# DerryHub/BEVFormer_tensorrt

Hardware: AMD Instinct MI355X
Metric: frames/sec BEVFormer-base bs=1 fp16 end-to-end on MI355X (re-hosted model, random weights, synthetic 6-camera frames) (higher is better)
Workload: dtype f16

## Files before the change

bevformer_tensorrt_amd/bevformer.py:

```python
import math
import os
import time

import torch
import torch.nn as nn
import torch.nn.functional as F

from . import functions as _hip_ops
from . import geometry as G
from .functions.dispatch import OWN_KERNELS, own_kernel_choice, using as _dispatch_using
from .functions.linear import tsgemm_weight_stationary
from .utils import lib as _lib

CONFIGS = {
    "tiny": dict(depth=50, dcn=(False, False, False, False), fpn_in=[2048], out_indices=(3,), levels=1,
                 image=(480, 800), bev=(50, 50), enc_layers=3, style="pytorch"),
    "small": dict(depth=101, dcn=(False, False, True, True), fpn_in=[2048], out_indices=(3,), levels=1,
                  image=(736, 1280), bev=(150, 150), enc_layers=3, style="caffe"),
    "base": dict(depth=101, dcn=(False, False, True, True), fpn_in=[512, 1024, 2048], out_indices=(1, 2, 3),
                 levels=4, image=(928, 1600), bev=(200, 200), enc_layers=6, style="caffe"),
}
PC_RANGE = [-51.2, -51.2, -5.0, 51.2, 51.2, 3.0]
POST_CENTER_RANGE = [-61.2, -61.2, -10.0, 61.2, 61.2, 10.0]
MAX_DETECTIONS = 300
EMBED, HEADS, NUM_QUERY, NUM_CAMS = 256, 8, 900, 6


inverse_sigmoid = G.inverse_sigmoid


_CAM_IDX = {}


def _take_cams(t, cams):
    cams = tuple(cams)
    if cams == tuple(range(t.shape[0])):
        return t
    key = (cams, str(t.device))
    idx = _CAM_IDX.get(key)
    if idx is None:
        idx = _CAM_IDX[key] = torch.tensor(cams, dtype=torch.long, device=t.device)
    return t.index_select(0, idx)


def _rows(x):
    return x.permute(0, 2, 3, 1).reshape(-1, x.shape[1])


def _from_rows(y, n, h, w):
    return y.view(n, h, w, y.shape[-1]).permute(0, 3, 1, 2)


_FUSED_LINEAR = {"enabled": os.environ.get("BEVOPS_FUSED_LINEAR", "1") != "0"}
_R3 = {"enabled": os.environ.get("BEVOPS_R3_FUSIONS", "1") != "0"}
_TSA_LOCAL = {"enabled": os.environ.get("BEVOPS_TSA_LOCAL", "1") == "1"}
_TSA_GLUE = {"enabled": os.environ.get("BEVOPS_TSA_GLUE", "1") == "1"}


def _or_none(fn, *args, **kwargs):
    try:
        return fn(*args, **kwargs)
    except _lib.BevopsError as exc:
        if exc.status != _lib.NOT_SUPPORTED:
            raise
        return None


def _fused_linear(ops, x, weight, bias, residual, relu):
    fn = getattr(ops, "linear_bias_act", None)
    if fn is None or not _FUSED_LINEAR["enabled"] or x.dtype != torch.float16 or not x.is_cuda:
        return None
    auto = getattr(ops, "dense_auto", None)
    if auto is not None and _R3["enabled"]:
        return _or_none(auto, x, weight, bias, residual, relu)
    return _or_none(fn, x, weight, bias, residual, relu)


def _gemm_entry(ops):
    return getattr(ops, "dense_auto", None) or getattr(ops, "linear_bias_act", None)


def _dense(ops, lin, x, residual=None, relu=False):
    if hasattr(lin, "fake_quant_reference"):
        return lin(x, residual, relu)
    y = _fused_linear(ops, x, lin.weight, lin.bias, residual, relu)
    if y is not None:
        return y
    y = lin(x)
    if residual is not None:
        y = y + residual
    return F.relu(y, inplace=True) if relu else y


def _mlp(ops, seq, x):
    mods = list(seq)
    if not _R3["enabled"] or not all(isinstance(m, (nn.Linear, nn.ReLU)) for m in mods):
        return seq(x)
    i = 0
    while i < len(mods):
        if isinstance(mods[i], nn.ReLU):
            x = F.relu(x)
            i += 1
            continue
        relu = i + 1 < len(mods) and isinstance(mods[i + 1], nn.ReLU)
        x = _dense(ops, mods[i], x, None, relu)
        i += 2 if relu else 1
    return x


def _layer_norm(ops, norm, x):
    fn = getattr(ops, "layer_norm", None)
    if fn is None or not _FUSED_LINEAR["enabled"] or x.dtype != torch.float16 or not x.is_cuda or \
            x.shape[-1] not in (64, 128, 256, 512):
        return norm(x)
    return fn(x, norm.weight, norm.bias, norm.eps)


_FUSED_REFINE = {"enabled": os.environ.get("BEVOPS_FUSED_REFINE", "1") == "1"}
_OWN_ATTN = {"enabled": os.environ.get("BEVOPS_OWN_ATTN", "1") == "1"}
_LN_FUSED = {"enabled": os.environ.get("BEVOPS_LN_FUSED", "1") == "1"}
_INT8_LN_FUSED = {"enabled": os.environ.get("BEVOPS_INT8_LN_FUSED", "0") == "1"}
_OWN_ENCODER = {"enabled": os.environ.get("BEVOPS_OWN_ENCODER", "1") == "1"}
_SHARDED_TABLE_BACKBONE = {"enabled": _OWN_ENCODER["enabled"] and os.environ.get("BEVOPS_SHARDED_RULE_DISPATCH", "0") != "1"}


def _dense_norm(ops, lin, x, residual, norm):
    fn = getattr(ops, "tsgemm_ln", None)
    if fn is not None and _LN_FUSED["enabled"] and _R3["enabled"] and _FUSED_LINEAR["enabled"] and type(lin) is nn.Linear \
            and x.dtype == torch.float16 and x.is_cuda and lin.out_features == EMBED and lin.in_features % 64 == 0 \
            and isinstance(norm, nn.LayerNorm) and norm.elementwise_affine and norm.normalized_shape == (EMBED,) \
            and x.numel() // x.shape[-1] >= 32:
        out = _or_none(fn, x, lin.weight, lin.bias, residual, norm.weight, norm.bias, norm.eps)
        if out is not None:
            return out
    if _int8_ln_on(ops) and _int8_norm_ok(lin, x, norm):
        return lin.forward_norm_from_q(_hip_ops.quantize_rows(x, lin.scale_in), residual, norm)
    return _layer_norm(ops, norm, _dense(ops, lin, x, residual, False))


def _int8_ln_on(ops):
    on = getattr(ops, "int8_ln_fused", None)
    return _INT8_LN_FUSED["enabled"] if on is None else on


def _int8_norm_ok(lin, x, norm):
    return hasattr(lin, "fake_quant_reference") and lin.mode == "int8" \
        and lin.in_features % 128 == 0 and lin.out_features == EMBED and x.dtype == torch.float16 and x.is_cuda \
        and isinstance(norm, nn.LayerNorm) and norm.elementwise_affine and norm.normalized_shape == (EMBED,)


def _int8_ffn_chain_ok(fc1, fc2, x, norm):
    return hasattr(fc1, "fake_quant_reference") and fc1.mode == "int8" and fc1.in_features % 16 == 0 \
        and _int8_norm_ok(fc2, x, norm)


def _conv1x1_nhwc(ops, x, conv, relu, residual=None):
    s = conv.stride[0]
    if s > 1:
        strided = getattr(ops, "conv_nhwc", None)
        if strided is not None and _R3["enabled"] and _FUSED_LINEAR["enabled"] and x.dtype == torch.float16 and x.is_cuda \
                and not hasattr(conv, "lin") and conv.in_channels % 32 == 0 and x.is_contiguous(memory_format=torch.channels_last):
            return strided(x, conv.weight, conv.bias, relu, residual, s)
        lin = getattr(conv, "lin", None)
        int8_conv = getattr(ops, "conv_int8_nhwc", None)
        if lin is not None and getattr(lin, "mode", None) == "int8" and int8_conv is not None and _R3["enabled"] \
                and x.dtype == torch.float16 and x.is_cuda and conv.in_channels % 64 == 0 \
                and x.is_contiguous(memory_format=torch.channels_last):
            return int8_conv(x, lin.scale_in, lin.weight_q.view(conv.out_channels, 1, 1, conv.in_channels), lin.scale_w,
                             lin.bias_f32, relu, residual, s)
        x = x[:, :, ::s, ::s].contiguous(memory_format=torch.channels_last)
    n, c, h, w = x.shape
    if hasattr(conv, "lin"):
        y = conv.lin(_rows(x), None if residual is None else _rows(residual), relu)
        return _from_rows(y, n, h, w)
    wt = conv.weight.view(conv.out_channels, c).t()
    if residual is not None:
        y = _fused_linear(ops, _rows(x), conv.weight.view(conv.out_channels, c), conv.bias, _rows(residual), relu)
        if y is None:
            y = torch.mm(_rows(x), wt)
            ops.bias_act_nhwc_(y, conv.bias, _rows(residual), relu)
    else:
        y = _fused_linear(ops, _rows(x), conv.weight.view(conv.out_channels, c), conv.bias, None, relu) \
            if _R3["enabled"] else None
        if y is None:
            y = torch._addmm_activation(conv.bias, _rows(x), wt) if relu else torch.addmm(conv.bias, _rows(x), wt)
    return _from_rows(y, n, h, w)


def _conv_nhwc(ops, x, conv, relu, residual=None):
    qmode = getattr(conv, "qmode", None)
    if qmode == "calibrate":
        conv.collect(x)
    elif qmode == "int8" and x.is_contiguous(memory_format=torch.channels_last):
        return conv.int8_nhwc(x, residual, relu)
    auto = getattr(ops, "conv3x3_auto", None)
    if auto is not None and _R3["enabled"] and _FUSED_LINEAR["enabled"] and x.dtype == torch.float16 and x.is_cuda \
            and conv.kernel_size == (3, 3) and conv.stride[0] == conv.stride[1] and conv.padding == (1, 1) \
            and conv.groups == 1 and conv.dilation == (1, 1) and conv.in_channels % 32 == 0 \
            and x.is_contiguous(memory_format=torch.channels_last):
        return auto(x, conv.weight, conv.bias, relu, residual, conv.stride[0])
    y = F.conv2d(x, conv.weight, None, conv.stride, conv.padding)
    if not y.is_contiguous(memory_format=torch.channels_last):
        y = y.contiguous(memory_format=torch.channels_last)
    return ops.bias_act_nhwc_(y, conv.bias, residual, relu)


class DCNv2Pack(nn.Module):

    def __init__(self, cin, cout, ops, stride=1):
        super().__init__()
        self.ops, self.stride = ops, stride
        self._c32_ok = True
        self.weight = nn.Parameter(torch.randn(cout, cin, 3, 3) / math.sqrt(cin * 9))
        self.bias = nn.Parameter(torch.zeros(cout))
        self.conv_offset = nn.Conv2d(cin, 27, 3, stride, 1)
        nn.init.normal_(self.conv_offset.weight, std=0.01)
        nn.init.zeros_(self.conv_offset.bias)

    def forward(self, x):
        out = self.conv_offset(x)
        o1, o2, mask = torch.chunk(out, 3, dim=1)
        offset = torch.cat((o1, o2), dim=1)
        return self.ops.modulated_deformable_conv2d(x, offset, torch.sigmoid(mask), self.weight,
                                                    self.bias, self.stride, 1, 1, 1, 1)

    def _chain_collect(self, om):
        cal = getattr(self, "chain_cal", None)
        if cal is not None:
            cal.collect(self.chain_site + ".offset", om[:, :18])
            cal.collect(self.chain_site + ".mask", torch.sigmoid(om[:, 18:27]))

    def forward_nhwc(self, x, relu):
        fn = getattr(self.ops, "conv_offset_nhwc", None)
        if fn is not None and self.stride == 1 and _FUSED_LINEAR["enabled"] and self._c32_ok:
            try:
                out = fn(x, self.conv_offset.weight, self.conv_offset.bias)
                self._chain_collect(out)
                return self.ops.modulated_deformable_conv2d_nhwc(x, None, None, self.weight, self.bias, self.stride,
                                                                 1, 1, 1, 1, relu=relu, offset_mask_nhwc=out)
            except _lib.BevopsError as exc:
                if exc.status != _lib.NOT_SUPPORTED:
                    raise
                self._c32_ok = False
        w = self.conv_offset.weight
        if getattr(self, "_w32", None) is None or self._w32[2] != (w._version, w.dtype, w.device):
            w32 = torch.zeros(32, *w.shape[1:], dtype=w.dtype, device=w.device)
            w32[:27] = w.detach()
            b32 = torch.zeros(32, dtype=w.dtype, device=w.device)
            b32[:27] = self.conv_offset.bias.detach()
            self._w32 = (w32.contiguous(memory_format=torch.channels_last), b32, (w._version, w.dtype, w.device))
        out = F.conv2d(x, self._w32[0], None, self.stride, 1)
        if not out.is_contiguous(memory_format=torch.channels_last):
            out = out.contiguous(memory_format=torch.channels_last)
        out = self.ops.bias_act_nhwc_(out, self._w32[1], None, False)
        self._chain_collect(out)
        return self.ops.modulated_deformable_conv2d_nhwc(x, None, None, self.weight, self.bias, self.stride, 1, 1,
                                                         1, 1, relu=relu, offset_mask_nhwc=out)


_FUSED_DOWNSAMPLE = {"enabled": os.environ.get("BEVOPS_FUSED_DOWNSAMPLE", "1") != "0"}
_FUSED_DOWNSAMPLE_SHAPES = {(64, 64, 1), (128, 256, 2), (256, 512, 2), (512, 1024, 2)}


def _two_source_ok(ops, blk, x):
    ds, c3 = blk.downsample, blk.conv3
    if ds is None or not (_FUSED_DOWNSAMPLE["enabled"] and _R3["enabled"] and _FUSED_LINEAR["enabled"]) \
            or getattr(ops, "gemm2", None) is None or getattr(blk, "chain_cal", None) is not None:
        return False
    if type(ds) is not nn.Conv2d or type(c3) is not nn.Conv2d or hasattr(ds, "lin") or hasattr(c3, "lin") \
            or ds.bias is None or c3.bias is None or ds.weight.dtype != torch.float16 or c3.weight.dtype != torch.float16 \
            or ds.kernel_size != (1, 1) or c3.kernel_size != (1, 1) or c3.stride != (1, 1) or ds.stride[0] != ds.stride[1]:
        return False
    if x.dtype != torch.float16 or not x.is_cuda or x.dim() != 4 or not x.is_contiguous(memory_format=torch.channels_last):
        return False
    return (c3.in_channels, ds.in_channels, ds.stride[0]) in _FUSED_DOWNSAMPLE_SHAPES


def _stacked_pair(blk):
    ds, c3 = blk.downsample, blk.conv3
    key = _versions(c3.weight, ds.weight, c3.bias, ds.bias)
    hit = getattr(blk, "_w3d", None)
    if hit is None or hit[0] != key:
        n = c3.out_channels
        w = torch.cat([c3.weight.detach().reshape(n, -1), ds.weight.detach().reshape(n, -1)], dim=1).contiguous()
        b = (c3.bias.detach().float() + ds.bias.detach().float()).to(c3.bias.dtype).contiguous()
        hit = (key, w, b)
        blk._w3d = hit
    return hit[1], hit[2]


class Bottleneck(nn.Module):

    def __init__(self, cin, planes, stride, dcn, ops, downsample, style="caffe"):
        super().__init__()
        s1, s2 = (stride, 1) if style == "caffe" else (1, stride)
        self.conv1 = nn.Conv2d(cin, planes, 1, s1)
        self.conv2 = DCNv2Pack(planes, planes, ops, s2) if dcn else nn.Conv2d(planes, planes, 3, s2, 1)
        self.conv3 = nn.Conv2d(planes, planes * 4, 1)
        self.downsample = nn.Conv2d(cin, planes * 4, 1, stride) if downsample else None

    def forward(self, x):
        idt = x if self.downsample is None else self.downsample(x)
        out = F.relu(self.conv1(x), inplace=True)
        out = F.relu(self.conv2(out), inplace=True)
        return F.relu(self.conv3(out) + idt, inplace=True)

    def _hidden_nhwc(self, x, ops):
        out = _conv1x1_nhwc(ops, x, self.conv1, True)
        if isinstance(self.conv2, DCNv2Pack):
            return self.conv2.forward_nhwc(out, True)
        return _conv_nhwc(ops, out, self.conv2, True)

    def forward_nhwc(self, x, ops):
        if _two_source_ok(ops, self, x):
            h = self._hidden_nhwc(x, ops)
            w, b = _stacked_pair(self)
            n, _, ho, wo = h.shape
            y = _or_none(ops.gemm2, _rows(h), x, w, b, self.downsample.stride[0], True)
            if y is not None:
                return _from_rows(y, n, ho, wo)
            return _conv1x1_nhwc(ops, h, self.conv3, True, residual=_conv1x1_nhwc(ops, x, self.downsample, False))
        idt = x if self.downsample is None else _conv1x1_nhwc(ops, x, self.downsample, False)
        out = _conv1x1_nhwc(ops, x, self.conv1, True)
        cal = getattr(self, "chain_cal", None)
        if cal is not None:
            cal.collect(self.chain_site + ".t1", out)
            if self.downsample is not None:
                cal.collect(self.chain_site + ".idt", idt)
        if isinstance(self.conv2, DCNv2Pack):
            out = self.conv2.forward_nhwc(out, True)
        else:
            out = _conv_nhwc(ops, out, self.conv2, True)
        return _conv1x1_nhwc(ops, out, self.conv3, True, residual=idt)


class ResNet(nn.Module):
    def __init__(self, depth, dcn, out_indices, ops, style="caffe"):
        super().__init__()
        blocks = {50: (3, 4, 6, 3), 101: (3, 4, 23, 3)}[depth]
        self.out_indices = out_indices
        self.stem = nn.Conv2d(3, 64, 7, 2, 3)
        cin, stages = 64, []
        for i, n in enumerate(blocks):
            planes, layers = 64 * 2 ** i, []
            for j in range(n):
                layers.append(Bottleneck(cin, planes, (2 if i > 0 else 1) if j == 0 else 1, dcn[i], ops, j == 0, style))
                cin = planes * 4
            stages.append(nn.Sequential(*layers))
        self.stages = nn.ModuleList(stages)

    def forward(self, x):
        x = F.max_pool2d(F.relu(self.stem(x), inplace=True), 3, 2, 1)
        outs = []
        for i, st in enumerate(self.stages):
            x = st(x)
            if i in self.out_indices:
                outs.append(x)
        return outs

    def _stem_fused(self, x, ops):
        fused = getattr(ops, "stem_conv_pool", None)
        if fused is None or not (_R3["enabled"] and _FUSED_LINEAR["enabled"]):
            return None
        from .functions.conv import STEM_FUSED
        st = self.stem
        ok = (STEM_FUSED["enabled"] and x.is_cuda and x.dtype == torch.float16 and x.is_contiguous() and x.shape[-1] % 2 == 0
              and tuple(st.weight.shape) == (64, 3, 7, 7) and st.stride == (2, 2) and st.padding == (3, 3))
        return fused(x, st.weight, st.bias) if ok else None

    def forward_nhwc(self, x, ops):
        y = self._stem_fused(x, ops)
        if y is not None:
            return self._stages_nhwc(y, ops)
        x = x.contiguous(memory_format=torch.channels_last)
        pool = getattr(ops, "bias_relu_maxpool_nhwc", None)
        if pool is not None and _R3["enabled"] and _FUSED_LINEAR["enabled"] and x.dtype == torch.float16 and x.is_cuda:
            y = F.conv2d(x, self.stem.weight, None, self.stem.stride, self.stem.padding)
            if not y.is_contiguous(memory_format=torch.channels_last):
                y = y.contiguous(memory_format=torch.channels_last)
            x = pool(y, self.stem.bias)
        else:
            x = F.max_pool2d(_conv_nhwc(ops, x, self.stem, True), 3, 2, 1)
        return self._stages_nhwc(x, ops)

    def _stages_nhwc(self, x, ops):
        outs = []
        for i, st in enumerate(self.stages):
            for blk in st:
                x = blk.forward_nhwc(x, ops)
            if i in self.out_indices:
                outs.append(x)
        return outs


class FPN(nn.Module):

    def __init__(self, cins, cout, num_outs):
        super().__init__()
        self.lateral = nn.ModuleList(nn.Conv2d(c, cout, 1) for c in cins)
        self.fpn = nn.ModuleList(nn.Conv2d(cout, cout, 3, 1, 1) for _ in cins)
        self.extra = nn.ModuleList(nn.Conv2d(cout, cout, 3, 2, 1) for _ in range(num_outs - len(cins)))

    def forward(self, feats):
        lat = [l(f) for l, f in zip(self.lateral, feats)]
        for i in range(len(lat) - 1, 0, -1):
            lat[i - 1] = lat[i - 1] + F.interpolate(lat[i], size=lat[i - 1].shape[2:], mode="nearest")
        outs = [c(x) for c, x in zip(self.fpn, lat)]
        for e in self.extra:
            outs.append(e(F.relu(outs[-1])))
        return outs

    def forward_nhwc(self, feats, ops):
        return self.topdown_nhwc([_conv1x1_nhwc(ops, f, l, False) for l, f in zip(self.lateral, feats)], ops)

    def topdown_nhwc(self, lat, ops):
        up_add = getattr(ops, "upsample_add_nhwc_", None)
        for i in range(len(lat) - 1, 0, -1):
            a, b = lat[i - 1], lat[i]
            if up_add is not None and _FUSED_LINEAR["enabled"] and _R3["enabled"] and a.dtype == torch.float16 and a.is_cuda \
                    and a.is_contiguous(memory_format=torch.channels_last) and b.is_contiguous(memory_format=torch.channels_last):
                up_add(a, b)
            else:
                lat[i - 1] = a + F.interpolate(b, size=a.shape[2:], mode="nearest")
        outs = [_conv_nhwc(ops, x.contiguous(memory_format=torch.channels_last), c, False) for c, x in zip(self.fpn, lat)]
        for e in self.extra:
            outs.append(_conv_nhwc(ops, F.relu(outs[-1]), e, False))
        return outs


class FFN(nn.Module):
    def __init__(self, dim=EMBED, hidden=2 * EMBED):
        super().__init__()
        self.fc1, self.fc2 = nn.Linear(dim, hidden), nn.Linear(hidden, dim)

    def forward(self, x, ops=None, norm=None):
        if norm is not None and _int8_ln_on(ops) and _int8_ffn_chain_ok(self.fc1, self.fc2, x, norm):
            h_q = self.fc1.forward_q(x, self.fc2.scale_in, relu=True)
            return self.fc2.forward_norm_from_q(h_q, x, norm)
        h = _dense(ops, self.fc1, x, None, True)
        return _dense(ops, self.fc2, h, x, False) if norm is None else _dense_norm(ops, self.fc2, h, x, norm)


class TemporalSelfAttention(nn.Module):

    def __init__(self, ops, points=4):
        super().__init__()
        self.ops, self.points = ops, points
        self.sampling_offsets = nn.Linear(EMBED * 2, 2 * HEADS * points * 2)
        self.attention_weights = nn.Linear(EMBED * 2, 2 * HEADS * points)
        self.value_proj, self.output_proj = nn.Linear(EMBED, EMBED), nn.Linear(EMBED, EMBED)
        self._split = self._pos_term = None

    def _split_projection(self, query, prev0, bev_pos, prev_term=None):
        def both_terms():
            terms = self._split_terms(query, bev_pos)
            if terms is None:
                return None
            fn, wa, wb, pos_term = terms
            t = prev_term if prev_term is not None else fn(prev0.reshape(-1, EMBED), wa, None, pos_term, False)
            return fn(query.reshape(-1, EMBED), wb, None, t, False)
        return _or_none(both_terms)

    def _split_terms(self, query, bev_pos):
        fn = _gemm_entry(self.ops)
        so, aw = self.sampling_offsets, self.attention_weights
        if fn is None or not (_R3["enabled"] and _FUSED_LINEAR["enabled"]) or query.dtype != torch.float16 \
                or not query.is_cuda or type(so) is not nn.Linear or type(aw) is not nn.Linear:
            return None
        key = (so.weight._version, aw.weight._version, so.bias._version, aw.bias._version, so.weight.data_ptr())
        if self._split is None or self._split[0] != key:
            w = torch.cat([so.weight, aw.weight]).detach()
            self._split = (key, w[:, :EMBED].contiguous(), w[:, EMBED:].contiguous(),
                           torch.cat([so.bias, aw.bias]).detach().contiguous())
            self._pos_term = None
        _, wa, wb, b = self._split
        pkey = (bev_pos.data_ptr(), bev_pos._version, tuple(bev_pos.shape), bev_pos.dtype)
        if self._pos_term is None or self._pos_term[0] != pkey:
            self._pos_term = (pkey, fn(bev_pos.reshape(-1, EMBED), wb, b, None, False))
        return fn, wa, wb, self._pos_term[1]

    def forward(self, query, value, bev_pos, ref_2d, spatial_shapes, rows=None, norm=None, prev_term=None):
        identity = query
        nq, nk = query.shape[1], value.shape[1]
        mine = value if rows is None else value[:, rows[0]:rows[1]]
        both = self._split_projection(query, mine[0], bev_pos, prev_term if rows is None else None)
        split = getattr(self.ops, "tsa_split", None) if _TSA_GLUE["enabled"] else None
        pre = None
        if both is not None and split is not None and self.points == 4:
            pre = split(both, HEADS, self.points)
        elif both is not None:
            n_off = 2 * HEADS * self.points * 2
            off = both[:, :n_off].view(1, nq, HEADS, 2, 1, self.points, 2)
            w = both[:, n_off:].view(1, nq, HEADS, 2, 1, self.points)
        else:
            query = torch.cat([mine[:1], query + bev_pos], -1)
            off = self.sampling_offsets(query).view(1, nq, HEADS, 2, 1, self.points, 2)
            w = self.attention_weights(query).view(1, nq, HEADS, 2, 1, self.points)
        value = _dense(self.ops, self.value_proj, value).view(2, nk, HEADS, EMBED // HEADS)
        if pre is not None:
            off, w = pre
        else:
            w = w.permute(0, 3, 1, 2, 4, 5).contiguous().view(2, nq, HEADS, -1)
            off = off.permute(0, 3, 1, 2, 4, 5, 6).contiguous().view(2, nq, HEADS, -1)
        msda = (getattr(self.ops, "multi_scale_deformable_attn_local", None) if _TSA_LOCAL["enabled"] else None) \
            or self.ops.multi_scale_deformable_attn
        out = msda(value, spatial_shapes, ref_2d, off, w).flatten(2)
        mean2 = getattr(self.ops, "queue_mean2", None) if _TSA_GLUE["enabled"] else None
        if mean2 is not None and out.is_cuda and out.dtype == torch.float16 and out.numel() % 16 == 0 and _R3["enabled"]:
            out = mean2(out)
        else:
            out = torch.mean(out, keepdim=True, dim=0)
        if norm is not None:
            return _dense_norm(self.ops, self.output_proj, out, identity, norm)
        return _dense(self.ops, self.output_proj, out, identity, False)


class SpatialCrossAttention(nn.Module):

    def __init__(self, ops, levels, points=8):
        super().__init__()
        self.ops = ops
        self._proj_ok = True
        self.sampling_offsets = nn.Linear(EMBED, HEADS * levels * points * 2)
        self.attention_weights = nn.Linear(EMBED, HEADS * levels * points)
        self.value_proj, self.output_proj = nn.Linear(EMBED, EMBED), nn.Linear(EMBED, EMBED)

    def _offsets_weights(self, query, nq, merged):
        pair = _merged_pair(self.ops, self, "_so_aw", self.sampling_offsets, self.attention_weights, query) if merged else None
        if pair is None:
            pair = (_dense(self.ops, self.sampling_offsets, query), _dense(self.ops, self.attention_weights, query))
        return pair[0].view(1, nq, HEADS, -1), pair[1].view(1, nq, HEADS, -1)

    def forward(self, query, value, reference_points_cam, bev_mask, spatial_shapes, cams=None, gather=None, plan=None,
                residual=None, norm=None, merged=False):
        inp_residual = query if residual is None else residual
        ncam, nk, nq = value.shape[0], value.shape[1], query.shape[1]
        mode = getattr(gather, "mode", None)
        if cams is None and gather is not None and hasattr(gather, "cams"):
            cams = gather.cams
        ref = reference_points_cam.reshape(reference_points_cam.shape[0], nq, 1, -1)
        ref_l, mask_l = (ref, bev_mask) if cams is None else (_take_cams(ref, cams), _take_cams(bev_mask, cams))
        local_sum = gather is None or mode in ("reduce", "scatter")
        projected = getattr(self.ops, "spatial_cross_attention_projected", None)
        fused = getattr(self.ops, "spatial_cross_attention_sample", None)
        fp16_gpu = value.dtype == torch.float16 and value.is_cuda
        slots = None
        if local_sum and ncam == 0:
            slots = torch.zeros((1, nq, EMBED), dtype=value.dtype, device=value.device)
        elif projected is not None and local_sum and _R3["enabled"] and self._proj_ok and fp16_gpu \
                and not hasattr(self.value_proj, "fake_quant_reference"):
            off, w = self._offsets_weights(query, nq, merged)
            try:
                slots = projected(value.reshape(ncam, nk, EMBED), self.value_proj.weight, self.value_proj.bias,
                                  spatial_shapes, ref_l.contiguous(), off, w, mask_l.contiguous(), HEADS,
                                  **({"plan": plan} if plan is not None else {}))
            except _lib.BevopsError as exc:
                if exc.status != _lib.NOT_SUPPORTED:
                    raise
                self._proj_ok = False
        if slots is None:
            value = _dense(self.ops, self.value_proj, value.reshape(ncam, nk, EMBED)).view(ncam, nk, HEADS, EMBED // HEADS)
            off, w = (t.expand(ncam, -1, -1, -1) for t in self._offsets_weights(query, nq, merged))
            msda = self.ops.multi_scale_deformable_attn
            if mode == "gather":
                ref_c = ref_l.contiguous()
                queries = gather.gather(
                    lambda i: msda(value[i:i + 1], spatial_shapes, ref_c[i:i + 1], off[:1], w[:1]).flatten(2),
                    (nq, EMBED), value.dtype, value.device)
                slots = (queries * bev_mask).sum(0, keepdim=True)
            elif local_sum and fused is not None and (fp16_gpu or getattr(fused, "any_device", False)):
                slots = fused(value, spatial_shapes, ref_l, off[:1], w[:1], mask_l)
            elif local_sum:
                queries = msda(value, spatial_shapes, ref_l.contiguous(), off, w).flatten(2)
                slots = (queries * mask_l).sum(0, keepdim=True)
            else:
                queries = gather(msda(value, spatial_shapes, ref_l.contiguous(), off, w).flatten(2))
                slots = (queries * bev_mask).sum(0, keepdim=True)
        if mode == "reduce":
            slots = gather.reduce(slots)
        elif mode == "scatter":
            slots = gather.reduce_scatter_queries(slots, nq)
        if norm is not None:
            return _dense_norm(self.ops, self.output_proj, slots, inp_residual, norm)
        return _dense(self.ops, self.output_proj, slots, inp_residual, False)


class BEVFormerLayer(nn.Module):
    def __init__(self, ops, levels):
        super().__init__()
        self.tsa, self.sca, self.ffn = TemporalSelfAttention(ops), SpatialCrossAttention(ops, levels), FFN()
        self.norms = nn.ModuleList(nn.LayerNorm(EMBED) for _ in range(3))

    def forward(self, query, value, bev_pos, ref_2d, ref_cam, bev_mask, spatial_shapes, bev_shapes, prev_bev,
                use_prev_bev, cams, gather, plan=None, rows=None, tsa_prev_term=None, merged=False):
        ops = self.tsa.ops
        if rows is not None:
            lo, hi = rows
            nq = bev_pos.shape[1]
            if torch.is_tensor(use_prev_bev) or not use_prev_bev:
                full = gather.all_gather_queries(query, nq)
                prev = torch.where(use_prev_bev.to(torch.bool), prev_bev, full.expand(2, -1, -1)) \
                    if torch.is_tensor(use_prev_bev) else full.repeat(2, 1, 1)
            else:
                prev = prev_bev
            query = self.tsa(query, prev, bev_pos[:, lo:hi], ref_2d[:, lo:hi].contiguous(), bev_shapes, rows=rows,
                             norm=self.norms[0])
            full = gather.all_gather_queries(query, nq)
            query = self.sca(full, value, ref_cam, bev_mask, spatial_shapes, cams, gather, plan, residual=query,
                             norm=self.norms[1])
            return self.ffn(query, ops, norm=self.norms[2])
        if torch.is_tensor(use_prev_bev):
            prev = torch.where(use_prev_bev.to(torch.bool), prev_bev, query.expand(2, -1, -1))
        else:
            prev = prev_bev if use_prev_bev else query.repeat(2, 1, 1)
        if prev is not prev_bev:
            tsa_prev_term = None
        query = self.tsa(query, prev, bev_pos, ref_2d, bev_shapes, norm=self.norms[0], prev_term=tsa_prev_term)
        query = self.sca(query, value, ref_cam, bev_mask, spatial_shapes, cams, gather, plan, norm=self.norms[1],
                         merged=merged)
        return self.ffn(query, ops, norm=self.norms[2])


def _static_term(cache, owner, key, pos, fn, weight, bias):
    hit = getattr(owner, cache, None)
    if hit is None or hit[0] != key or hit[1] is not pos:
        hit = (key, pos, fn(pos.reshape(-1, pos.shape[-1]), weight, bias, None, False))
        setattr(owner, cache, hit)
    return hit[2]


def _fast_dense_ok(ops, x, *linears):
    return getattr(ops, "linear_bias_act", None) is not None and _R3["enabled"] and _FUSED_LINEAR["enabled"] \
        and x.dtype == torch.float16 and x.is_cuda \
        and all(isinstance(l, nn.Linear) and not hasattr(l, "fake_quant_reference") for l in linears)


def _versions(*tensors):
    return tuple(t._version for t in tensors) + tuple(t.data_ptr() for t in tensors)


_MERGED_PROJ = {"enabled": os.environ.get("BEVOPS_MERGED_PROJ", "1") != "0"}


def _merge_ok(ops, x, linears, has_res):
    if not (_MERGED_PROJ["enabled"] and _R3["enabled"] and _FUSED_LINEAR["enabled"]) \
            or getattr(ops, "dense_auto", None) is None or x.dtype != torch.float16 or not x.is_cuda \
            or not all(type(l) is nn.Linear and l.bias is not None and l.weight.dtype == torch.float16 for l in linears):
        return False
    if not OWN_KERNELS["enabled"]:
        return False
    K = x.shape[-1]
    return _per_layer_kernels(x.device, x.numel() // K, [l.weight.shape[0] for l in linears], K, not has_res, has_res) == "tiled"


def _per_layer_kernels(device, M, widths, K, has_bias, has_res):
    if M <= 0:
        return None
    names = {own_kernel_choice(device, M, n, K, False, has_bias, has_res) for n in widths}
    if names == {"small"}:
        return "small"
    if names <= {"tile", "tsgemm"} and ("tsgemm" not in names or tsgemm_weight_stationary(K)):
        return "tiled"
    return None


def _merged_pair(ops, owner, cache, lin_a, lin_b, x):
    fn = getattr(ops, "tile_gemm_dst", None)
    widths = [lin_a.weight.shape[0], lin_b.weight.shape[0]]
    if fn is None or not _merge_ok(ops, x, (lin_a, lin_b), False) or any(n % 64 for n in widths):
        return None
    key = _versions(lin_a.weight, lin_b.weight, lin_a.bias, lin_b.bias)
    hit = getattr(owner, cache, None)
    if hit is None or hit[0] != key:
        hit = (key, torch.cat([lin_a.weight, lin_b.weight]).detach().contiguous(),
               torch.cat([lin_a.bias, lin_b.bias]).detach().contiguous())
        setattr(owner, cache, hit)
    return _or_none(fn, x.reshape(-1, x.shape[-1]), hit[1], hit[2], widths)


def _merged_prev_terms(ops, owner, cache, tsas, query, prev0, bev_pos):
    fn = getattr(ops, "tile_gemm_dst", None)
    if fn is None or not (_MERGED_PROJ["enabled"] and _R3["enabled"] and _FUSED_LINEAR["enabled"]) \
            or prev0.dtype != torch.float16 or not prev0.is_cuda:
        return None
    if not OWN_KERNELS["enabled"]:
        return None

    def all_layers():
        terms = [t._split_terms(query, bev_pos) for t in tsas]
        if any(t is None for t in terms):
            return None
        widths = [t[1].shape[0] for t in terms]
        M = prev0.numel() // EMBED
        if any(n % 64 for n in widths) or _per_layer_kernels(prev0.device, M, widths, EMBED, False, True) != "tiled":
            return None
        key = tuple(t._split[0] for t in tsas)
        hit = getattr(owner, cache, None)
        if hit is None or hit[0] != key:
            hit = (key, torch.cat([t[1] for t in terms]).contiguous())
            setattr(owner, cache, hit)
        return fn(prev0.reshape(-1, EMBED), hit[1], None, widths, [t[3] for t in terms])
    return _or_none(all_layers)


def _merged_value_proj(ops, owner, cache, linears, x):
    fn = getattr(ops, "tsgemm_grouped", None)
    if fn is None or not _merge_ok(ops, x, linears, False) \
            or not all(tuple(l.weight.shape) == (EMBED, EMBED) for l in linears):
        return None
    key = _versions(*[l.weight for l in linears], *[l.bias for l in linears])
    hit = getattr(owner, cache, None)
    if hit is None or hit[0] != key:
        hit = (key, torch.cat([l.weight for l in linears]).detach().contiguous(),
               torch.cat([l.bias for l in linears]).detach().contiguous())
        setattr(owner, cache, hit)
    return _or_none(fn, x.reshape(-1, EMBED), hit[1], hit[2])


class CustomMSDeformableAttention(nn.Module):

    def __init__(self, ops, points=4):
        super().__init__()
        self.ops = ops
        self.sampling_offsets = nn.Linear(EMBED, HEADS * points * 2)
        self.attention_weights = nn.Linear(EMBED, HEADS * points)
        self.value_proj, self.output_proj = nn.Linear(EMBED, EMBED), nn.Linear(EMBED, EMBED)
        self._pos_so = self._pos_aw = self._so_aw = None

    def _merged_offsets_weights(self, q2, t_so, t_aw):
        ops, so, aw = self.ops, self.sampling_offsets, self.attention_weights
        fn = getattr(ops, "small_gemm_dst", None)
        widths = [so.weight.shape[0], aw.weight.shape[0]]
        if fn is None or not _MERGED_PROJ["enabled"] or not OWN_KERNELS["enabled"] or widths[0] % 64 or widths[1] % 8 \
                or so.weight.dtype != torch.float16 or aw.weight.dtype != torch.float16 \
                or _per_layer_kernels(q2.device, q2.shape[0], widths, EMBED, False, True) != "small":
            return None
        key = _versions(so.weight, aw.weight)
        if self._so_aw is None or self._so_aw[0] != key:
            self._so_aw = (key, torch.cat([so.weight, aw.weight]).detach().contiguous())
        return _or_none(fn, q2, self._so_aw[1], None, widths, [t_so, t_aw])

    def forward(self, query, value, query_pos, reference_points, spatial_shapes, norm=None, projected=None, merged=False):
        identity = query
        ops, so, aw = self.ops, self.sampling_offsets, self.attention_weights
        n = query.shape[0]
        if projected is not None:
            value = projected.view(1, -1, HEADS, EMBED // HEADS)
        else:
            value = _dense(ops, self.value_proj, value.view(1, -1, EMBED)).view(1, -1, HEADS, EMBED // HEADS)
        off = w = None
        if _fast_dense_ok(ops, query, so, aw):
            fn = _gemm_entry(ops)
            try:
                t_so = _static_term("_pos_so", self, _versions(so.weight, so.bias), query_pos, fn, so.weight, so.bias)
                t_aw = _static_term("_pos_aw", self, _versions(aw.weight, aw.bias), query_pos, fn, aw.weight, aw.bias)
                pair = self._merged_offsets_weights(query.view(n, EMBED), t_so, t_aw) if merged else None
                if pair is not None:
                    off, w = pair[0].view(1, n, HEADS, -1), pair[1].view(1, n, HEADS, -1)
                else:
                    off = fn(query.view(n, EMBED), so.weight, None, t_so, False).view(1, n, HEADS, -1)
                    w = fn(query.view(n, EMBED), aw.weight, None, t_aw, False).view(1, n, HEADS, -1)
            except _lib.BevopsError as exc:
                if exc.status != _lib.NOT_SUPPORTED:
                    raise
                off = None
        if off is None:
            q = (query + query_pos).view(1, -1, EMBED)
            off = so(q).view(1, n, HEADS, -1)
            w = aw(q).view(1, n, HEADS, -1)
        out = ops.multi_scale_deformable_attn(value, spatial_shapes, reference_points, off, w).flatten(2)
        if norm is not None:
            return _dense_norm(ops, self.output_proj, out.view(n, 1, EMBED), identity, norm)
        return _dense(ops, self.output_proj, out.view(n, 1, EMBED), identity, False)


class DecoderLayer(nn.Module):
    def __init__(self, ops):
        super().__init__()
        self.self_attn = nn.MultiheadAttention(EMBED, HEADS)
        self.cross_attn, self.ffn = CustomMSDeformableAttention(ops), FFN()
        self.norms = nn.ModuleList(nn.LayerNorm(EMBED) for _ in range(3))
        self._pos_qkv = None

    def _self_attention(self, ops, query, query_pos, norm=None):
        mha = self.self_attn
        if not _fast_dense_ok(ops, query, mha.out_proj) or mha.in_proj_weight is None:
            return None
        fn, n = _gemm_entry(ops), query.shape[0]
        w, b = mha.in_proj_weight, mha.in_proj_bias
        key = _versions(w, b)
        hit = self._pos_qkv
        try:
            if hit is None or hit[0] != key or hit[1] is not query_pos:
                term = torch.empty(n, 3 * EMBED, dtype=query.dtype, device=query.device)
                term[:, :2 * EMBED] = fn(query_pos.reshape(n, EMBED), w[:2 * EMBED], b[:2 * EMBED], None, False)
                term[:, 2 * EMBED:] = b[2 * EMBED:]
                hit = self._pos_qkv = (key, query_pos, term)
            qkv = fn(query.view(n, EMBED), w, None, hit[2], False).view(1, n, 3, HEADS, EMBED // HEADS)
        except _lib.BevopsError as exc:
            if exc.status != _lib.NOT_SUPPORTED:
                raise
            return None
        own = getattr(ops, "self_attention_qkv", None) if _OWN_ATTN["enabled"] else None
        o = None
        if own is not None:
            o = _or_none(own, qkv.view(n, 3, HEADS, EMBED // HEADS))
            o = o.view(n, 1, EMBED) if o is not None else None
        if o is None:
            q, k, v = (qkv[:, :, i].transpose(1, 2) for i in range(3))
            o = F.scaled_dot_product_attention(q, k, v)
            o = o.transpose(1, 2).reshape(n, 1, EMBED)
        return _dense(ops, mha.out_proj, o, query, False) if norm is None else _dense_norm(ops, mha.out_proj, o, query, norm)

    def forward(self, query, value, query_pos, reference_points, spatial_shapes, projected=None, merged=False):
        ops = self.cross_attn.ops
        query_n = self._self_attention(ops, query, query_pos, norm=self.norms[0])
        if query_n is None:
            qk = query + query_pos
            query_n = _layer_norm(ops, self.norms[0], query + self.self_attn(qk, qk, query, need_weights=False)[0])
        query = self.cross_attn(query_n, value, query_pos, reference_points, spatial_shapes, norm=self.norms[1],
                                projected=projected, merged=merged)
        return self.ffn(query, ops, norm=self.norms[2])


class BEVFormer(nn.Module):

    def __init__(self, name="base", ops=None, seed=0, backbone_layout="auto"):
        super().__init__()
        torch.manual_seed(seed)
        cfg = CONFIGS[name]
        self.cfg, self.name = cfg, name
        self.ops = ops = ops if ops is not None else _hip_ops
        self.backbone_layout = backbone_layout
        self._nhwc_ready = False
        self.bev_h, self.bev_w = cfg["bev"]
        nq = self.bev_h * self.bev_w
        self.backbone = ResNet(cfg["depth"], cfg["dcn"], cfg["out_indices"], ops, cfg["style"])
        self.neck = FPN(cfg["fpn_in"], EMBED, cfg["levels"])
        self.bev_embedding = nn.Embedding(nq, EMBED)
        self.query_embedding = nn.Embedding(NUM_QUERY, EMBED * 2)
        self.row_embed, self.col_embed = nn.Embedding(self.bev_h, EMBED // 2), nn.Embedding(self.bev_w, EMBED // 2)
        self.cls_branches = nn.ModuleList(nn.Sequential(
            nn.Linear(EMBED, EMBED), nn.LayerNorm(EMBED), nn.ReLU(inplace=True),
            nn.Linear(EMBED, EMBED), nn.LayerNorm(EMBED), nn.ReLU(inplace=True), nn.Linear(EMBED, 10)) for _ in range(6))
        self.reg_branches = nn.ModuleList(nn.Sequential(
            nn.Linear(EMBED, EMBED), nn.ReLU(inplace=True), nn.Linear(EMBED, EMBED), nn.ReLU(inplace=True),
            nn.Linear(EMBED, 10)) for _ in range(6))
        self.level_embeds = nn.Parameter(torch.randn(cfg["levels"], EMBED) * 0.02)
        self.cams_embeds = nn.Parameter(torch.randn(NUM_CAMS, EMBED) * 0.02)
        self.reference_points = nn.Linear(EMBED, 3)
        self.can_bus_mlp = nn.Sequential(nn.Linear(18, EMBED // 2), nn.ReLU(inplace=True),
                                         nn.Linear(EMBED // 2, EMBED), nn.ReLU(inplace=True), nn.LayerNorm(EMBED))
        self.encoder = nn.ModuleList(BEVFormerLayer(ops, cfg["levels"]) for _ in range(cfg["enc_layers"]))
        self.decoder = nn.ModuleList(DecoderLayer(ops) for _ in range(6))
        self.register_buffer("rotate_center", torch.tensor([100.0, 100.0]))
        self._static = None
        self._pos_cache = self._query_cache = None
        self.eval()

    def extract_feat(self, image, cams=None):
        B, N, C, H, W = image.shape
        img = image.view(B * N, C, H, W)
        if cams is not None:
            img = _take_cams(img, cams)
        nhwc = self.backbone_layout == "nhwc" or (self.backbone_layout == "auto" and self.ops is _hip_ops)
        chain = getattr(self, "int8_chain", None)
        if chain is not None and chain.ready and img.dtype == torch.float16 and img.is_cuda:
            return chain(img)
        if nhwc and img.dtype == torch.float16 and img.is_cuda:
            if not self._nhwc_ready:
                for m in list(self.backbone.modules()) + list(self.neck.modules()):
                    if isinstance(m, nn.Conv2d) and m.kernel_size != (1, 1):
                        m.weight.data = m.weight.data.contiguous(memory_format=torch.channels_last)
                self._nhwc_ready = True
            return self.neck.forward_nhwc(self.backbone.forward_nhwc(img, self.ops), self.ops)
        return self.neck(self.backbone(img))

    def positional_encoding(self, dtype, device):
        x = self.col_embed(torch.arange(self.bev_w, device=device))
        y = self.row_embed(torch.arange(self.bev_h, device=device))
        pos = torch.cat((x.unsqueeze(0).repeat(self.bev_h, 1, 1), y.unsqueeze(1).repeat(1, self.bev_w, 1)), dim=-1)
        return pos.permute(2, 0, 1).unsqueeze(0).to(dtype)

    @torch.no_grad()
    def _geometry(self, dev):
        if self._static is None or self._static[0].device != dev:
            ref_3d = G.reference_points_3d(self.bev_h, self.bev_w, PC_RANGE[5] - PC_RANGE[2], 4, device="cpu", dtype=torch.float)
            self._static = tuple(t.to(dev) for t in (ref_3d, G.reference_points_2d(ref_3d),
                                                     G.pillar_points(ref_3d, PC_RANGE)))
        return self._static

    @torch.no_grad()
    def project(self, lidar2img, image_shape, dtype, cams=None):
        _, _, pillars = self._geometry(lidar2img.device)
        fused = getattr(self.ops, "point_sampling", None)
        if fused is not None and _R3["enabled"] and lidar2img.is_cuda and dtype in (torch.float16, torch.float32) \
                and pillars.shape[0] == 4:
            ref_cam, bev_mask = fused(pillars, lidar2img, image_shape, dtype)
        else:
            ref_cam, bev_mask = G.project_points(pillars, lidar2img.float(), image_shape, projection="fma")
            ref_cam, bev_mask = ref_cam.to(dtype), bev_mask.to(dtype)
        plan = self._sca_plan(bev_mask, cams)
        return (ref_cam, bev_mask) if plan is None else (ref_cam, bev_mask, plan)

    def _sca_plan(self, bev_mask, cams):
        fn = getattr(self.ops, "spatial_cross_attention_plan", None)
        if fn is None or not _R3["enabled"] or not bev_mask.is_cuda or bev_mask.dtype != torch.float16 \
                or self.cfg["levels"] != 4:
            return None
        mask_l = bev_mask if cams is None else _take_cams(bev_mask, cams)
        return fn(mask_l) if mask_l.shape[0] > 0 else None

    def forward(self, image, prev_bev, use_prev_bev, can_bus, lidar2img, cams=None, gather=None, shift=None, proj=None):
        mlvl = self.extract_feat(image, cams)
        own = _OWN_ENCODER["enabled"] and image.is_cuda and image.dtype == torch.float16
        with _dispatch_using(own=True if own else None):
            return self._transformer(mlvl, image, prev_bev, use_prev_bev, can_bus, lidar2img, cams, gather, shift, proj)

    def _transformer(self, mlvl, image, prev_bev, use_prev_bev, can_bus, lidar2img, cams, gather, shift, proj):
        dev, dtype = image.device, image.dtype
        image_shape = image.shape[-2:]
        bev_h, bev_w, nq = self.bev_h, self.bev_w, self.bev_h * self.bev_w
        bev_queries = self.bev_embedding.weight.to(dtype).unsqueeze(1)
        pkey = (self.col_embed.weight._version, self.row_embed.weight._version, dtype, dev)
        if _R3["enabled"] and self._pos_cache is not None and self._pos_cache[0] == pkey:
            bev_pos = self._pos_cache[1]
        else:
            bev_pos = self.positional_encoding(dtype, dev).flatten(2).permute(2, 0, 1).contiguous()
            self._pos_cache = (pkey, bev_pos)

        grid_length = ((PC_RANGE[4] - PC_RANGE[1]) / bev_h, (PC_RANGE[3] - PC_RANGE[0]) / bev_w)
        if shift is None:
            shift = G.bev_shift(can_bus.float(), bev_h, bev_w, grid_length)
        shift = shift.to(dtype)
        rot_hwc = getattr(self.ops, "rotate_hwc", None)
        stack = None
        if rot_hwc is not None and prev_bev.is_cuda and prev_bev.shape[-1] % 8 == 0 and _R3["enabled"] \
                and prev_bev.dtype == dtype and prev_bev.shape[-1] == EMBED:
            stack = torch.empty((2, nq, EMBED), dtype=dtype, device=dev)
            rot_hwc(prev_bev.view(bev_h, bev_w, -1), can_bus[-1].float().reshape(1), self.rotate_center.float(),
                    out=stack[0].view(bev_h, bev_w, EMBED))
            prev_bev = stack[0].view(nq, 1, EMBED)
            bev_queries = torch.add(bev_queries.detach(),
                                    self.can_bus_mlp(can_bus.view(1, -1).to(dtype)).view(1, 1, -1).detach(),
                                    out=stack[1].view(nq, 1, EMBED))
        elif rot_hwc is not None and prev_bev.is_cuda and prev_bev.shape[-1] % 8 == 0:
            prev_bev = rot_hwc(prev_bev.view(bev_h, bev_w, -1), can_bus[-1].float().reshape(1),
                               self.rotate_center.float()).view(nq, 1, -1)
        else:
            prev_bev = self.ops.rotate(prev_bev.view(bev_h, bev_w, -1).permute(2, 0, 1),
                                       can_bus[-1].float().reshape(1), self.rotate_center.float())
            prev_bev = prev_bev.permute(1, 2, 0).reshape(nq, 1, -1)
        if stack is None:
            bev_queries = bev_queries + self.can_bus_mlp(can_bus.view(1, -1).to(dtype)).view(1, 1, -1)
        feats, level_hw = [], []
        cam_embed = self.cams_embeds if cams is None else _take_cams(self.cams_embeds, cams)
        embed_fn = getattr(self.ops, "feat_embed_nhwc", None)
        fused_embed = embed_fn is not None and _FUSED_LINEAR["enabled"] and _R3["enabled"] and dtype == torch.float16 and image.is_cuda \
            and all(f.is_contiguous(memory_format=torch.channels_last) for f in mlvl) and mlvl[0].shape[0] > 0
        if fused_embed:
            level_hw = [f.shape[-2:] for f in mlvl]
            feat_flatten = torch.empty((mlvl[0].shape[0], sum(h * w for h, w in level_hw), EMBED), dtype=dtype, device=dev)
            row = 0
            for lvl, feat in enumerate(mlvl):
                hw = feat.shape[2] * feat.shape[3]
                embed_fn(feat.permute(0, 2, 3, 1).reshape(feat.shape[0], hw, feat.shape[1]), cam_embed,
                         self.level_embeds[lvl], feat_flatten[:, row:row + hw, :])
                row += hw
        else:
            for lvl, feat in enumerate(mlvl):
                level_hw.append(feat.shape[-2:])
                if feat.is_contiguous(memory_format=torch.channels_last):
                    f = feat.permute(0, 2, 3, 1).reshape(feat.shape[0], feat.shape[2] * feat.shape[3], feat.shape[1])
                else:
                    f = feat.flatten(2).permute(0, 2, 1)
                feats.append(f + cam_embed.to(dtype)[:, None, :] + self.level_embeds[lvl].to(dtype)[None, None, :])
            feat_flatten = torch.cat(feats, dim=1)
        spatial_shapes, _ = G.level_layout(level_hw, "cpu")
        bev_shapes = torch.tensor([[bev_h, bev_w]])

        ref_3d, ref_2d, pillars = self._geometry(dev)
        if cams is None and gather is not None and hasattr(gather, "cams"):
            cams = gather.cams
        ref_cam, bev_mask, *rest = proj if proj is not None else self.project(lidar2img, image_shape, dtype, cams)
        plan = rest[0] if rest else None
        hybrid = G.hybrid_ref_2d(ref_2d, shift.float(), use_prev_bev).to(dtype)
        q = bev_queries.view(1, nq, EMBED)
        pos = bev_pos.view(1, nq, EMBED)
        prev = stack if stack is not None else torch.cat([prev_bev.view(1, nq, EMBED), q], dim=0)
        rows = None
        if getattr(gather, "mode", None) == "scatter":
            lo, hi, _ = gather.query_range(nq)
            rows = (lo, hi)
            q = q[:, lo:hi].contiguous()
        merged = gather is None and not torch.is_tensor(use_prev_bev) and bool(use_prev_bev)
        tsa_terms = None
        if merged:
            tsa_terms = _merged_prev_terms(self.ops, self, "_tsa_wacat", [l.tsa for l in self.encoder], q, prev[0], pos)
        for li, layer in enumerate(self.encoder):
            q = layer(q, feat_flatten, pos, hybrid, ref_cam, bev_mask, spatial_shapes, bev_shapes, prev,
                      use_prev_bev, cams, gather, plan, rows, None if tsa_terms is None else tsa_terms[li], merged)
            if tsa_terms is not None:
                tsa_terms[li] = None
        if rows is not None:
            q = gather.all_gather_queries(q, nq)
        bev_embed = q.view(nq, 1, EMBED)

        qkey = _versions(self.query_embedding.weight, self.reference_points.weight, self.reference_points.bias) + (dtype, dev)
        if _R3["enabled"] and self._query_cache is not None and self._query_cache[0] == qkey:
            _, query_pos, query, reference_points = self._query_cache
        else:
            query_pos, query = (t.contiguous() for t in
                                torch.split(self.query_embedding.weight.to(dtype).unsqueeze(1), EMBED, dim=2))
            reference_points = self.reference_points(query_pos).sigmoid().view(1, NUM_QUERY, 3)
            self._query_cache = (qkey, query_pos, query, reference_points)
        init_reference = reference_points
        inter, inter_refs, regs = [], [], []
        out = query
        fused_refine = getattr(self.ops, "refine_reference_points", None) if _FUSED_REFINE["enabled"] and _R3["enabled"] \
            and dtype == torch.float16 and dev.type == "cuda" else None
        ref_xy = reference_points[..., :2].unsqueeze(2).contiguous()
        dec_values = _merged_value_proj(self.ops, self, "_dec_vcat", [l.cross_attn.value_proj for l in self.decoder],
                                        bev_embed) if merged else None
        for lid, layer in enumerate(self.decoder):
            out = layer(out, bev_embed, query_pos, ref_xy, bev_shapes, None if dec_values is None else dec_values[lid], merged)
            tmp = _mlp(self.ops, self.reg_branches[lid], out).view(1, -1, 10)
            if fused_refine is not None:
                reference_points, ref_xy = fused_refine(tmp, reference_points)
            else:
                reference_points = G.refine_reference_points(tmp, reference_points)
                ref_xy = reference_points[..., :2].unsqueeze(2).contiguous()
            inter.append(out)
            inter_refs.append(reference_points)
            regs.append(tmp)

        if not _R3["enabled"]:
            classes, coords = [], []
            for lvl in range(6):
                reference = inverse_sigmoid(init_reference if lvl == 0 else inter_refs[lvl - 1])
                hs = inter[lvl].view(1, NUM_QUERY, EMBED)
                crd = self.reg_branches[lvl](hs).clone()
                crd[..., 0:2] = (crd[..., 0:2] + reference[..., 0:2]).sigmoid()
                crd[..., 4:5] = (crd[..., 4:5] + reference[..., 2:3]).sigmoid()
                crd[..., 0:1] = crd[..., 0:1] * (PC_RANGE[3] - PC_RANGE[0]) + PC_RANGE[0]
                crd[..., 1:2] = crd[..., 1:2] * (PC_RANGE[4] - PC_RANGE[1]) + PC_RANGE[1]
                crd[..., 4:5] = crd[..., 4:5] * (PC_RANGE[5] - PC_RANGE[2]) + PC_RANGE[2]
                classes.append(self.cls_branches[lvl](hs))
                coords.append(crd)
            return bev_embed, torch.stack(classes), torch.stack(coords)
        crd = torch.stack(regs)
        decode = getattr(self.ops, "decode_boxes", None) if fused_refine is not None else None
        hs = torch.stack(inter).view(6, NUM_QUERY, EMBED)
        if decode is not None:
            crd = decode(crd, torch.stack([init_reference] + inter_refs[:-1]), PC_RANGE)
            return bev_embed, self._cls_batched(hs).view(6, 1, NUM_QUERY, -1), crd
        reference = inverse_sigmoid(torch.stack([init_reference] + inter_refs[:-1]))
        crd[..., 0:2] = (crd[..., 0:2] + reference[..., 0:2]).sigmoid()
        crd[..., 4:5] = (crd[..., 4:5] + reference[..., 2:3]).sigmoid()
        crd[..., 0:1] = crd[..., 0:1] * (PC_RANGE[3] - PC_RANGE[0]) + PC_RANGE[0]
        crd[..., 1:2] = crd[..., 1:2] * (PC_RANGE[4] - PC_RANGE[1]) + PC_RANGE[1]
        crd[..., 4:5] = crd[..., 4:5] * (PC_RANGE[5] - PC_RANGE[2]) + PC_RANGE[2]
        return bev_embed, self._cls_batched(hs).view(6, 1, NUM_QUERY, -1), crd

    @property
    def bbox_coder(self):
        from .postprocess import NMSFreeCoder
        if getattr(self, "_bbox_coder", None) is None:
            self._bbox_coder = NMSFreeCoder(PC_RANGE, voxel_size=[0.512, 0.512, 8], post_center_range=POST_CENTER_RANGE,
                                            max_num=MAX_DETECTIONS, num_classes=10)
        return self._bbox_coder

    def get_bboxes(self, classes, coords, padded=False):
        padded_out = self.bbox_coder.decode_padded(classes[-1], coords[-1], bottom_center=True)
        if padded:
            return padded_out
        from .postprocess import _dicts
        return _dicts(padded_out, 9, torch.int64, classes.device)

    def _cls_batched(self, hs):
        key = tuple(p._version for p in self.cls_branches.parameters()) + (hs.dtype, hs.device)
        if getattr(self, "_cls_stack", None) is None or self._cls_stack[0] != key:
            st = lambda k, attr: torch.stack([getattr(b[k], attr).detach() for b in self.cls_branches]).to(hs.dtype)
            self._cls_stack = (key, [(st(k, "weight").transpose(1, 2).contiguous(), st(k, "bias").unsqueeze(1)) for k in (0, 3, 6)],
                               [(st(k, "weight").unsqueeze(1), st(k, "bias").unsqueeze(1), self.cls_branches[0][k].eps) for k in (1, 4)])
        _, lin, norm = self._cls_stack
        x = hs
        for i in range(3):
            x = torch.baddbmm(lin[i][1], x, lin[i][0])
            if i < 2:
                g, b, eps = norm[i]
                x = F.relu(F.layer_norm(x, (x.shape[-1],), None, None, eps) * g + b, inplace=True)
        return x


def use_tuned_gemms(path=None):
    import os
    path = path or os.path.join(os.path.dirname(os.path.abspath(__file__)), "tunableop_gfx950.csv")
    try:
        if not os.path.exists(path) or os.environ.get("PYTORCH_TUNABLEOP_ENABLED") is not None:
            return False
        import torch.cuda.tunable as tunable
        tunable.enable(True)
        tunable.tuning_enable(False)
        tunable.set_filename(path)
        tunable.read_file(path)
        return True
    except Exception:
        return False


class FrameRunner:

    def __init__(self, model, device, dtype, graph=False, cams=None, gather=None, clone_outputs=True, decode=False,
                 raw_size=None):
        self.model, self.device, self.dtype, self.clone_outputs = model, device, dtype, clone_outputs
        self.cams, self.gather, self.decode = cams, gather, decode
        self.tuned_gemms = use_tuned_gemms() if device.type == "cuda" else False
        nq = model.bev_h * model.bev_w
        self.prev_bev = torch.zeros(nq, 1, EMBED, device=device, dtype=dtype)
        self.prev = {"scene": None, "pos": None, "angle": None}
        self.use_graph, self._graphs, self._graphs_raw, self._use = graph, {}, {}, 0.0
        H, W = model.cfg["image"]
        self.raw_size, self.pipeline = None, None
        if raw_size is not None:
            from .functions.image import BEVFORMER_IMAGE_PIPELINES, padded_size, scaled_size
            self.raw_size = (int(raw_size[0]), int(raw_size[1]))
            self.pipeline = BEVFORMER_IMAGE_PIPELINES[model.name]
            net = padded_size(*scaled_size(*self.raw_size, self.pipeline["scale"]), self.pipeline["size_divisor"])
            if tuple(net) != (H, W):
                raise ValueError(f"raw_size {self.raw_size}: the {model.name} pipeline (scale {self.pipeline['scale']}, "
                                 f"pad to {self.pipeline['size_divisor']}) gives {net}, the model takes {(H, W)}")
        n_small = 20 + NUM_CAMS * 16
        small = torch.zeros(n_small, device=device)
        self._host_small = torch.zeros(n_small)
        self._in = dict(image=torch.zeros(1, NUM_CAMS, 3, H, W, device=device, dtype=dtype),
                        small=small, can_bus=small[:18], shift=small[18:20].view(1, 2),
                        lidar2img=small[20:].view(1, NUM_CAMS, 4, 4),
                        use=torch.zeros((), device=device, dtype=dtype))
        if self.raw_size is not None:
            self._in["raw"] = torch.zeros((NUM_CAMS,) + self.raw_size + (3,), device=device, dtype=torch.uint8)

    @property
    def image_buffer(self):
        return self._in["image"]

    @property
    def raw_buffer(self):
        return self._in.get("raw")

    @property
    def _graph(self):
        return self._graphs.get(self._use, (None, None))[0]

    def _prepare(self):
        fn = getattr(self.model.ops, "image_normalize_resize_pad", None)
        if fn is None:
            raise RuntimeError("the operator set has no image_normalize_resize_pad")
        p, buf = self.pipeline, self._in["image"][0]
        fn(self._in["raw"], scale=p["scale"], mean=p["mean"], std=p["std"], to_rgb=p["to_rgb"],
           size_divisor=p["size_divisor"], dtype=buf.dtype, out=buf)

    def _forward(self, raw=False):
        if raw:
            self._prepare()
        if self.gather is not None and self.device.type == "cuda" and not _SHARDED_TABLE_BACKBONE["enabled"]:
            with _dispatch_using(rule=True):
                return self._forward_impl()
        return self._forward_impl()

    def _forward_impl(self):
        i = self._in
        if not _R3["enabled"]:
            return self.model(i["image"], self.prev_bev, i["use"], i["can_bus"], i["lidar2img"], self.cams, self.gather,
                              shift=i["shift"])
        return self.model(i["image"], self.prev_bev, self._use, i["can_bus"], i["lidar2img"], self.cams, self.gather,
                          shift=i["shift"])

    def _capture(self, raw=False):
        s = torch.cuda.Stream()
        s.wait_stream(torch.cuda.current_stream())
        with torch.cuda.stream(s):
            for _ in range(2):
                out = self._forward(raw)
                if self.decode:
                    self.model.get_bboxes(out[1], out[2], padded=True)
        torch.cuda.current_stream().wait_stream(s)
        graph = torch.cuda.CUDAGraph()
        kw = {"capture_error_mode": "thread_local"} if self.gather is not None else {}
        if self.gather is not None or (torch.distributed.is_available() and torch.distributed.is_initialized()):
            torch.cuda.synchronize()
            time.sleep(0.35)
        with torch.cuda.graph(graph, **kw):
            bev, cls, crd = self._forward(raw)
            self.prev_bev.copy_(bev)
            det = self.model.get_bboxes(cls, crd, padded=True) if self.decode else ()
        (self._graphs_raw if raw else self._graphs)[self._use] = (graph, (cls, crd) + tuple(det))

    def step_raw(self, raw_images, can_bus, lidar2img, scene_token):
        if self.raw_size is not None:
            from .functions.image import scale_lidar2img
            buf = self._in["raw"]
            if raw_images.dtype != torch.uint8 or tuple(raw_images.shape) != tuple(buf.shape):
                raise ValueError(f"raw_images must be uint8 {list(buf.shape)}")
            if raw_images.data_ptr() != buf.data_ptr():
                buf.copy_(raw_images, non_blocking=True)
            return self._step(None, can_bus, scale_lidar2img(lidar2img, self.pipeline["scale"]), scene_token, raw=True)
        fn = getattr(self.model.ops, "image_normalize_pad", None)
        if fn is None:
            raise RuntimeError("the operator set has no image_normalize_pad")
        buf = self._in["image"][0]
        fn(raw_images, dtype=buf.dtype, out=buf)
        return self.step(buf[None], can_bus, lidar2img, scene_token)

    def step(self, image, can_bus, lidar2img, scene_token):
        return self._step(image, can_bus, lidar2img, scene_token)

    def _step(self, image, can_bus, lidar2img, scene_token, raw=False):
        can_bus = can_bus.clone().float()
        use_prev = 0.0 if scene_token != self.prev["scene"] else 1.0
        pos, angle = can_bus[:3].clone(), can_bus[-1].clone()
        if use_prev:
            can_bus[:3] -= self.prev["pos"]
            can_bus[-1] -= self.prev["angle"]
        else:
            can_bus[:3] = 0
            can_bus[-1] = 0
        self.prev.update(scene=scene_token, pos=pos, angle=angle)
        i = self._in
        if not raw and image.data_ptr() != i["image"].data_ptr():
            i["image"].copy_(image, non_blocking=True)
        m = self.model
        grid_length = ((PC_RANGE[4] - PC_RANGE[1]) / m.bev_h, (PC_RANGE[3] - PC_RANGE[0]) / m.bev_w)
        can_host = can_bus.cpu()
        self._host_small[:18] = can_host
        self._host_small[18:20] = G.bev_shift(can_host, m.bev_h, m.bev_w, grid_length)[0]
        on_host = lidar2img.device.type == "cpu"
        if on_host:
            self._host_small[20:] = lidar2img.detach().reshape(-1).to(torch.float32)
        i["small"].copy_(self._host_small)
        if not on_host:
            i["lidar2img"].copy_(lidar2img.detach().reshape(i["lidar2img"].shape), non_blocking=True)
        if not _R3["enabled"]:
            i["use"].fill_(use_prev)
        self._use = use_prev
        if self.use_graph:
            graphs = self._graphs_raw if raw else self._graphs
            if self._use not in graphs:
                saved = self.prev_bev.clone()
                self._capture(raw)
                self.prev_bev.copy_(saved)
            graph, outs = graphs[self._use]
            graph.replay()
            return tuple(t.clone() for t in outs) if self.clone_outputs else outs
        bev_embed, cls, crd = self._forward(raw)
        self.prev_bev = bev_embed
        if self.decode:
            return (cls, crd) + tuple(self.model.get_bboxes(cls, crd, padded=True))
        return cls, crd
```

bevformer_tensorrt_amd/csrc/capi.hip:

```cpp
#include <string.h>

#include "common.h"

extern "C" const char *bevops_version(void) { return "bevops-hip 0.1 (gfx950)"; }

extern "C" const char *bevops_status_string(int status) {
  switch (status) {
    case BEVOPS_SUCCESS: return "success";
    case BEVOPS_FAILURE: return "failure (kernel launch error)";
    case BEVOPS_BAD_PARAM: return "bad parameter";
    case BEVOPS_NOT_SUPPORTED: return "dtype/shape combination not supported";
    case BEVOPS_NOT_INITIALIZED: return "not initialized";
    default: return "unknown status";
  }
}

namespace {
struct Entry {
  const char *name;
  void *fn;
};
const Entry kTable[] = {
    {"bevops_msda_forward", (void *)&bevops_msda_forward},
    {"bevops_msda_forward_ws", (void *)&bevops_msda_forward_ws},
    {"bevops_msda_workspace_size", (void *)&bevops_msda_workspace_size},
    {"MultiScaleDeformableAttnTRT", (void *)&bevops_msda_forward},
    {"MultiScaleDeformableAttnTRT2", (void *)&bevops_msda_forward},
    {"bevops_rotate_forward", (void *)&bevops_rotate_forward},
    {"RotateTRT", (void *)&bevops_rotate_forward},
    {"RotateTRT2", (void *)&bevops_rotate_forward},
    {"bevops_grid_sampler_2d_forward", (void *)&bevops_grid_sampler_2d_forward},
    {"GridSampler2DTRT", (void *)&bevops_grid_sampler_2d_forward},
    {"GridSampler2DTRT2", (void *)&bevops_grid_sampler_2d_forward},
    {"bevops_grid_sampler_3d_forward", (void *)&bevops_grid_sampler_3d_forward},
    {"GridSampler3DTRT", (void *)&bevops_grid_sampler_3d_forward},
    {"GridSampler3DTRT2", (void *)&bevops_grid_sampler_3d_forward},
    {"bevops_bev_pool_v2_forward", (void *)&bevops_bev_pool_v2_forward},
    {"BEVPoolV2TRT", (void *)&bevops_bev_pool_v2_forward},
    {"BEVPoolV2TRT2", (void *)&bevops_bev_pool_v2_forward},
    {"bevops_mdconv_forward", (void *)&bevops_mdconv_forward},
    {"bevops_mdconv_workspace_size", (void *)&bevops_mdconv_workspace_size},
    {"bevops_mdconv_forward_int8", (void *)&bevops_mdconv_forward_int8},
    {"bevops_mdconv_forward_int8_packed", (void *)&bevops_mdconv_forward_int8_packed},
    {"ModulatedDeformableConv2dTRT", (void *)&bevops_mdconv_forward},
    {"ModulatedDeformableConv2dTRT2", (void *)&bevops_mdconv_forward},
    {"bevops_qkv_forward", (void *)&bevops_qkv_forward},
    {"bevops_qkv_workspace_size", (void *)&bevops_qkv_workspace_size},
    {"QKVTRT", (void *)&bevops_qkv_forward},
    {"QKVTRT2", (void *)&bevops_qkv_forward},
    {"bevops_inverse_forward", (void *)&bevops_inverse_forward},
    {"InverseTRT", (void *)&bevops_inverse_forward},
    {"bevops_nms_free_decode", (void *)&bevops_nms_free_decode},
    {"bevops_centerpoint_decode", (void *)&bevops_centerpoint_decode},
    {"bevops_centerpoint_decode_ex", (void *)&bevops_centerpoint_decode_ex},
    {"bevops_centerpoint_decode_workspace_size", (void *)&bevops_centerpoint_decode_workspace_size},
    {"bevops_bev_nms", (void *)&bevops_bev_nms},
    {"bevops_bev_nms_workspace_size", (void *)&bevops_bev_nms_workspace_size},
    {"bevops_bev_iou", (void *)&bevops_bev_iou},
    {"bevops_centernet_decode", (void *)&bevops_centernet_decode},
    {"bevops_centernet_decode_workspace_size", (void *)&bevops_centernet_decode_workspace_size},
    {"bevops_yolox_decode", (void *)&bevops_yolox_decode},
    {"bevops_box_nms", (void *)&bevops_box_nms},
    {"bevops_box_nms_workspace_size", (void *)&bevops_box_nms_workspace_size},
    {"bevops_lss_voxel_prepare", (void *)&bevops_lss_voxel_prepare},
    {"bevops_lss_voxel_prepare_workspace_size", (void *)&bevops_lss_voxel_prepare_workspace_size},
    {"bevops_lss_voxel_prepare_batched", (void *)&bevops_lss_voxel_prepare_batched},
    {"bevops_lss_voxel_prepare_batched_workspace_size", (void *)&bevops_lss_voxel_prepare_batched_workspace_size},
    {"bevops_bev_pool_v2_forward_indirect", (void *)&bevops_bev_pool_v2_forward_indirect},
    {"bevops_grid_sampler_2d_forward_ws", (void *)&bevops_grid_sampler_2d_forward_ws},
    {"bevops_grid_sampler_2d_workspace_size", (void *)&bevops_grid_sampler_2d_workspace_size},
    {"bevops_rotate_forward_hwc", (void *)&bevops_rotate_forward_hwc},
    {"bevops_sca_forward", (void *)&bevops_sca_forward},
    {"bevops_mdconv_forward_nhwc", (void *)&bevops_mdconv_forward_nhwc},
    {"bevops_conv3x3_c32_forward_nhwc", (void *)&bevops_conv3x3_c32_forward_nhwc},
    {"bevops_bias_act_nhwc", (void *)&bevops_bias_act_nhwc},
    {"bevops_bias_relu_maxpool_nhwc", (void *)&bevops_bias_relu_maxpool_nhwc},
    {"bevops_stem_packed_size", (void *)&bevops_stem_packed_size},
    {"bevops_stem_pack", (void *)&bevops_stem_pack},
    {"bevops_stem_conv_pool", (void *)&bevops_stem_conv_pool},
    {"bevops_stem_set_variant", (void *)&bevops_stem_set_variant},
    {"bevops_upsample_add_nhwc", (void *)&bevops_upsample_add_nhwc},
    {"bevops_lss_depth_split", (void *)&bevops_lss_depth_split},
    {"bevops_upsample_bilinear_concat_nhwc", (void *)&bevops_upsample_bilinear_concat_nhwc},
    {"bevops_lss_depth_split_s8", (void *)&bevops_lss_depth_split_s8},
    {"bevops_upsample_bilinear_s8", (void *)&bevops_upsample_bilinear_s8},
    {"bevops_tsa_split", (void *)&bevops_tsa_split},
    {"bevops_queue_mean2", (void *)&bevops_queue_mean2},
    {"bevops_tsgemm_f16", (void *)&bevops_tsgemm_f16},
    {"bevops_tsgemm_s8", (void *)&bevops_tsgemm_s8},
    {"bevops_tsgemm_s8_ln", (void *)&bevops_tsgemm_s8_ln},
    {"bevops_tsgemm_tile_rows", (void *)&bevops_tsgemm_tile_rows},
    {"bevops_tsgemm_f16_ln", (void *)&bevops_tsgemm_f16_ln},
    {"bevops_tsgemm_f16_grouped", (void *)&bevops_tsgemm_f16_grouped},
    {"bevops_mha_selfattn_f16", (void *)&bevops_mha_selfattn_f16},
    {"bevops_mha_selfattn_max_queries", (void *)&bevops_mha_selfattn_max_queries},
    {"bevops_value_proj_packed_size", (void *)&bevops_value_proj_packed_size},
    {"bevops_value_proj_packed", (void *)&bevops_value_proj_packed},
    {"bevops_value_pack_planes", (void *)&bevops_value_pack_planes},
    {"bevops_sca_prepacked_workspace_size", (void *)&bevops_sca_prepacked_workspace_size},
    {"bevops_sca_forward_prepacked", (void *)&bevops_sca_forward_prepacked},
    {"bevops_sca_plan_size", (void *)&bevops_sca_plan_size},
    {"bevops_sca_plan_build", (void *)&bevops_sca_plan_build},
    {"bevops_sca_forward_planned", (void *)&bevops_sca_forward_planned},
    {"bevops_point_sampling", (void *)&bevops_point_sampling},
    {"bevops_feat_embed_nhwc", (void *)&bevops_feat_embed_nhwc},
    {"bevops_linear_bias_act", (void *)&bevops_linear_bias_act},
    {"bevops_linear_tune", (void *)&bevops_linear_tune},
    {"bevops_quantize_rows", (void *)&bevops_quantize_rows},
    {"bevops_dequantize_rows", (void *)&bevops_dequantize_rows},
    {"bevops_linear_int8", (void *)&bevops_linear_int8},
    {"bevops_linear_int8_fused", (void *)&bevops_linear_int8_fused},
    {"bevops_tile_gemm_f16", (void *)&bevops_tile_gemm_f16},
    {"bevops_tile_gemm_f16_dst", (void *)&bevops_tile_gemm_f16_dst},
    {"bevops_gemm2_f16", (void *)&bevops_gemm2_f16},
    {"bevops_small_gemm_f16_dst", (void *)&bevops_small_gemm_f16_dst},
    {"bevops_small_gemm_f16", (void *)&bevops_small_gemm_f16},
    {"bevops_conv_tile_f16", (void *)&bevops_conv_tile_f16},
    {"bevops_conv3x3_c64_f16", (void *)&bevops_conv3x3_c64_f16},
    {"bevops_deconv4x4s2_packed_weight_size", (void *)&bevops_deconv4x4s2_packed_weight_size},
    {"bevops_deconv4x4s2_pack_weight", (void *)&bevops_deconv4x4s2_pack_weight},
    {"bevops_deconv4x4s2_f16", (void *)&bevops_deconv4x4s2_f16},
    {"bevops_conv_slice_f16", (void *)&bevops_conv_slice_f16},
    {"bevops_conv_slice_f16_ex", (void *)&bevops_conv_slice_f16_ex},
    {"bevops_lss_camera_gate_packed_size", (void *)&bevops_lss_camera_gate_packed_size},
    {"bevops_lss_camera_gate", (void *)&bevops_lss_camera_gate},
    {"bevops_se_gate2_nhwc", (void *)&bevops_se_gate2_nhwc},
    {"bevops_global_avgpool_nhwc", (void *)&bevops_global_avgpool_nhwc},
    {"bevops_focus_nhwc", (void *)&bevops_focus_nhwc},
    {"bevops_spp_maxpool_nhwc", (void *)&bevops_spp_maxpool_nhwc},
    {"bevops_upsample_nearest2x_nhwc", (void *)&bevops_upsample_nearest2x_nhwc},
    {"bevops_conv_slice_s8", (void *)&bevops_conv_slice_s8},
    {"bevops_conv_slice_s8_ex", (void *)&bevops_conv_slice_s8_ex},
    {"bevops_conv_slice_s8_ex2", (void *)&bevops_conv_slice_s8_ex2},
    {"bevops_se_gate2_nhwc_s8", (void *)&bevops_se_gate2_nhwc_s8},
    {"bevops_global_avgpool_nhwc_s8", (void *)&bevops_global_avgpool_nhwc_s8},
    {"bevops_deconv4x4s2_s8", (void *)&bevops_deconv4x4s2_s8},
    {"bevops_focus_nhwc_q", (void *)&bevops_focus_nhwc_q},
    {"bevops_spp_maxpool_nhwc_s8", (void *)&bevops_spp_maxpool_nhwc_s8},
    {"bevops_upsample_nearest2x_nhwc_s8", (void *)&bevops_upsample_nearest2x_nhwc_s8},
    {"bevops_refine_reference_points", (void *)&bevops_refine_reference_points},
    {"bevops_decode_boxes", (void *)&bevops_decode_boxes},
    {"bevops_conv_tile_int8_fused", (void *)&bevops_conv_tile_int8_fused},
    {"bevops_linear_int8_chain", (void *)&bevops_linear_int8_chain},
    {"bevops_conv_tile_int8", (void *)&bevops_conv_tile_int8},
    {"bevops_bias_relu_maxpool_nhwc_int8", (void *)&bevops_bias_relu_maxpool_nhwc_int8},
    {"bevops_mdconv_int8_nhwc_workspace_size", (void *)&bevops_mdconv_int8_nhwc_workspace_size},
    {"bevops_mdconv_forward_int8_nhwc", (void *)&bevops_mdconv_forward_int8_nhwc},
    {"bevops_image_normalize_pad", (void *)&bevops_image_normalize_pad},
    {"bevops_image_normalize_resize_pad", (void *)&bevops_image_normalize_resize_pad},
    {"bevops_image_letterbox", (void *)&bevops_image_letterbox},
    {"bevops_image_resize_plan_size", (void *)&bevops_image_resize_plan_size},
    {"bevops_image_resize_plan_build", (void *)&bevops_image_resize_plan_build},
    {"bevops_image_resize_crop_normalize", (void *)&bevops_image_resize_crop_normalize},
    {"bevops_msda_packed_size", (void *)&bevops_msda_packed_size},
    {"bevops_msda_pack_value", (void *)&bevops_msda_pack_value},
    {"bevops_msda_forward_prepacked", (void *)&bevops_msda_forward_prepacked},
    {"bevops_linear_workspace_size", (void *)&bevops_linear_workspace_size},
    {"bevops_msda_workspace_size_shapes", (void *)&bevops_msda_workspace_size_shapes},
    {"bevops_sca_workspace_size", (void *)&bevops_sca_workspace_size},
    {"bevops_mdconv_forward_packed", (void *)&bevops_mdconv_forward_packed},
    {"bevops_mdconv_pack_weight", (void *)&bevops_mdconv_pack_weight},
    {"bevops_mdconv_packed_weight_size", (void *)&bevops_mdconv_packed_weight_size},
    {"bevops_conv3x3_c32_pack_weight", (void *)&bevops_conv3x3_c32_pack_weight},
    {"bevops_conv3x3_c32_packed_weight_size", (void *)&bevops_conv3x3_c32_packed_weight_size},
    {"bevops_layer_norm", (void *)&bevops_layer_norm},
    {"bevops_calib_state_size", (void *)&bevops_calib_state_size},
    {"bevops_calib_collect", (void *)&bevops_calib_collect},
    {"bevops_calib_threshold_workspace_size", (void *)&bevops_calib_threshold_workspace_size},
    {"bevops_calib_threshold", (void *)&bevops_calib_threshold},
    {"bevops_deform_conv3x3_nhwc_f16", (void *)&bevops_deform_conv3x3_nhwc_f16},
};
}

extern "C" void *bevops_query(const char *name) {
  if (!name) return nullptr;
  for (const Entry &e : kTable)
    if (strcmp(e.name, name) == 0) return e.fn;
  return nullptr;
}
```

bevformer_tensorrt_amd/functions/__init__.py:

```python
from .multi_scale_deformable_attn import (
    multi_scale_deformable_attn,
    multi_scale_deformable_attn2,
    multi_scale_deformable_attn_int8,
    multi_scale_deformable_attn_local,
    msda_pack_value,
    multi_scale_deformable_attn_prepacked,
)
from .rotate import rotate, rotate2, rotate_int8, rotate_hwc
from .grid_sampler import grid_sampler, grid_sampler2, grid_sampler_int8
from .bev_pool_v2 import bev_pool_v2, bev_pool_v2_2, bev_pool_v2_int8
from .modulated_deformable_conv2d import (modulated_deformable_conv2d, modulated_deformable_conv2d2,
                                          modulated_deformable_conv2d_int8, modulated_deformable_conv2d_nhwc,
                                          bias_act_nhwc_, bias_relu_maxpool_nhwc, conv_offset_nhwc, upsample_add_nhwc_,
                                          feat_embed_nhwc)
from .spatial_cross_attention import (spatial_cross_attention_sample, spatial_cross_attention_projected,
                                      spatial_cross_attention_plan)
from .linear import (linear_bias_act, layer_norm, quantize_rows, dequantize_rows, linear_int8, tsgemm, tsgemm_ln, tsgemm_grouped, tile_gemm, tile_gemm_dst, gemm2, small_gemm, small_gemm_dst,
                     dense_auto, tsa_split, queue_mean2)
from .int8_chain import linear_int8_chain, linear_int8_ln, conv_int8_chain_nhwc, modulated_deformable_conv2d_int8_nhwc
from .conv import conv_nhwc, conv3x3_nhwc, conv3x3_auto, conv3x3_c64, conv_int8_nhwc, stem_conv_pool
from .image import (image_normalize_pad, padded_size, bevdet_test_augmentation, bevdet_post_transform, image_resize_plan,
                    image_resize_crop_normalize, BEVFORMER_IMAGE_PIPELINES, scaled_size, scale_lidar2img,
                    image_normalize_resize_pad, DETECT2D_IMAGE_PIPELINES, keep_ratio_size, yolox_test_geometry,
                    centernet_test_geometry, image_letterbox)
from .point_sampling import point_sampling
from .attention import self_attention_qkv
from .refine import refine_reference_points, decode_boxes
from .multi_head_attn import qkv, qkv2
from .inverse import inverse
from .decode import nms_free_decode, centerpoint_decode
from .nms import bev_nms, nms_bev, circle_nms, bev_iou
from .decode2d import centernet_decode, yolox_decode, box_nms
from .lss_prepare import (lss_voxel_prepare, lss_lidar_coor, bev_pool_v2_indirect, lss_voxel_prepare_batched,
                          lss_lidar_coor_batched)
from .calibrate import calib_state_size, calib_collect, calib_threshold
from .bev_half import lss_depth_split, upsample_bilinear_concat_nhwc, lss_depth_split_q, upsample_bilinear_nhwc_q
from .deconv import conv_transpose2d_nhwc, pack_deconv4x4s2, deconv_packed_weight, conv_transpose2d_q_nhwc, quantize_deconv_weight
from .yolox_ops import (conv_slice_nhwc, conv_slice_taps, conv_slice_packed_weight, focus_nhwc, spp_maxpool_nhwc,
                        upsample_nearest2x_nhwc, pad_channels, unpad_channels, conv_slice_q_taps, focus_nhwc_q,
                        quantize_weight_taps)
from .lss_depthnet import (lss_camera_gate, se_gate2_nhwc, global_avgpool_nhwc, pack_camera_gate, camera_gate_packed,
                           se_gate2_nhwc_q, global_avgpool_nhwc_q)
from .deform_conv import deform_conv2d, deform_conv2d_nhwc, deform_conv_packed_weight
from ..utils.register import TRT_FUNCTIONS

TRT_FUNCTIONS.register_module(module=multi_scale_deformable_attn)
TRT_FUNCTIONS.register_module(module=multi_scale_deformable_attn2)
TRT_FUNCTIONS.register_module(module=multi_scale_deformable_attn_int8)
for _f in (rotate, rotate2, rotate_int8, grid_sampler, grid_sampler2, grid_sampler_int8,
           bev_pool_v2, bev_pool_v2_2, bev_pool_v2_int8, modulated_deformable_conv2d,
           modulated_deformable_conv2d2, modulated_deformable_conv2d_int8,
           spatial_cross_attention_sample, inverse, qkv, qkv2):
    TRT_FUNCTIONS.register_module(module=_f)

__all__ = [
    "multi_scale_deformable_attn",
    "multi_scale_deformable_attn2",
    "multi_scale_deformable_attn_int8",
    "rotate", "rotate2", "rotate_int8",
    "grid_sampler", "grid_sampler2", "grid_sampler_int8",
    "bev_pool_v2", "bev_pool_v2_2", "bev_pool_v2_int8",
    "modulated_deformable_conv2d", "modulated_deformable_conv2d2", "modulated_deformable_conv2d_int8",
    "inverse", "qkv", "qkv2",
    "nms_free_decode", "centerpoint_decode",
    "bev_nms", "nms_bev", "circle_nms", "bev_iou",
    "centernet_decode", "yolox_decode", "box_nms",
    "lss_voxel_prepare", "lss_lidar_coor", "bev_pool_v2_indirect", "lss_voxel_prepare_batched", "lss_lidar_coor_batched",
    "calib_state_size", "calib_collect", "calib_threshold",
    "bevdet_test_augmentation", "bevdet_post_transform", "image_resize_plan", "image_resize_crop_normalize",
    "BEVFORMER_IMAGE_PIPELINES", "scaled_size", "scale_lidar2img", "image_normalize_resize_pad",
    "DETECT2D_IMAGE_PIPELINES", "keep_ratio_size", "yolox_test_geometry", "centernet_test_geometry", "image_letterbox",
    "spatial_cross_attention_sample", "spatial_cross_attention_projected", "spatial_cross_attention_plan", "modulated_deformable_conv2d_nhwc", "bias_act_nhwc_", "linear_bias_act", "layer_norm", "rotate_hwc", "conv_offset_nhwc", "upsample_add_nhwc_", "feat_embed_nhwc",
    "msda_pack_value", "multi_scale_deformable_attn_prepacked", "multi_scale_deformable_attn_local", "image_normalize_pad", "padded_size", "quantize_rows", "dequantize_rows", "linear_int8", "tsgemm", "tsgemm_ln", "tsgemm_grouped", "tile_gemm", "tile_gemm_dst", "gemm2", "small_gemm_dst", "small_gemm", "dense_auto", "tsa_split", "queue_mean2", "conv_nhwc", "conv3x3_nhwc", "conv3x3_auto", "conv3x3_c64", "conv_int8_nhwc", "bias_relu_maxpool_nhwc", "stem_conv_pool", "point_sampling", "self_attention_qkv", "refine_reference_points", "decode_boxes",
    "linear_int8_chain", "linear_int8_ln", "conv_int8_chain_nhwc", "modulated_deformable_conv2d_int8_nhwc",
    "lss_depth_split", "upsample_bilinear_concat_nhwc", "lss_depth_split_q", "upsample_bilinear_nhwc_q",
    "conv_transpose2d_nhwc", "pack_deconv4x4s2", "deconv_packed_weight", "conv_transpose2d_q_nhwc", "quantize_deconv_weight",
    "conv_slice_nhwc", "conv_slice_taps", "conv_slice_packed_weight", "focus_nhwc", "spp_maxpool_nhwc",
    "upsample_nearest2x_nhwc", "pad_channels", "unpad_channels",
    "conv_slice_q_taps", "focus_nhwc_q", "quantize_weight_taps",
    "lss_camera_gate", "se_gate2_nhwc", "global_avgpool_nhwc", "pack_camera_gate", "camera_gate_packed",
    "se_gate2_nhwc_q", "global_avgpool_nhwc_q",
    "deform_conv2d", "deform_conv2d_nhwc", "deform_conv_packed_weight",
]
```

bevformer_tensorrt_amd/functions/linear.py:

```python
import ctypes
import os

import torch

from ..utils import lib as _lib
from ..utils import workspace as _ws
from . import dispatch as _dispatch
from .dispatch import (DENSE_LOG, DENSE_MISSES, DETERMINISTIC, OWN_KERNELS, _DENSE_CHOICE, _TABLE,
                       _dense_default, _dense_deterministic, _dense_own, _problem, _small_pays, _table, graph_time_us,
                       own_kernel_choice)


_TUNED = set()


def _tune_once(handle, key, args, x2, out_shape):
    _TUNED.add(key)
    if os.environ.get("BEVOPS_LINEAR_TUNE", "1") == "0":
        return
    scratch = torch.empty(out_shape, dtype=x2.dtype, device=x2.device)
    a = list(args)
    a[5] = scratch.data_ptr()
    handle.bevops_linear_tune(*a)


def _operands(x, weight, bias, residual, out, bias_dtype=torch.float16, res_dtypes=None, out_dtype=None):
    K, N = x.shape[-1], weight.shape[0]
    if weight.shape[1] != K:
        raise ValueError(f"weight {tuple(weight.shape)} does not match x [..., {K}]")
    x2 = x.reshape(-1, K)
    if not x2.is_contiguous():
        x2 = x2.contiguous()
    if not weight.is_contiguous():
        weight = weight.contiguous()
    M = x2.shape[0]
    r2 = None
    if residual is not None:
        if residual.dtype not in (res_dtypes or (x.dtype,)) or residual.numel() != M * N:
            raise ValueError(f"residual must be {res_dtypes or x.dtype} with M*N elements")
        r2 = residual.reshape(M, N)
        if not r2.is_contiguous():
            r2 = r2.contiguous()
    if bias is not None and (bias.dtype != bias_dtype or not bias.is_contiguous()):
        bias = bias.to(bias_dtype).contiguous()
    if out is None:
        out = torch.empty((M, N), dtype=out_dtype or x.dtype, device=x.device)
    elif out is not False:
        assert out.is_contiguous() and out.numel() == M * N and out.dtype == (out_dtype or x.dtype)
    return x2, weight, bias, r2, out, M, N, K


def _like_rows(out, x, N):
    return out.view(*x.shape[:-1], N)


def _ptr(t):
    return t.data_ptr() if t is not None else None


def _call(entry, device, *args):
    handle = _lib.load_library()
    with torch.cuda.device(device):
        st = getattr(handle, entry)(*args, _lib.current_stream_ptr(device))
    _lib.check(st, entry)


def _gemm_f16(entry, x, weight, bias, residual, relu, out, max_rows=None, launch=None):
    assert x.is_cuda and x.dtype == torch.float16 and weight.dtype == torch.float16
    x2, weight, bias, r2, out, M, N, K = _operands(x, weight, bias, residual, out)
    if max_rows is not None and M > max_rows:
        raise _lib.BevopsError(f"{entry}: more than {max_rows} rows (the tiled GEMMs' domain)", _lib.NOT_SUPPORTED)
    if M == 0:
        return _like_rows(out, x, N)
    handle = _lib.load_library()
    stream = _lib.current_stream_ptr(x.device)
    args = (x2.data_ptr(), weight.data_ptr(), _ptr(bias), _ptr(r2), out.data_ptr(), M, N, K, int(bool(relu)))
    with torch.cuda.device(x.device):
        st = getattr(handle, entry)(*args, stream) if launch is None else launch(handle, args, stream)
    _lib.check(st, entry)
    return _like_rows(out, x, N)


def linear_bias_act(x, weight, bias=None, residual=None, relu=False, out=None):
    def launch(handle, args, stream):
        nbytes = handle.bevops_linear_workspace_size() if os.environ.get("BEVOPS_LINEAR_WS", "1") != "0" else 0
        ws = _ws.lend("linear", nbytes, x.device, stream) if nbytes else None
        full = (_lib.F16,) + args + (_ptr(ws), nbytes, stream)
        key = (str(x.device),) + args[5:8] + (bool(relu), args[2] is not None, args[3] is not None)
        if key not in _TUNED and not torch.cuda.is_current_stream_capturing():
            _tune_once(handle, key, full, x, args[5:7])
        return handle.bevops_linear_bias_act(*full)
    return _gemm_f16("bevops_linear_bias_act", x, weight, bias, residual, relu, out, launch=launch)


def layer_norm(x, weight=None, bias=None, eps=1e-5, out=None):
    assert x.is_cuda and x.dtype == torch.float16
    C = x.shape[-1]
    x2 = x.reshape(-1, C)
    if not x2.is_contiguous():
        x2 = x2.contiguous()
    if out is None:
        out = torch.empty_like(x2)
    else:
        assert out.is_contiguous() and out.numel() == x2.numel() and out.dtype == x.dtype
    w = weight.to(torch.float16).contiguous() if weight is not None else None
    b = bias.to(torch.float16).contiguous() if bias is not None else None
    if x2.shape[0] == 0:
        return out.view(x.shape)
    _call("bevops_layer_norm", x.device, _lib.F16, x2.data_ptr(), _ptr(w), _ptr(b), out.data_ptr(), x2.shape[0], C, float(eps))
    return out.view(x.shape)


def _scaled_rows(entry, x, scale, out_dtype, out=None):
    x = x.contiguous()
    if x.numel() % 8:
        raise ValueError("element count must be a multiple of 8")
    if out is None:
        out = torch.empty(x.shape, dtype=out_dtype, device=x.device)
    if x.numel() == 0:
        return out
    _call(entry, x.device, _lib.F16, x.data_ptr(), out.data_ptr(), x.numel(), float(scale))
    return out


def quantize_rows(x, scale, out=None):
    assert x.is_cuda and x.dtype == torch.float16
    return _scaled_rows("bevops_quantize_rows", x, scale, torch.int8, out)


def dequantize_rows(q, scale):
    assert q.is_cuda and q.dtype == torch.int8
    return _scaled_rows("bevops_dequantize_rows", q, scale, torch.float16)


def linear_int8(a_q, scale_a, w_q, scale_w, bias=None, residual=None, relu=False, out_dtype=torch.float16,
                scale_out=1.0):
    assert a_q.is_cuda and a_q.dtype in (torch.int8, torch.float16) and w_q.dtype == torch.int8
    fused = a_q.dtype == torch.float16
    a2, w_q, b, r, out, M, N, K = _operands(a_q, w_q, bias, residual, None, bias_dtype=torch.float32,
                                            res_dtypes=(torch.float16,), out_dtype=out_dtype)
    per_channel = torch.is_tensor(scale_w)
    ws = scale_w.float().contiguous() if per_channel else None
    if M == 0:
        return _like_rows(out, a_q, N)
    _call("bevops_linear_int8_fused" if fused else "bevops_linear_int8", a_q.device,
          a2.data_ptr(), float(scale_a), w_q.data_ptr(), _ptr(ws), 1.0 if per_channel else float(scale_w), _ptr(b),
          _ptr(r), _lib.torch_dtype_code(out), out.data_ptr(), float(scale_out), M, N, K, int(bool(relu)))
    return _like_rows(out, a_q, N)


def tsgemm(x, weight, bias=None, residual=None, relu=False, out=None):
    return _gemm_f16("bevops_tsgemm_f16", x, weight, bias, residual, relu, out)


def tsgemm_grouped(x, weight, bias=None, out=None):
    assert x.is_cuda and x.dtype == torch.float16 and weight.dtype == torch.float16
    x2, weight, bias, _, _, M, N, K = _operands(x, weight, bias, None, False)
    if N % 256 != 0 or N == 0:
        raise ValueError(f"weight {tuple(weight.shape)} must be [G * 256, {K}]")
    G = N // 256
    if out is None:
        out = torch.empty((G, M, 256), dtype=x.dtype, device=x.device)
    else:
        assert out.is_contiguous() and tuple(out.shape) == (G, M, 256) and out.dtype == x.dtype
    if M == 0:
        return out
    _call("bevops_tsgemm_f16_grouped", x.device, x2.data_ptr(), weight.data_ptr(), _ptr(bias), out.data_ptr(), M * 256, M, G, K)
    return out


def tsgemm_ln(x, weight, bias, residual, ln_weight, ln_bias, eps=1e-5):
    g, b = ln_weight.to(torch.float16).contiguous(), ln_bias.to(torch.float16).contiguous()
    return _gemm_f16("bevops_tsgemm_f16_ln", x, weight, bias, residual, False, None, launch=lambda handle, a, stream:
                     handle.bevops_tsgemm_f16_ln(*a[:4], g.data_ptr(), b.data_ptr(), float(eps), *a[4:8], stream))


def tile_gemm(x, weight, bias=None, residual=None, relu=False, out=None):
    return _gemm_f16("bevops_tile_gemm_f16", x, weight, bias, residual, relu, out)


class _GemmDst(ctypes.Structure):
    _fields_ = [("col_begin", ctypes.c_int), ("col_end", ctypes.c_int), ("out", ctypes.c_void_p),
                ("out_pitch", ctypes.c_longlong), ("res", ctypes.c_void_p), ("res_pitch", ctypes.c_longlong)]


def tile_gemm_dst(x, weight, bias, widths, residuals=None, relu=False, outs=None, _entry="bevops_tile_gemm_f16_dst"):
    assert x.is_cuda and x.dtype == torch.float16 and weight.dtype == torch.float16
    x2, weight, bias, _, _, M, N, K = _operands(x, weight, bias, None, False)
    if sum(widths) != N:
        raise ValueError(f"weight {tuple(weight.shape)} does not match widths {list(widths)}")
    if outs is None:
        outs = [torch.empty((M, n), dtype=x.dtype, device=x.device) for n in widths]
    residuals = residuals if residuals is not None else [None] * len(widths)
    if M == 0:
        return outs
    tab = (_GemmDst * len(widths))()
    col = 0
    for i, n in enumerate(widths):
        o, r = outs[i], residuals[i]
        assert o.dtype == x.dtype and tuple(o.shape) == (M, n) and (n == 1 or o.stride(1) == 1)
        tab[i].col_begin, tab[i].col_end, tab[i].out, tab[i].out_pitch = col, col + n, o.data_ptr(), o.stride(0) if M > 1 else n
        if r is not None:
            if r.dtype != x.dtype or tuple(r.shape) != (M, n) or r.stride(1) != 1:
                raise ValueError("residual must be fp16 [M, width] with unit column stride")
            tab[i].res, tab[i].res_pitch = r.data_ptr(), r.stride(0) if M > 1 else n
        col += n
    _call(_entry, x.device, x2.data_ptr(), weight.data_ptr(), _ptr(bias), ctypes.addressof(tab), len(widths), M, N, K,
          int(bool(relu)))
    return outs


def gemm2(a1, a2, weight, bias=None, stride=1, relu=False, out=None):
    assert a1.is_cuda and a1.dtype == torch.float16 and a2.dtype == torch.float16 and weight.dtype == torch.float16
    if a2.dim() != 4 or not a2.is_contiguous(memory_format=torch.channels_last):
        raise ValueError("a2 must be a 4-d tensor in channels-last memory")
    B, K2, H, W = a2.shape
    K1, N = a1.shape[-1], weight.shape[0]
    if weight.shape[1] != K1 + K2:
        raise ValueError(f"weight {tuple(weight.shape)} does not match [N, {K1} + {K2}]")
    x1 = a1.reshape(-1, K1)
    if not x1.is_contiguous():
        x1 = x1.contiguous()
    if not weight.is_contiguous():
        weight = weight.contiguous()
    if bias is not None and (bias.dtype != torch.float16 or not bias.is_contiguous()):
        bias = bias.to(torch.float16).contiguous()
    M = x1.shape[0]
    if out is None:
        out = torch.empty((M, N), dtype=a1.dtype, device=a1.device)
    else:
        assert out.is_contiguous() and out.numel() == M * N and out.dtype == a1.dtype
    if M == 0:
        return out
    _call("bevops_gemm2_f16", a1.device, x1.data_ptr(), a2.data_ptr(), weight.data_ptr(), _ptr(bias), out.data_ptr(), M, N,
          K1, K2, B, H, W, int(stride), int(bool(relu)))
    return out


def small_gemm_dst(x, weight, bias, widths, residuals=None, relu=False, outs=None):
    if x.numel() // x.shape[-1] > 8192:
        raise _lib.BevopsError("small_gemm_dst: more than 8192 rows (the tiled GEMMs' domain)", _lib.NOT_SUPPORTED)
    return tile_gemm_dst(x, weight, bias, widths, residuals, relu, outs, _entry="bevops_small_gemm_f16_dst")


def tsgemm_weight_stationary(K):
    return _lib.load_library().bevops_tsgemm_tile_rows(int(K)) == 64


def small_gemm(x, weight, bias=None, residual=None, relu=False, out=None):
    return _gemm_f16("bevops_small_gemm_f16", x, weight, bias, residual, relu, out, max_rows=8192)


def _torch_dense(x, weight, bias, residual, relu):
    if residual is not None or bias is None:
        raise _lib.BevopsError("torch addmm path: bias required, no identity term", _lib.NOT_SUPPORTED)
    x2 = x.reshape(-1, x.shape[-1])
    y = torch._addmm_activation(bias, x2, weight.t()) if relu else torch.addmm(bias, x2, weight.t())
    return y.view(*x.shape[:-1], weight.shape[0])


_DENSE = {"tsgemm": tsgemm, "tile": tile_gemm, "small": small_gemm, "blaslt": linear_bias_act, "torch": _torch_dense}


def dense_auto(x, weight, bias=None, residual=None, relu=False):
    K, N = x.shape[-1], weight.shape[0]
    M = x.numel() // K
    if M == 0:
        return x.new_empty((*x.shape[:-1], N))
    key = (str(x.device), M, N, K, bool(relu), bias is not None, residual is not None)
    name, keep, miss = _dispatch.dense_choice(key, DETERMINISTIC["enabled"], OWN_KERNELS["enabled"],
                                              torch.cuda.is_current_stream_capturing, _dispatch._tune, _table(_TABLE),
                                              _DENSE_CHOICE.get(key))
    if miss and _problem(key) not in DENSE_MISSES:
        DENSE_MISSES.append(_problem(key))
    if name == "measure":
        name = _dense_measure(key, x, weight, bias, residual, relu)
    if keep:
        _DENSE_CHOICE[key] = name
    try:
        return _DENSE[name](x, weight, bias, residual, relu)
    except _lib.BevopsError as exc:
        if exc.status != _lib.NOT_SUPPORTED or name == "blaslt":
            raise
        return linear_bias_act(x, weight, bias, residual, relu)


def _dense_measure(key, x, weight, bias, residual, relu, rounds=3, iters=8):
    with torch.cuda.device(x.device):
        times = _dispatch.measure(_DENSE, lambda name: _DENSE[name](x, weight, bias, residual, relu), iters, rounds)
    DENSE_LOG.append((key, {k: round(v, 1) for k, v in times.items()}))
    return min(times, key=times.get) if times else "blaslt"


def tsa_split(both, heads, points):
    assert both.is_cuda and both.dtype == torch.float16 and both.dim() == 2 and both.is_contiguous()
    nq = both.shape[0]
    assert both.shape[1] == heads * 2 * points * 3
    off = torch.empty((2, nq, heads, points * 2), dtype=both.dtype, device=both.device)
    w = torch.empty((2, nq, heads, points), dtype=both.dtype, device=both.device)
    _call("bevops_tsa_split", both.device, _lib.F16, both.data_ptr(), off.data_ptr(), w.data_ptr(), nq, heads, points)
    return off, w


def queue_mean2(x):
    assert x.is_cuda and x.dtype == torch.float16 and x.shape[0] == 2 and x.is_contiguous()
    out = torch.empty((1,) + tuple(x.shape[1:]), dtype=x.dtype, device=x.device)
    if out.numel() == 0:
        return out
    _call("bevops_queue_mean2", x.device, _lib.F16, x.data_ptr(), out.data_ptr(), out.numel())
    return out
```

bevformer_tensorrt_amd/utils/lib.py:

```python
import ctypes
import os

_PKG = os.path.dirname(os.path.dirname(os.path.abspath(__file__)))
_LIB = None

c_int, c_float, c_void_p, c_size_t = ctypes.c_int, ctypes.c_float, ctypes.c_void_p, ctypes.c_size_t

SIGNATURES = {
    "bevops_version": (ctypes.c_char_p, []),
    "bevops_status_string": (ctypes.c_char_p, [c_int]),
    "bevops_query": (c_void_p, [ctypes.c_char_p]),
    "bevops_msda_set_variant": (c_int, [c_int]),
    "bevops_msda_forward": (c_int, [c_int, c_void_p, c_void_p, c_void_p, c_void_p, c_int,
                                    c_void_p, c_void_p, c_void_p] + [c_int] * 8 +
                            [c_float] * 4 + [c_void_p]),
    "bevops_msda_workspace_size": (c_size_t, [c_int] * 8),
    "bevops_msda_workspace_size_shapes": (c_size_t, [c_int, c_void_p] + [c_int] * 7),
    "bevops_msda_forward_ws": (c_int, [c_int, c_void_p, c_void_p, c_void_p, c_void_p, c_int,
                                       c_void_p, c_void_p, c_void_p] + [c_int] * 8 +
                               [c_float] * 4 + [c_int, c_void_p, c_size_t, c_void_p]),
    "bevops_msda_packed_size": (c_size_t, [c_int, c_void_p] + [c_int] * 7),
    "bevops_msda_pack_value": (c_int, [c_int, c_int, c_void_p, c_void_p, c_void_p, c_size_t] + [c_int] * 7 + [c_void_p]),
    "bevops_msda_forward_prepacked": (c_int, [c_int, c_void_p, c_size_t, c_void_p, c_void_p, c_int, c_void_p, c_void_p,
                                              c_void_p] + [c_int] * 8 + [c_float] * 4 + [c_int, c_void_p]),
    "bevops_sca_workspace_size": (c_size_t, [c_int, c_void_p] + [c_int] * 7),
    "bevops_sca_forward": (c_int, [c_int] + [c_void_p] * 7 + [c_int] * 8 + [c_void_p, c_size_t, c_void_p]),
    "bevops_rotate_forward": (c_int, [c_int, c_void_p, c_void_p, c_void_p, c_int, c_void_p,
                                      c_int, c_int, c_int, c_int, c_float, c_float, c_void_p]),
    "bevops_grid_sampler_2d_forward": (c_int, [c_int, c_void_p, c_void_p, c_void_p] + [c_int] * 9 +
                                       [c_float] * 3 + [c_void_p]),
    "bevops_grid_sampler_2d_workspace_size": (c_size_t, [c_int] * 5),
    "bevops_grid_sampler_2d_forward_ws": (c_int, [c_int, c_void_p, c_void_p, c_void_p] + [c_int] * 9 +
                                          [c_float] * 3 + [c_void_p, c_size_t, c_void_p]),
    "bevops_bev_pool_v2_forward": (c_int, [c_int] + [c_void_p] * 8 + [c_int] * 4 + [c_float] * 3 +
                                   [c_void_p]),
    "bevops_mdconv_set_variant": (c_int, [c_int]),
    "bevops_mdconv_workspace_size": (c_size_t, [c_int] * 16),
    "bevops_mdconv_forward_int8": (c_int, [c_void_p, c_float, c_void_p, c_float, c_void_p, c_float,
                                           c_void_p, c_float, c_void_p, c_void_p, c_float, c_void_p,
                                           c_size_t] + [c_int] * 15 + [c_void_p]),
    "bevops_mdconv_forward_int8_packed": (c_int, [c_void_p, c_float, c_void_p, c_float, c_void_p, c_float,
                                           c_void_p, c_float, c_void_p, c_void_p, c_float, c_void_p,
                                           c_size_t] + [c_int] * 15 + [c_void_p]),
    "bevops_mdconv_forward": (c_int, [c_int] + [c_void_p] * 7 + [c_size_t] + [c_int] * 15 +
                              [c_void_p]),
    "bevops_mdconv_forward_packed": (c_int, [c_int] + [c_void_p] * 7 + [c_size_t] + [c_int] * 15 +
                                     [c_void_p]),
    "bevops_mdconv_forward_nhwc": (c_int, [c_int] + [c_void_p] * 6 + [c_int, c_int, c_void_p, c_size_t] + [c_int] * 15 +
                                   [c_void_p]),
    "bevops_bias_act_nhwc": (c_int, [c_int, c_void_p, c_void_p, c_void_p, c_size_t, c_int, c_int, c_void_p]),
    "bevops_value_proj_packed_size": (c_size_t, [c_void_p] + [c_int] * 7),
    "bevops_value_proj_packed": (c_int, [c_void_p] * 5 + [c_size_t] + [c_int] * 7 + [c_void_p]),
    "bevops_value_pack_planes": (c_int, [c_void_p, c_void_p, c_void_p, c_size_t] + [c_int] * 7 + [c_void_p]),
    "bevops_sca_prepacked_workspace_size": (c_size_t, [c_int] * 4),
    "bevops_sca_forward_prepacked": (c_int, [c_int, c_void_p, c_size_t] + [c_void_p] * 6 + [c_int] * 8 +
                                     [c_void_p, c_size_t, c_void_p]),
    "bevops_sca_plan_size": (c_size_t, [c_int, c_int]),
    "bevops_sca_plan_build": (c_int, [c_int, c_void_p, c_int, c_int, c_void_p, c_size_t, c_void_p]),
    "bevops_sca_forward_planned": (c_int, [c_int, c_void_p, c_size_t] + [c_void_p] * 6 + [c_size_t, c_void_p] + [c_int] * 8 +
                                   [c_void_p, c_size_t, c_void_p]),
    "bevops_point_sampling": (c_int, [c_int, c_void_p, c_void_p, c_void_p, c_void_p, c_int, c_int, c_int, c_float, c_float,
                                      c_void_p]),
    "bevops_tsgemm_f16": (c_int, [c_void_p] * 5 + [ctypes.c_longlong, c_int, c_int, c_int, c_void_p]),
    "bevops_tsgemm_f16_grouped": (c_int, [c_void_p] * 4 + [ctypes.c_longlong, ctypes.c_longlong, c_int, c_int, c_void_p]),
    "bevops_tsgemm_set_variant": (c_int, [c_int]),
    "bevops_tsgemm_tile_rows": (c_int, [c_int]),
    "bevops_tsgemm_f16_ln": (c_int, [c_void_p] * 6 + [c_float, c_void_p, ctypes.c_longlong, c_int, c_int, c_void_p]),
    "bevops_mha_selfattn_max_queries": (c_size_t, []),
    "bevops_mha_selfattn_f16": (c_int, [c_void_p, c_void_p, c_int, c_int, c_int, c_float, c_void_p]),
    "bevops_tsgemm_s8": (c_int, [c_void_p, c_float, c_void_p, c_void_p, c_float, c_void_p, c_void_p, c_int, c_float, c_int,
                                 c_void_p, c_float, ctypes.c_longlong, c_int, c_int, c_int, c_void_p]),
    "bevops_tsgemm_s8_ln": (c_int, [c_void_p, c_float, c_void_p, c_void_p, c_float, c_void_p, c_void_p, c_int, c_float,
                                    c_void_p, c_void_p, c_float, c_void_p, ctypes.c_longlong, c_int, c_int, c_void_p]),
    "bevops_tsa_split": (c_int, [c_int, c_void_p, c_void_p, c_void_p, c_int, c_int, c_int, c_void_p]),
    "bevops_queue_mean2": (c_int, [c_int, c_void_p, c_void_p, c_size_t, c_void_p]),
    "bevops_upsample_add_nhwc": (c_int, [c_int, c_void_p, c_void_p] + [c_int] * 6 + [c_void_p]),
    "bevops_lss_depth_split": (c_int, [c_int, c_void_p, c_void_p, c_void_p] + [c_int] * 7 + [c_void_p]),
    "bevops_upsample_bilinear_concat_nhwc": (c_int, [c_int, c_void_p, c_void_p, c_void_p] + [c_int] * 7 + [c_void_p]),
    "bevops_lss_depth_split_s8": (c_int, [c_void_p, c_void_p, c_void_p] + [c_int] * 7 + [c_float, c_float, c_void_p]),
    "bevops_upsample_bilinear_s8": (c_int, [c_void_p, c_int, c_float, c_void_p, c_int, c_float] + [c_int] * 6 +
                                    [c_void_p]),
    "bevops_feat_embed_nhwc": (c_int, [c_int, c_void_p, c_void_p, c_void_p, c_void_p, c_int, c_size_t, c_int, c_size_t,
                                       c_void_p]),
    "bevops_conv3x3_c32_set_variant": (c_int, [c_int]),
    "bevops_conv3x3_c32_packed_weight_size": (c_size_t, [c_int, c_int]),
    "bevops_conv3x3_c32_pack_weight": (c_int, [c_int, c_void_p, c_void_p, c_int, c_int, c_void_p]),
    "bevops_conv3x3_c32_forward_nhwc": (c_int, [c_int, c_void_p, c_void_p, c_void_p, c_void_p, c_int, c_int, c_int,
                                                c_int, c_void_p]),
    "bevops_rotate_set_variant": (c_int, [c_int]),
    "bevops_rotate_forward_hwc": (c_int, [c_int, c_void_p, c_void_p, c_void_p, c_int, c_void_p,
                                          c_int, c_int, c_int, c_int, c_void_p]),
    "bevops_layer_norm": (c_int, [c_int, c_void_p, c_void_p, c_void_p, c_void_p, c_size_t, c_int, c_float, c_void_p]),
    "bevops_linear_workspace_size": (c_size_t, []),
    "bevops_linear_bias_act": (c_int, [c_int] + [c_void_p] * 5 + [ctypes.c_longlong, c_int, c_int, c_int,
                                                                  c_void_p, c_size_t, c_void_p]),
    "bevops_image_normalize_pad": (c_int, [c_int, c_void_p, c_int, c_void_p] + [c_int] * 5 +
                                   [ctypes.POINTER(ctypes.c_double), ctypes.POINTER(ctypes.c_double), c_int, c_int, c_void_p]),
    "bevops_image_normalize_resize_pad": (c_int, [c_int, c_void_p, c_int, c_void_p] + [c_int] * 7 +
                                          [ctypes.POINTER(ctypes.c_double), ctypes.POINTER(ctypes.c_double), c_int, c_int,
                                           c_void_p]),
    "bevops_image_letterbox": (c_int, [c_int, c_void_p, c_int, c_void_p] + [c_int] * 9 +
                               [ctypes.POINTER(ctypes.c_double)] * 3 + [c_int, c_int, c_void_p]),
    "bevops_image_resize_plan_size": (c_size_t, [c_int] * 8),
    "bevops_image_resize_plan_build": (c_int, [c_int] * 8 + [c_void_p, c_size_t]),
    "bevops_image_resize_crop_normalize": (c_int, [c_void_p, c_void_p, c_size_t, c_int, c_void_p, c_void_p] + [c_int] * 10 +
                                           [ctypes.POINTER(ctypes.c_double), ctypes.POINTER(ctypes.c_double), c_int, c_int,
                                            c_int, c_void_p]),
    "bevops_quantize_rows": (c_int, [c_int, c_void_p, c_void_p, c_size_t, c_float, c_void_p]),
    "bevops_dequantize_rows": (c_int, [c_int, c_void_p, c_void_p, c_size_t, c_float, c_void_p]),
    "bevops_linear_int8": (c_int, [c_void_p, c_float, c_void_p, c_void_p, c_float, c_void_p, c_void_p, c_int, c_void_p,
                                   c_float, ctypes.c_longlong, c_int, c_int, c_int, c_void_p]),
    "bevops_linear_int8_fused": (c_int, [c_void_p, c_float, c_void_p, c_void_p, c_float, c_void_p, c_void_p, c_int, c_void_p,
                                         c_float, ctypes.c_longlong, c_int, c_int, c_int, c_void_p]),
    "bevops_small_gemm_f16": (c_int, [c_void_p] * 5 + [ctypes.c_longlong, c_int, c_int, c_int, c_void_p]),
    "bevops_tile_gemm_f16": (c_int, [c_void_p] * 5 + [ctypes.c_longlong, c_int, c_int, c_int, c_void_p]),
    "bevops_tile_gemm_f16_dst": (c_int, [c_void_p] * 4 + [c_int, ctypes.c_longlong, c_int, c_int, c_int, c_void_p]),
    "bevops_gemm2_f16": (c_int, [c_void_p] * 5 + [ctypes.c_longlong] + [c_int] * 8 + [c_void_p]),
    "bevops_small_gemm_f16_dst": (c_int, [c_void_p] * 4 + [c_int, ctypes.c_longlong, c_int, c_int, c_int, c_void_p]),
    "bevops_conv_tile_f16": (c_int, [c_void_p] * 5 + [c_int] * 8 + [c_void_p]),
    "bevops_conv3x3_c64_f16": (c_int, [c_void_p] * 4 + [c_int] * 6 + [c_void_p]),
    "bevops_deconv4x4s2_packed_weight_size": (c_size_t, [c_int] * 3),
    "bevops_deconv4x4s2_pack_weight": (c_int, [c_int, c_void_p, c_void_p, c_int, c_int, c_void_p]),
    "bevops_deconv4x4s2_f16": (c_int, [c_int] + [c_void_p] * 4 + [c_int] * 9 + [c_void_p]),
    "bevops_conv_slice_f16": (c_int, [c_void_p, c_int, c_void_p, c_void_p, c_void_p, c_int, c_void_p] + [c_int] * 9 +
                              [c_void_p]),
    "bevops_conv_slice_f16_ex": (c_int, [c_void_p, c_int, c_void_p, c_void_p, c_void_p, c_int, c_void_p] + [c_int] * 11 +
                                 [c_void_p]),
    "bevops_lss_camera_gate_packed_size": (c_size_t, [c_int]),
    "bevops_lss_camera_gate": (c_int, [c_void_p, c_int, c_void_p, c_void_p, c_int, c_int, c_void_p]),
    "bevops_se_gate2_nhwc": (c_int, [c_void_p, c_int, c_void_p, c_void_p, c_int, c_void_p] + [c_int] * 4 + [c_void_p]),
    "bevops_global_avgpool_nhwc": (c_int, [c_void_p, c_int, c_void_p] + [c_int] * 4 + [c_void_p]),
    "bevops_focus_nhwc": (c_int, [c_void_p, c_void_p] + [c_int] * 4 + [c_void_p]),
    "bevops_spp_maxpool_nhwc": (c_int, [c_void_p, c_int, c_void_p] + [c_int] * 8 + [c_void_p]),
    "bevops_upsample_nearest2x_nhwc": (c_int, [c_void_p, c_int, c_void_p] + [c_int] * 5 + [c_void_p]),
    "bevops_conv_slice_s8": (c_int, [c_void_p, c_int, c_float, c_void_p, c_void_p, c_float, c_void_p, c_void_p, c_int,
                                     c_float, c_int, c_void_p, c_int, c_float] + [c_int] * 8 + [c_void_p]),
    "bevops_conv_slice_s8_ex": (c_int, [c_void_p, c_int, c_float, c_void_p, c_void_p, c_float, c_void_p, c_void_p, c_int,
                                        c_float, c_int, c_void_p, c_int, c_float] + [c_int] * 9 + [c_void_p]),
    "bevops_conv_slice_s8_ex2": (c_int, [c_void_p, c_int, c_float, c_void_p, c_void_p, c_float, c_void_p, c_void_p, c_int,
                                         c_float, c_int, c_void_p, c_int, c_float] + [c_int] * 10 + [c_void_p, c_int, c_void_p]),
    "bevops_se_gate2_nhwc_s8": (c_int, [c_void_p, c_int, c_float, c_void_p, c_void_p, c_int, c_float, c_void_p, c_int,
                                        c_float] + [c_int] * 3 + [c_void_p]),
    "bevops_global_avgpool_nhwc_s8": (c_int, [c_void_p, c_int, c_float, c_void_p] + [c_int] * 4 + [c_void_p]),
    "bevops_deconv4x4s2_s8": (c_int, [c_void_p, c_float, c_void_p, c_void_p, c_float, c_void_p, c_int, c_void_p, c_float] +
                              [c_int] * 6 + [c_void_p]),
    "bevops_focus_nhwc_q": (c_int, [c_void_p, c_float, c_void_p] + [c_int] * 4 + [c_void_p]),
    "bevops_spp_maxpool_nhwc_s8": (c_int, [c_void_p, c_int, c_void_p] + [c_int] * 8 + [c_void_p]),
    "bevops_upsample_nearest2x_nhwc_s8": (c_int, [c_void_p, c_int, c_void_p] + [c_int] * 5 + [c_void_p]),
    "bevops_refine_reference_points": (c_int, [c_int] + [c_void_p] * 4 + [c_int] * 2 + [c_void_p] * 3),
    "bevops_decode_boxes": (c_int, [c_int] + [c_void_p] * 3 + [c_int] + [c_float] * 6 + [c_void_p] * 3),
    "bevops_bias_relu_maxpool_nhwc": (c_int, [c_int, c_void_p, c_void_p, c_void_p, c_int, c_int, c_int, c_int, c_void_p]),
    "bevops_stem_packed_size": (c_size_t, []),
    "bevops_stem_pack": (c_int, [c_int, c_void_p, c_void_p, c_void_p, c_void_p]),
    "bevops_stem_conv_pool": (c_int, [c_int, c_int, c_void_p, c_void_p, c_void_p, c_int, c_int, c_int, c_float, c_void_p]),
    "bevops_stem_set_variant": (c_int, [c_int]),
    "bevops_conv_tile_int8_fused": (c_int, [c_void_p, c_float, c_void_p, c_void_p, c_float, c_void_p, c_void_p, c_void_p]
                                    + [c_int] * 8 + [c_void_p]),
    "bevops_linear_int8_chain": (c_int, [c_void_p, c_int, c_float, c_void_p, c_void_p, c_float, c_void_p, c_void_p, c_int,
                                         c_float, c_int, c_void_p, c_float, ctypes.c_longlong, c_int, c_int, c_int, c_void_p]),
    "bevops_conv_tile_int8": (c_int, [c_void_p, c_float, c_void_p, c_void_p, c_float, c_void_p, c_void_p, c_int, c_void_p,
                                      c_float] + [c_int] * 8 + [c_void_p]),
    "bevops_bias_relu_maxpool_nhwc_int8": (c_int, [c_int, c_void_p, c_void_p, c_void_p, c_float, c_int, c_int, c_int, c_int,
                                                   c_void_p]),
    "bevops_mdconv_int8_nhwc_workspace_size": (c_size_t, []),
    "bevops_mdconv_forward_int8_nhwc": (c_int, [c_void_p, c_float, c_void_p, c_int, c_float, c_float, c_void_p, c_float,
                                                c_void_p, c_void_p, c_float, c_int, c_int, c_void_p, c_size_t] + [c_int] * 15 +
                                        [c_void_p]),
    "bevops_linear_tune": (c_int, [c_int] + [c_void_p] * 5 + [ctypes.c_longlong, c_int, c_int, c_int,
                                                              c_void_p, c_size_t, c_void_p]),
    "bevops_mdconv_packed_weight_size": (c_size_t, [c_int] * 5),
    "bevops_mdconv_pack_weight": (c_int, [c_int, c_void_p, c_void_p] + [c_int] * 4 + [c_void_p]),
    "bevops_grid_sampler_3d_forward": (c_int, [c_int, c_void_p, c_void_p, c_void_p] + [c_int] * 11 +
                                       [c_void_p]),
    "bevops_qkv_workspace_size": (c_size_t, [c_int] * 5),
    "bevops_qkv_forward": (c_int, [c_int, c_void_p, c_void_p, c_void_p, c_void_p] + [c_int] * 4 + [c_float] * 4 +
                           [c_void_p, c_size_t, c_void_p]),
    "bevops_inverse_forward": (c_int, [c_int, c_void_p, c_void_p, c_int, c_int, c_void_p]),
    "bevops_nms_free_decode": (c_int, [c_int] + [c_void_p] * 6 + [c_int] * 4 + [c_void_p, c_float, c_int, c_void_p]),
    "bevops_centerpoint_decode_workspace_size": (c_size_t, [c_int] * 5),
    "bevops_centerpoint_decode": (c_int, [c_int] + [c_void_p] * 11 + [c_int] * 5 + [c_float] * 5 +
                                  [c_void_p, c_float, c_int, c_int, c_void_p, c_size_t, c_void_p]),
    "bevops_centerpoint_decode_ex": (c_int, [c_int] + [c_void_p] * 11 + [c_int] * 5 + [c_float] * 5 +
                                     [c_void_p, c_float, c_int, c_int, c_void_p, c_size_t, c_void_p]),
    "bevops_bev_nms_workspace_size": (c_size_t, [c_int, c_int]),
    "bevops_bev_nms": (c_int, [c_int] + [c_void_p] * 9 + [c_int] * 4 + [c_float, c_void_p, c_int, c_int, c_void_p,
                                                                        c_size_t, c_void_p]),
    "bevops_bev_iou": (c_int, [c_void_p, c_int, c_void_p, c_int, c_void_p, c_void_p]),
    "bevops_centernet_decode_workspace_size": (c_size_t, [c_int] * 5),
    "bevops_centernet_decode": (c_int, [c_int] + [c_void_p] * 8 + [c_int] * 8 + [c_void_p, c_void_p, c_float, c_void_p,
                                                                               c_size_t, c_void_p]),
    "bevops_yolox_decode": (c_int, [c_int] + [c_void_p] * 8 + [c_int] * 3 + [c_void_p, c_void_p]),
    "bevops_box_nms_workspace_size": (c_size_t, [c_int, c_int]),
    "bevops_box_nms": (c_int, [c_void_p] * 9 + [c_int, c_int, c_float, c_float, c_int, c_int, c_void_p, c_size_t,
                                                c_void_p]),
    "bevops_lss_voxel_prepare_workspace_size": (c_size_t, [c_int] * 4),
    "bevops_lss_voxel_prepare": (c_int, [c_void_p] * 10 + [c_int] * 5 + [c_void_p, c_size_t, c_void_p]),
    "bevops_lss_voxel_prepare_batched_workspace_size": (c_size_t, [c_int] * 5),
    "bevops_lss_voxel_prepare_batched": (c_int, [c_void_p] * 10 + [c_int] * 5 + [c_void_p, c_size_t, c_void_p]),
    "bevops_bev_pool_v2_forward_indirect": (c_int, [c_int] + [c_void_p] * 9 + [c_int] * 4 + [c_float] * 3 + [c_void_p]),
    "bevops_calib_state_size": (c_size_t, []),
    "bevops_calib_collect": (c_int, [c_int, c_void_p, c_size_t, c_void_p, c_void_p]),
    "bevops_calib_threshold_workspace_size": (c_size_t, [c_int]),
    "bevops_calib_threshold": (c_int, [c_int, ctypes.c_double, c_void_p, c_int, c_size_t, c_void_p, c_void_p, c_void_p,
                                       c_size_t, c_void_p]),
    "bevops_deform_conv3x3_nhwc_f16": (c_int, [c_void_p, c_void_p, c_int, c_void_p, c_void_p, c_void_p] + [c_int] * 7 +
                                       [c_void_p]),
}

F32, F16, I8, U8 = 0, 1, 2, 3


def lib_path():
    return os.environ.get("BEVOPS_LIB", os.path.join(_PKG, "libbevops_hip.so"))


def load_library():
    global _LIB
    if _LIB is not None:
        return _LIB
    path = lib_path()
    if not os.path.exists(path):
        raise RuntimeError(
            f"{path} not found: build the HIP kernels first "
            "(`python -c 'import __graft_entry__ as g; g.build()'` or "
            "`make -C bevformer_tensorrt_amd/csrc`). There is no fallback path.")
    import torch
    handle = ctypes.CDLL(os.path.realpath(path))
    for name, (res, args) in SIGNATURES.items():
        fn = getattr(handle, name)
        fn.restype, fn.argtypes = res, args
    _LIB = handle
    return handle


SUCCESS, FAILURE, BAD_PARAM, NOT_SUPPORTED, NOT_INITIALIZED = range(5)


class BevopsError(RuntimeError):

    def __init__(self, message, status):
        super().__init__(message)
        self.status = status


def check(status, what):
    if status != 0:
        msg = load_library().bevops_status_string(status).decode()
        raise BevopsError(f"{what}: {msg} (status {status})", status)


def torch_dtype_code(t):
    import torch
    code = {torch.float32: F32, torch.float16: F16, torch.int8: I8}.get(t.dtype)
    if code is None:
        raise TypeError(f"unsupported dtype {t.dtype}; expected float32, float16 or int8")
    return code


def current_stream_ptr(device):
    import torch
    return torch.cuda.current_stream(device).cuda_stream
```

include/bevops.h:

```cpp
#ifndef BEVOPS_H_
#define BEVOPS_H_

#include <stddef.h>
#include <stdint.h>

#ifdef __cplusplus
extern "C" {
#endif

typedef enum {
  BEVOPS_SUCCESS = 0,
  BEVOPS_FAILURE = 1,
  BEVOPS_BAD_PARAM = 2,
  BEVOPS_NOT_SUPPORTED = 3,
  BEVOPS_NOT_INITIALIZED = 4
} bevops_status_t;

typedef enum { BEVOPS_F32 = 0, BEVOPS_F16 = 1, BEVOPS_I8 = 2, BEVOPS_U8 = 3  } bevops_dtype_t;

typedef enum { BEVOPS_BILINEAR = 0, BEVOPS_NEAREST = 1, BEVOPS_BICUBIC = 2 } bevops_interp_t;
typedef enum { BEVOPS_PAD_ZEROS = 0, BEVOPS_PAD_BORDER = 1, BEVOPS_PAD_REFLECTION = 2 } bevops_pad_t;

const char *bevops_version(void);
const char *bevops_status_string(int status);
void *bevops_query(const char *name);

int bevops_msda_forward(int dtype, const void *value, const int32_t *spatial_shapes,
                        const int32_t *spatial_shapes_host, const void *reference_points,
                        int ref_dtype, const void *sampling_offsets,
                        const void *attention_weights, void *output, int bs, int nk,
                        int heads, int channels, int num_levels, int num_query,
                        int num_point, int points_per_group, float scale_value,
                        float scale_offset, float scale_weight, float scale_out,
                        void *stream);

size_t bevops_msda_workspace_size(int dtype, int bs, int nk, int heads, int channels,
                                  int num_levels, int num_query, int num_point);
size_t bevops_msda_workspace_size_shapes(int dtype, const int32_t *spatial_shapes_host, int bs,
                                         int nk, int heads, int channels, int num_levels,
                                         int num_query, int num_point);
int bevops_msda_forward_ws(int dtype, const void *value, const int32_t *spatial_shapes,
                           const int32_t *spatial_shapes_host, const void *reference_points,
                           int ref_dtype, const void *sampling_offsets,
                           const void *attention_weights, void *output, int bs, int nk,
                           int heads, int channels, int num_levels, int num_query,
                           int num_point, int points_per_group, float scale_value,
                           float scale_offset, float scale_weight, float scale_out,
                           int shared_offsets, void *workspace, size_t workspace_bytes,
                           void *stream);

int bevops_msda_set_variant(int variant);


int bevops_rotate_forward(int dtype, const void *img, const void *angle, const void *center,
                          int angle_dtype, void *output, int channels, int height, int width,
                          int interpolation, float scale_in, float scale_out, void *stream);

int bevops_grid_sampler_2d_forward(int dtype, const void *input, const void *grid, void *output,
                                   int N, int C, int H_in, int W_in, int H_out, int W_out,
                                   int interpolation, int padding, int align_corners,
                                   float scale_in, float scale_grid, float scale_out,
                                   void *stream);
size_t bevops_grid_sampler_2d_workspace_size(int dtype, int N, int C, int H_in, int W_in);
int bevops_grid_sampler_2d_forward_ws(int dtype, const void *input, const void *grid, void *output,
                                      int N, int C, int H_in, int W_in, int H_out, int W_out,
                                      int interpolation, int padding, int align_corners,
                                      float scale_in, float scale_grid, float scale_out,
                                      void *workspace, size_t workspace_bytes, void *stream);
int bevops_grid_sampler_3d_forward(int dtype, const void *input, const void *grid, void *output,
                                   int N, int C, int D_in, int H_in, int W_in, int D_out,
                                   int H_out, int W_out, int interpolation, int padding,
                                   int align_corners, void *stream);

int bevops_bev_pool_v2_forward(int dtype, const void *depth, const void *feat,
                               const int32_t *ranks_depth, const int32_t *ranks_feat,
                               const int32_t *ranks_bev, const int32_t *interval_starts,
                               const int32_t *interval_lengths, void *output, int channels,
                               int n_intervals, int out_height, int out_width,
                               float scale_depth, float scale_feat, float scale_out,
                               void *stream);

size_t bevops_sca_workspace_size(int dtype, const int32_t *spatial_shapes_host, int num_cams, int nk,
                                 int heads, int channels, int num_levels, int num_query,
                                 int num_point);
int bevops_sca_forward(int dtype, const void *value, const int32_t *spatial_shapes_host,
                       const void *reference_points_cam, const void *sampling_offsets,
                       const void *attention_weights, const void *bev_mask, void *output,
                       int num_cams, int nk, int heads, int channels, int num_levels, int num_query,
                       int num_point, int points_per_group, void *workspace, size_t workspace_bytes,
                       void *stream);

int bevops_mdconv_set_variant(int variant);
size_t bevops_mdconv_workspace_size(int dtype, int B, int Cin, int H, int W, int Cout, int Kh,
                                    int Kw, int stride_h, int stride_w, int pad_h, int pad_w,
                                    int dil_h, int dil_w, int groups, int deform_groups);
int bevops_mdconv_forward_int8(const void *input, float scale_in, const void *offset,
                               float scale_offset, const void *mask, float scale_mask,
                               const void *weight, float scale_weight, const float *bias,
                               void *output, float scale_out, void *workspace,
                               size_t workspace_bytes, int B, int Cin, int H, int W, int Cout, int Kh,
                               int Kw, int stride_h, int stride_w, int pad_h, int pad_w, int dil_h,
                               int dil_w, int groups, int deform_groups, void *stream);
int bevops_mdconv_forward_int8_packed(const void *input, float scale_in, const void *offset,
                                      float scale_offset, const void *mask, float scale_mask,
                                      const void *packed_weight, float scale_weight, const float *bias,
                                      void *output, float scale_out, void *workspace,
                                      size_t workspace_bytes, int B, int Cin, int H, int W, int Cout, int Kh,
                                      int Kw, int stride_h, int stride_w, int pad_h, int pad_w, int dil_h,
                                      int dil_w, int groups, int deform_groups, void *stream);
int bevops_mdconv_forward(int dtype, const void *input, const void *offset, const void *mask,
                          const void *weight, const void *bias, void *output, void *workspace,
                          size_t workspace_bytes, int B, int Cin, int H, int W, int Cout, int Kh,
                          int Kw, int stride_h, int stride_w, int pad_h, int pad_w, int dil_h,
                          int dil_w, int groups, int deform_groups, void *stream);
size_t bevops_mdconv_packed_weight_size(int dtype, int Cout, int Cin_per_group, int Kh, int Kw);
int bevops_mdconv_pack_weight(int dtype, const void *weight, void *packed, int Cout,
                              int Cin_per_group, int Kh, int Kw, void *stream);
int bevops_mdconv_forward_nhwc(int dtype, const void *input_nhwc, const void *offset,
                               const void *mask, const void *packed_weight, const void *bias,
                               void *output_nhwc, int relu, int offset_mask_channels,
                               void *workspace, size_t workspace_bytes,
                               int B, int Cin, int H, int W, int Cout, int Kh, int Kw, int stride_h,
                               int stride_w, int pad_h, int pad_w, int dil_h, int dil_w, int groups,
                               int deform_groups, void *stream);
int bevops_bias_act_nhwc(int dtype, void *x, const void *bias, const void *residual, size_t rows,
                         int channels, int relu, void *stream);
int bevops_bias_relu_maxpool_nhwc(int dtype, const void *x, const void *bias, void *out, int n, int h, int w,
                                  int channels, void *stream);
size_t bevops_stem_packed_size(void);
int bevops_stem_pack(int dtype, const void *weight, const void *bias, void *packed, void *stream);
int bevops_stem_conv_pool(int dtype, int out_dtype, const void *x, const void *packed, void *out, int n, int h, int w,
                          float scale_out, void *stream);
int bevops_stem_set_variant(int variant);

int bevops_upsample_add_nhwc(int dtype, void *a, const void *b, int n, int h, int w, int hb, int wb,
                             int channels, void *stream);

int bevops_lss_depth_split(int dtype, const void *x, void *depth, void *feat, int n, int hw, int row_stride,
                           int depth_offset, int D, int feat_offset, int C, void *stream);

int bevops_upsample_bilinear_concat_nhwc(int dtype, const void *a, const void *b, void *out, int n, int h, int w,
                                         int ca, int hb, int wb, int cb, void *stream);

int bevops_lss_depth_split_s8(const void *x_f16, void *depth_q, void *feat_q, int n, int hw, int row_stride,
                              int depth_offset, int D, int feat_offset, int C, float scale_depth, float scale_feat,
                              void *stream);

int bevops_upsample_bilinear_s8(const void *b_q, int b_pitch, float scale_b, void *out_q, int out_pitch, float scale_out,
                                int n, int h, int w, int hb, int wb, int C, void *stream);

int bevops_feat_embed_nhwc(int dtype, const void *src, const void *cam_embed, const void *level_embed, void *dst,
                           int n, size_t rows, int channels, size_t dst_batch_stride, void *stream);
size_t bevops_conv3x3_c32_packed_weight_size(int dtype, int Cin);
int bevops_conv3x3_c32_pack_weight(int dtype, const void *weight, void *packed, int Cout, int Cin, void *stream);
int bevops_conv3x3_c32_set_variant(int variant);
int bevops_conv3x3_c32_forward_nhwc(int dtype, const void *input_nhwc, const void *packed_weight,
                                    const void *bias32, void *output_nhwc, int B, int H, int W, int Cin,
                                    void *stream);
int bevops_rotate_set_variant(int variant);
int bevops_tsa_split(int dtype, const void *both, void *offsets, void *weights, int num_query, int heads, int points,
                     void *stream);
int bevops_queue_mean2(int dtype, const void *x, void *out, size_t count, void *stream);
int bevops_rotate_forward_hwc(int dtype, const void *img, const void *angle, const void *center,
                              int angle_dtype, void *output, int channels, int height, int width,
                              int interpolation, void *stream);
int bevops_layer_norm(int dtype, const void *x, const void *gamma, const void *beta, void *out,
                      size_t rows, int channels, float eps, void *stream);
int bevops_quantize_rows(int dtype, const void *x, void *q, size_t count, float scale, void *stream);
int bevops_dequantize_rows(int dtype, const void *q, void *out, size_t count, float scale, void *stream);
int bevops_linear_int8(const void *a_q, float scale_a, const void *w_q, const float *w_scales,
                       float scale_w, const float *bias, const void *residual, int out_dtype,
                       void *out, float scale_out, long long M, int N, int K, int relu, void *stream);
int bevops_linear_int8_fused(const void *x_f16, float scale_a, const void *w_q, const float *w_scales,
                             float scale_w, const float *bias, const void *residual, int out_dtype,
                             void *out, float scale_out, long long M, int N, int K, int relu, void *stream);
int bevops_tile_gemm_f16(const void *x, const void *weight, const void *bias, const void *residual,
                         void *out, long long M, int N, int K, int relu, void *stream);
int bevops_gemm2_f16(const void *a1, const void *a2, const void *weight, const void *bias, void *out, long long M, int N,
                     int K1, int K2, int a2_B, int a2_H, int a2_W, int a2_stride, int relu, void *stream);
typedef struct bevops_gemm_dst {
  int col_begin, col_end;
  void *out;
  long long out_pitch;
  const void *res;
  long long res_pitch;
} bevops_gemm_dst;
int bevops_tile_gemm_f16_dst(const void *x, const void *weight, const void *bias, const bevops_gemm_dst *dst, int num_dst,
                             long long M, int N, int K, int relu, void *stream);
int bevops_small_gemm_f16_dst(const void *x, const void *weight, const void *bias, const bevops_gemm_dst *dst, int num_dst,
                              long long M, int N, int K, int relu, void *stream);
int bevops_conv_tile_f16(const void *x, const void *weight_taps, const void *bias, const void *residual,
                         void *out, int B, int H, int W, int Cin, int Cout, int ksize, int stride, int relu,
                         void *stream);
int bevops_conv3x3_c64_f16(const void *x, const void *weight_taps, const void *bias, void *out, int B, int H, int W,
                           int Cin, int Cout, int relu, void *stream);
size_t bevops_deconv4x4s2_packed_weight_size(int dtype, int Cin, int Cout);
int bevops_deconv4x4s2_pack_weight(int dtype, const void *weight, void *packed, int Cin, int Cout, void *stream);
int bevops_deconv4x4s2_f16(int dtype, const void *x, const void *packed_weight, const void *bias, void *out, int B, int H,
                           int W, int Cin, int Cout, int ksize, int stride, int pad, int relu, void *stream);
int bevops_conv_slice_f16(const void *x, int x_pitch, const void *weight_taps, const void *bias, const void *residual,
                          int res_pitch, void *out, int out_pitch, int B, int H, int W, int Cin, int Cout, int ksize,
                          int stride, int act, void *stream);
int bevops_conv_slice_f16_ex(const void *x, int x_pitch, const void *weight_taps, const void *bias, const void *residual,
                             int res_pitch, void *out, int out_pitch, int B, int H, int W, int Cin, int Cout, int ksize,
                             int stride, int act, int dilation, int bias_pitch, void *stream);
size_t bevops_lss_camera_gate_packed_size(int mid);
int bevops_lss_camera_gate(const float *mlp_input, int in_pitch, const void *packed, float *gates, int n, int mid,
                           void *stream);
int bevops_se_gate2_nhwc(const void *x, int x_pitch, const float *gates, void *out_a, int a_pitch, void *out_b,
                         int b_pitch, int n, int hw, int c, void *stream);
int bevops_global_avgpool_nhwc(const void *x, int x_pitch, void *out, int out_pitch, int n, int hw, int c, void *stream);
int bevops_focus_nhwc(const void *image, void *out, int out_pitch, int B, int H, int W, void *stream);
int bevops_spp_maxpool_nhwc(const void *x, int x_pitch, void *out, int out_pitch, int B, int H, int W, int C, int k0,
                            int k1, int k2, void *stream);
int bevops_upsample_nearest2x_nhwc(const void *x, int x_pitch, void *out, int out_pitch, int B, int H, int W, int C,
                                   void *stream);
int bevops_conv_slice_s8(const void *x_q, int x_pitch, float scale_a, const void *w_q_taps, const float *w_scales,
                         float scale_w, const float *bias, const void *residual_q, int res_pitch, float scale_res,
                         int out_dtype, void *out, int out_pitch, float scale_out, int B, int H, int W, int Cin, int Cout,
                         int ksize, int stride, int act, void *stream);
int bevops_conv_slice_s8_ex(const void *x_q, int x_pitch, float scale_a, const void *w_q_taps, const float *w_scales,
                            float scale_w, const float *bias, const void *residual_q, int res_pitch, float scale_res,
                            int out_dtype, void *out, int out_pitch, float scale_out, int B, int H, int W, int Cin, int Cout,
                            int ksize, int stride, int act, int res_first, void *stream);
int bevops_conv_slice_s8_ex2(const void *x_q, int x_pitch, float scale_a, const void *w_q_taps, const float *w_scales,
                             float scale_w, const float *bias, const void *residual_q, int res_pitch, float scale_res,
                             int out_dtype, void *out, int out_pitch, float scale_out, int B, int H, int W, int Cin, int Cout,
                             int ksize, int stride, int act, int res_first, int dilation, const void *image_bias_f16,
                             int image_bias_pitch, void *stream);
int bevops_se_gate2_nhwc_s8(const void *x_q, int x_pitch, float scale_x, const float *gates, void *out_a, int a_pitch,
                            float scale_a, void *out_b, int b_pitch, float scale_b, int n, int hw, int c, void *stream);
int bevops_global_avgpool_nhwc_s8(const void *x_q, int x_pitch, float scale_x, void *out, int out_pitch, int n, int hw,
                                  int c, void *stream);
int bevops_deconv4x4s2_s8(const void *x_q, float scale_a, const void *packed_w_q, const float *w_scales, float scale_w,
                          const float *bias, int out_dtype, void *out, float scale_out, int B, int H, int W, int Cin,
                          int Cout, int relu, void *stream);
int bevops_focus_nhwc_q(const void *image, float scale, void *out, int out_pitch, int B, int H, int W, void *stream);
int bevops_spp_maxpool_nhwc_s8(const void *x, int x_pitch, void *out, int out_pitch, int B, int H, int W, int C, int k0,
                               int k1, int k2, void *stream);
int bevops_upsample_nearest2x_nhwc_s8(const void *x, int x_pitch, void *out, int out_pitch, int B, int H, int W, int C,
                                      void *stream);
int bevops_refine_reference_points(int dtype, const void *tmp, const void *reference_points, void *new_reference_points,
                                   void *reference_xy, int num_query, int tmp_stride, const void *log_table,
                                   const void *sigmoid_table, void *stream);
int bevops_decode_boxes(int dtype, const void *regs, const void *refs, void *out, int count, float scale_x, float offset_x,
                        float scale_y, float offset_y, float scale_z, float offset_z, const void *log_table,
                        const void *sigmoid_table, void *stream);
int bevops_conv_tile_int8_fused(const void *x_f16, float scale_a, const void *w_q_taps, const float *w_scales,
                                float scale_w, const float *bias, const void *residual, void *out, int B, int H,
                                int W, int Cin, int Cout, int ksize, int stride, int relu, void *stream);
int bevops_linear_int8_chain(const void *a, int a_dtype, float scale_a, const void *w_q, const float *w_scales,
                             float scale_w, const float *bias, const void *residual, int res_dtype, float scale_res,
                             int out_dtype, void *out, float scale_out, long long M, int N, int K, int relu,
                             void *stream);
int bevops_conv_tile_int8(const void *x_q, float scale_a, const void *w_q_taps, const float *w_scales, float scale_w,
                          const float *bias, const void *residual, int out_dtype, void *out, float scale_out, int B,
                          int H, int W, int Cin, int Cout, int ksize, int stride, int relu, void *stream);
int bevops_bias_relu_maxpool_nhwc_int8(int dtype, const void *x, const void *bias, void *out_q, float scale_out,
                                       int n, int h, int w, int channels, void *stream);
size_t bevops_mdconv_int8_nhwc_workspace_size(void);
int bevops_mdconv_forward_int8_nhwc(const void *input_nhwc, float scale_in, const void *offset_mask_nhwc,
                                    int offset_mask_channels, float scale_offset, float scale_mask,
                                    const void *packed_weight, float scale_weight, const float *bias,
                                    void *output_nhwc, float scale_out, int relu, int exact, void *workspace,
                                    size_t workspace_bytes, int B, int Cin, int H, int W, int Cout, int Kh, int Kw,
                                    int stride_h, int stride_w, int pad_h, int pad_w, int dil_h, int dil_w,
                                    int groups, int deform_groups, void *stream);
int bevops_image_normalize_pad(int in_dtype, const void *images, int out_dtype, void *output, int N,
                               int H0, int W0, int Hp, int Wp, const double *mean_host,
                               const double *std_host, int to_rgb, int channels_last, void *stream);
size_t bevops_image_resize_plan_size(int H0, int W0, int resize_w, int resize_h, int crop_x0, int crop_y0,
                                     int crop_x1, int crop_y1);
int bevops_image_resize_plan_build(int H0, int W0, int resize_w, int resize_h, int crop_x0, int crop_y0, int crop_x1,
                                   int crop_y1, void *plan_host, size_t plan_bytes);
int bevops_image_resize_crop_normalize(const void *images, const void *plan_dev, size_t plan_bytes, int out_dtype,
                                       void *output, void *canvas_or_null, int N, int H0, int W0, int resize_w,
                                       int resize_h, int crop_x0, int crop_y0, int crop_x1, int crop_y1, int rotate,
                                       const double *mean_host, const double *std_host, int to_rgb, int flip,
                                       int channels_last, void *stream);
int bevops_image_normalize_resize_pad(int in_dtype, const void *images, int out_dtype, void *output, int N,
                                      int H0, int W0, int Hs, int Ws, int Hp, int Wp, const double *mean_host,
                                      const double *std_host, int to_rgb, int channels_last, void *stream);
int bevops_image_letterbox(int arith, const void *images, int out_dtype, void *output, int N, int H0, int W0, int Hs,
                           int Ws, int Hp, int Wp, int oy, int ox, const double *pad_host, const double *mean_host,
                           const double *std_host, int to_rgb, int channels_last, void *stream);
size_t bevops_msda_packed_size(int dtype, const int32_t *spatial_shapes_host, int bs, int nk, int heads,
                               int channels, int num_levels, int num_query, int num_point);
int bevops_msda_pack_value(int dtype, int ref_dtype, const void *value, const int32_t *spatial_shapes_host,
                           void *packed, size_t packed_bytes, int bs, int nk, int heads, int channels,
                           int num_levels, int num_query, int num_point, void *stream);
int bevops_msda_forward_prepacked(int dtype, const void *packed, size_t packed_bytes,
                                  const int32_t *spatial_shapes_host, const void *reference_points,
                                  int ref_dtype, const void *sampling_offsets, const void *attention_weights,
                                  void *output, int bs, int nk, int heads, int channels, int num_levels,
                                  int num_query, int num_point, int points_per_group, float scale_value,
                                  float scale_offset, float scale_weight, float scale_out, int shared_offsets,
                                  void *stream);
size_t bevops_linear_workspace_size(void);
int bevops_linear_bias_act(int dtype, const void *a, const void *weight, const void *bias,
                           const void *residual, void *out, long long M, int N, int K, int relu,
                           void *workspace, size_t workspace_bytes, void *stream);
size_t bevops_value_proj_packed_size(const int32_t *spatial_shapes_host, int num_cams, int nk, int heads, int channels,
                                     int num_levels, int num_query, int num_point);
int bevops_value_proj_packed(const void *x, const void *weight, const void *bias, const int32_t *spatial_shapes_host,
                             void *packed, size_t packed_bytes, int num_cams, int nk, int heads, int channels,
                             int num_levels, int num_query, int num_point, void *stream);
int bevops_value_pack_planes(const void *value, const int32_t *spatial_shapes_host, void *packed, size_t packed_bytes,
                             int num_cams, int nk, int heads, int channels, int num_levels, int num_query,
                             int num_point, void *stream);
size_t bevops_sca_prepacked_workspace_size(int num_cams, int heads, int channels, int num_query);
int bevops_sca_forward_prepacked(int dtype, const void *packed, size_t packed_bytes, const int32_t *spatial_shapes_host,
                                 const void *reference_points_cam, const void *sampling_offsets,
                                 const void *attention_weights, const void *bev_mask, void *output, int num_cams,
                                 int nk, int heads, int channels, int num_levels, int num_query, int num_point,
                                 int points_per_group, void *workspace, size_t workspace_bytes, void *stream);
size_t bevops_sca_plan_size(int num_cams, int num_query);
int bevops_sca_plan_build(int dtype, const void *bev_mask, int num_cams, int num_query, void *plan, size_t plan_bytes,
                          void *stream);
int bevops_sca_forward_planned(int dtype, const void *packed, size_t packed_bytes, const int32_t *spatial_shapes_host,
                               const void *reference_points_cam, const void *sampling_offsets,
                               const void *attention_weights, const void *bev_mask, const void *plan, size_t plan_bytes,
                               void *output, int num_cams, int nk, int heads, int channels, int num_levels,
                               int num_query, int num_point, int points_per_group, void *workspace,
                               size_t workspace_bytes, void *stream);

int bevops_point_sampling(int out_dtype, const float *pillars, const float *lidar2img, void *reference_points_cam,
                          void *bev_mask, int num_cams, int num_query, int num_points_in_pillar, float image_h,
                          float image_w, void *stream);

int bevops_tsgemm_f16(const void *x, const void *weight, const void *bias, const void *residual, void *out,
                      long long m, int n, int k, int relu, void *stream);
int bevops_tsgemm_set_variant(int variant);
int bevops_tsgemm_tile_rows(int k);
int bevops_tsgemm_f16_grouped(const void *x, const void *weight, const void *bias, void *out, long long group_stride,
                              long long m, int groups, int k, void *stream);
int bevops_tsgemm_f16_ln(const void *x, const void *weight, const void *bias, const void *residual, const void *ln_weight,
                         const void *ln_bias, float eps, void *out, long long m, int n, int k, void *stream);
size_t bevops_mha_selfattn_max_queries(void);
int bevops_mha_selfattn_f16(const void *qkv, void *out, int num_query, int heads, int head_dim, float scale, void *stream);
int bevops_tsgemm_s8(const void *a_q, float scale_a, const void *w_q, const float *w_scales, float scale_w,
                     const float *bias, const void *residual, int res_dtype, float scale_res, int out_dtype,
                     void *out, float scale_out, long long m, int n, int k, int relu, void *stream);
int bevops_tsgemm_s8_ln(const void *a_q, float scale_a, const void *w_q, const float *w_scales, float scale_w,
                        const float *bias, const void *residual, int res_dtype, float scale_res,
                        const void *ln_weight, const void *ln_bias, float eps, void *out, long long m, int n, int k,
                        void *stream);

int bevops_small_gemm_f16(const void *x, const void *weight, const void *bias, const void *residual, void *out,
                          long long m, int n, int k, int relu, void *stream);

int bevops_linear_tune(int dtype, const void *a, const void *weight, const void *bias,
                       const void *residual, void *out, long long M, int N, int K, int relu,
                       void *workspace, size_t workspace_bytes, void *stream);
int bevops_mdconv_forward_packed(int dtype, const void *input, const void *offset,
                                 const void *mask, const void *packed_weight, const void *bias,
                                 void *output, void *workspace, size_t workspace_bytes, int B,
                                 int Cin, int H, int W, int Cout, int Kh, int Kw, int stride_h,
                                 int stride_w, int pad_h, int pad_w, int dil_h, int dil_w,
                                 int groups, int deform_groups, void *stream);

size_t bevops_qkv_workspace_size(int dtype, int batch, int q_len, int kv_len, int embed_dim);
int bevops_qkv_forward(int dtype, const void *query, const void *key, const void *value, void *output, int batch,
                       int q_len, int kv_len, int embed_dim, float scale_q, float scale_k, float scale_v,
                       float scale_o, void *workspace, size_t workspace_bytes, void *stream);

int bevops_inverse_forward(int dtype, const void *input, void *output, int batch, int n, void *stream);

int bevops_nms_free_decode(int dtype, const void *cls_logits, const void *bbox_preds, float *boxes, float *scores,
                           int32_t *labels, int32_t *count, int batch, int num_query, int num_classes, int max_num,
                           const float *post_center_range_host, float score_threshold, int bottom_center,
                           void *stream);
size_t bevops_centerpoint_decode_workspace_size(int batch, int num_classes, int height, int width, int max_num);
int bevops_centerpoint_decode(int dtype, const void *reg, const void *height, const void *dim, const void *rot,
                              const void *vel, const void *heatmap, const int32_t *strides_host, float *boxes,
                              float *scores, int32_t *labels, int32_t *count, int batch, int num_classes, int map_h,
                              int map_w, int max_num, float out_size_factor, float voxel_x, float voxel_y, float pc_x,
                              float pc_y, const float *post_center_range_host, float score_threshold, int norm_bbox,
                              int heatmap_is_score, void *workspace, size_t workspace_bytes, void *stream);
int bevops_centerpoint_decode_ex(int dtype, const void *reg, const void *height, const void *dim, const void *rot,
                                 const void *vel, const void *heatmap, const int64_t *strides_host, float *boxes,
                                 float *scores, int32_t *labels, int32_t *count, int batch, int num_classes, int map_h,
                                 int map_w, int max_num, float out_size_factor, float voxel_x, float voxel_y,
                                 float pc_x, float pc_y, const float *post_center_range_host, float score_threshold,
                                 int norm_bbox, int heatmap_is_score, void *workspace, size_t workspace_bytes,
                                 void *stream);

size_t bevops_bev_nms_workspace_size(int batch, int num);
int bevops_bev_nms(int mode, const float *boxes_in, const float *scores_in, const int32_t *labels_in,
                   const int32_t *count_in, float *boxes, float *scores, int32_t *labels, int32_t *count,
                   int32_t *index, int batch, int num, int pre_max_size, int post_max_size, float threshold,
                   const float *rescale_factor_host, int num_factors, int bottom_center, void *workspace,
                   size_t workspace_bytes, void *stream);
int bevops_bev_iou(const float *boxes_a, int num_a, const float *boxes_b, int num_b, float *iou, void *stream);

size_t bevops_centernet_decode_workspace_size(int batch, int num_classes, int height, int width, int k);
int bevops_centernet_decode(int dtype, const void *heatmap, const void *wh, const void *offset,
                            const int32_t *strides_host, float *boxes, float *scores, int32_t *labels, int32_t *count,
                            int batch, int num_classes, int map_h, int map_w, int k, int kernel, int inp_h, int inp_w,
                            const float *border_host, const float *scale_factor_host, float score_threshold,
                            void *workspace, size_t workspace_bytes, void *stream);
int bevops_yolox_decode(int dtype, const void *const *cls_host, const void *const *bbox_host,
                        const void *const *obj_host, const int32_t *level_shapes_host, const int32_t *strides_host,
                        float *boxes, float *scores, int32_t *labels, int batch, int num_levels, int num_classes,
                        const float *scale_factor_host, void *stream);
size_t bevops_box_nms_workspace_size(int batch, int num);
int bevops_box_nms(const float *boxes_in, const float *scores_in, const int32_t *labels_in, const int32_t *count_in,
                   float *boxes, float *scores, int32_t *labels, int32_t *count, int32_t *index, int batch, int num,
                   float score_threshold, float iou_threshold, int class_aware, int max_out, void *workspace,
                   size_t workspace_bytes, void *stream);

size_t bevops_lss_voxel_prepare_workspace_size(int n_cams, int d, int h, int w);
int bevops_lss_voxel_prepare(const float *frustum, const float *calib, const float *grid_host, int32_t *ranks_bev,
                             int32_t *ranks_depth, int32_t *ranks_feat, int32_t *interval_starts,
                             int32_t *interval_lengths, int32_t *counts, float *coor, int batch, int n_cams, int d,
                             int h, int w, void *workspace, size_t workspace_bytes, void *stream);
size_t bevops_lss_voxel_prepare_batched_workspace_size(int batch, int n_cams, int d, int h, int w);
int bevops_lss_voxel_prepare_batched(const float *frustum, const float *calib, const float *grid_host,
                                     int32_t *ranks_bev, int32_t *ranks_depth, int32_t *ranks_feat,
                                     int32_t *interval_starts, int32_t *interval_lengths, int32_t *counts, float *coor,
                                     int batch, int n_cams, int d, int h, int w, void *workspace,
                                     size_t workspace_bytes, void *stream);
int bevops_bev_pool_v2_forward_indirect(int dtype, const void *depth, const void *feat, const int32_t *ranks_depth,
                                        const int32_t *ranks_feat, const int32_t *ranks_bev,
                                        const int32_t *interval_starts, const int32_t *interval_lengths,
                                        const int32_t *n_intervals_dev, void *output, int channels, int max_intervals,
                                        int out_height, int out_width, float scale_depth, float scale_feat,
                                        float scale_out, void *stream);

size_t bevops_calib_state_size(void);
int bevops_calib_collect(int dtype, const void *x, size_t count, void *state, void *stream);
size_t bevops_calib_threshold_workspace_size(int num_states);
int bevops_calib_threshold(int method, double percentile, const void *states, int num_states, size_t state_stride,
                           int32_t *bins, double *kl, void *workspace, size_t workspace_bytes, void *stream);

int bevops_deform_conv3x3_nhwc_f16(const void *input_nhwc, const void *offset_nhwc, int offset_channels,
                                   const void *packed_weight, const void *bias, void *output_nhwc, int relu,
                                   int B, int H, int W, int Cin, int Cout, int groups, void *stream);

#ifdef __cplusplus
}
#endif
#endif
```

Measured before the change: 106.6.

## Fuse decoder layer tail and classifier MLPs into a row-chained GEMM kernel

Adds a row_chain kernel that runs a sequence of linear+bias+ReLU/LayerNorm/residual stages for a 16-row block while keeping intermediates in LDS. The decoder uses it to fuse output_proj+norm, FFN, the regression MLP and the next layer's QKV projection into one launch per layer. The batched classification heads go through the same path. This is meant to remove many small kernel launches and global-memory round trips at 900 queries. The cost is low occupancy: few blocks of 1024 threads with large LDS use.

```diff
diff --git a/bevformer_tensorrt_amd/bevformer.py b/bevformer_tensorrt_amd/bevformer.py
--- a/bevformer_tensorrt_amd/bevformer.py
+++ b/bevformer_tensorrt_amd/bevformer.py
@@ -642,6 +642,35 @@
 _MERGED_PROJ = {"enabled": os.environ.get("BEVOPS_MERGED_PROJ", "1") != "0"}
 
 
+_ROW_CHAIN = {"enabled": os.environ.get("BEVOPS_ROW_CHAIN", "1") != "0"}
+
+
+def _chain_ok(ops, x, linears, norms=()):
+    return _ROW_CHAIN["enabled"] and getattr(ops, "row_chain", None) is not None and OWN_KERNELS["enabled"] \
+        and _fast_dense_ok(ops, x, *linears) \
+        and all(type(l) is nn.Linear and l.bias is not None and l.weight.dtype == torch.float16 for l in linears) \
+        and all(isinstance(n, nn.LayerNorm) and n.elementwise_affine and n.weight.dtype == torch.float16 for n in norms)
+
+
+def _packed_weights(ops, owner, cache, weights):
+    key = _versions(*weights)
+    hit = getattr(owner, cache, None)
+    if hit is None or hit[0] != key:
+        hit = (key, [ops.pack_chain_weight(w) for w in weights])
+        setattr(owner, cache, hit)
+    return hit[1]
+
+
+def _chain_stage(lin, norm=None, packed=None, **kw):
+    st = {"weight": lin.weight, "bias": lin.bias}
+    if packed is not None:
+        st["weight"], st["packed"] = packed, tuple(lin.weight.shape)
+    if norm is not None:
+        st["norm"] = (norm.weight, norm.bias, norm.eps)
+    st.update(kw)
+    return st
+
+
 def _merge_ok(ops, x, linears, has_res):
     if not (_MERGED_PROJ["enabled"] and _R3["enabled"] and _FUSED_LINEAR["enabled"]) \
             or getattr(ops, "dense_auto", None) is None or x.dtype != torch.float16 or not x.is_cuda \
@@ -740,7 +769,8 @@
             self._so_aw = (key, torch.cat([so.weight, aw.weight]).detach().contiguous())
         return _or_none(fn, q2, self._so_aw[1], None, widths, [t_so, t_aw])
 
-    def forward(self, query, value, query_pos, reference_points, spatial_shapes, norm=None, projected=None, merged=False):
+    def forward(self, query, value, query_pos, reference_points, spatial_shapes, norm=None, projected=None, merged=False,
+                sample_only=False):
         identity = query
         ops, so, aw = self.ops, self.sampling_offsets, self.attention_weights
         n = query.shape[0]
@@ -769,6 +799,8 @@
             off = so(q).view(1, n, HEADS, -1)
             w = aw(q).view(1, n, HEADS, -1)
         out = ops.multi_scale_deformable_attn(value, spatial_shapes, reference_points, off, w).flatten(2)
+        if sample_only:
+            return out.view(n, EMBED)
         if norm is not None:
             return _dense_norm(ops, self.output_proj, out.view(n, 1, EMBED), identity, norm)
         return _dense(ops, self.output_proj, out.view(n, 1, EMBED), identity, False)
@@ -782,21 +814,27 @@
         self.norms = nn.ModuleList(nn.LayerNorm(EMBED) for _ in range(3))
         self._pos_qkv = None
 
-    def _self_attention(self, ops, query, query_pos, norm=None):
+    def _qkv_term(self, ops, query, query_pos):
+        fn, n = _gemm_entry(ops), query.shape[0]
+        w, b = self.self_attn.in_proj_weight, self.self_attn.in_proj_bias
+        key = _versions(w, b)
+        hit = self._pos_qkv
+        if hit is None or hit[0] != key or hit[1] is not query_pos:
+            term = torch.empty(n, 3 * EMBED, dtype=query.dtype, device=query.device)
+            term[:, :2 * EMBED] = fn(query_pos.reshape(n, EMBED), w[:2 * EMBED], b[:2 * EMBED], None, False)
+            term[:, 2 * EMBED:] = b[2 * EMBED:]
+            hit = self._pos_qkv = (key, query_pos, term)
+        return hit[2]
+
+    def _self_attention(self, ops, query, query_pos, norm=None, qkv=None):
         mha = self.self_attn
         if not _fast_dense_ok(ops, query, mha.out_proj) or mha.in_proj_weight is None:
             return None
         fn, n = _gemm_entry(ops), query.shape[0]
-        w, b = mha.in_proj_weight, mha.in_proj_bias
-        key = _versions(w, b)
-        hit = self._pos_qkv
         try:
-            if hit is None or hit[0] != key or hit[1] is not query_pos:
-                term = torch.empty(n, 3 * EMBED, dtype=query.dtype, device=query.device)
-                term[:, :2 * EMBED] = fn(query_pos.reshape(n, EMBED), w[:2 * EMBED], b[:2 * EMBED], None, False)
-                term[:, 2 * EMBED:] = b[2 * EMBED:]
-                hit = self._pos_qkv = (key, query_pos, term)
-            qkv = fn(query.view(n, EMBED), w, None, hit[2], False).view(1, n, 3, HEADS, EMBED // HEADS)
+            if qkv is None:
+                qkv = fn(query.view(n, EMBED), mha.in_proj_weight, None, self._qkv_term(ops, query, query_pos), False)
+            qkv = qkv.view(1, n, 3, HEADS, EMBED // HEADS)
         except _lib.BevopsError as exc:
             if exc.status != _lib.NOT_SUPPORTED:
                 raise
@@ -812,12 +850,47 @@
             o = o.transpose(1, 2).reshape(n, 1, EMBED)
         return _dense(ops, mha.out_proj, o, query, False) if norm is None else _dense_norm(ops, mha.out_proj, o, query, norm)
 
-    def forward(self, query, value, query_pos, reference_points, spatial_shapes, projected=None, merged=False):
+    def _tail(self, ops, sampled, query_n, query_pos, reg, nxt, out, reg_out):
+        n = sampled.shape[0]
+        cross, ffn = self.cross_attn, self.ffn
+        lins = [cross.output_proj, ffn.fc1, ffn.fc2, reg[0], reg[2], reg[4]]
+        if not _chain_ok(ops, sampled, lins, (self.norms[1], self.norms[2])):
+            return None
+
+        def launch():
+            mha = nxt.self_attn if nxt is not None else None
+            if mha is not None and (mha.in_proj_weight is None or mha.in_proj_weight.dtype != torch.float16
+                                    or not _fast_dense_ok(ops, sampled, mha.out_proj)):
+                mha = None
+            pk = _packed_weights(ops, self, "_tail_packed", [l.weight for l in lins] + ([mha.in_proj_weight] if mha else []))
+            stages = [_chain_stage(cross.output_proj, self.norms[1], pk[0], res=query_n.view(n, EMBED)),
+                      _chain_stage(ffn.fc1, None, pk[1], relu=True),
+                      _chain_stage(ffn.fc2, self.norms[2], pk[2], res_stage=1, store=out),
+                      _chain_stage(reg[0], None, pk[3], relu=True), _chain_stage(reg[2], None, pk[4], relu=True),
+                      _chain_stage(reg[4], None, pk[5], store=reg_out)]
+            if mha is not None:
+                stages.append({"weight": pk[6], "packed": tuple(mha.in_proj_weight.shape), "bias": None, "input": 2,
+                               "res": nxt._qkv_term(ops, sampled, query_pos), "store": True})
+            got = ops.row_chain(sampled, stages)
+            return got[0], got[1], got[2] if len(got) > 2 else None
+        return _or_none(launch)
+
+    def forward(self, query, value, query_pos, reference_points, spatial_shapes, projected=None, merged=False, qkv=None,
+                tail=None):
         ops = self.cross_attn.ops
-        query_n = self._self_attention(ops, query, query_pos, norm=self.norms[0])
+        query_n = self._self_attention(ops, query, query_pos, norm=self.norms[0], qkv=qkv)
         if query_n is None:
             qk = query + query_pos
             query_n = _layer_norm(ops, self.norms[0], query + self.self_attn(qk, qk, query, need_weights=False)[0])
+        if tail is not None:
+            reg, nxt, out, reg_out = tail
+            sampled = self.cross_attn(query_n, value, query_pos, reference_points, spatial_shapes, projected=projected,
+                                      merged=merged, sample_only=True)
+            done = self._tail(ops, sampled, query_n, query_pos, reg, nxt, out, reg_out)
+            if done is not None:
+                return done[0].view(-1, 1, EMBED), done[1].view(1, -1, 10), done[2]
+            query = _dense_norm(ops, self.cross_attn.output_proj, sampled.view(-1, 1, EMBED), query_n, self.norms[1])
+            return self.ffn(query, ops, norm=self.norms[2]), None, None
         query = self.cross_attn(query_n, value, query_pos, reference_points, spatial_shapes, norm=self.norms[1],
                                 projected=projected, merged=merged)
         return self.ffn(query, ops, norm=self.norms[2])
@@ -1022,9 +1095,24 @@
         ref_xy = reference_points[..., :2].unsqueeze(2).contiguous()
         dec_values = _merged_value_proj(self.ops, self, "_dec_vcat", [l.cross_attn.value_proj for l in self.decoder],
                                         bev_embed) if merged else None
+        chained = _ROW_CHAIN["enabled"] and _fast_dense_ok(self.ops, out) and OWN_KERNELS["enabled"] \
+            and getattr(self.ops, "row_chain", None) is not None and all(len(b) == 5 for b in self.reg_branches)
+        hs_all = reg_all = qkv = None
+        if chained:
+            hs_all = torch.empty(6, NUM_QUERY, EMBED, dtype=dtype, device=dev)
+            reg_all = torch.empty(6, NUM_QUERY, 10, dtype=dtype, device=dev)
         for lid, layer in enumerate(self.decoder):
-            out = layer(out, bev_embed, query_pos, ref_xy, bev_shapes, None if dec_values is None else dec_values[lid], merged)
-            tmp = _mlp(self.ops, self.reg_branches[lid], out).view(1, -1, 10)
+            tmp = None
+            if chained:
+                out, tmp, qkv = layer(out, bev_embed, query_pos, ref_xy, bev_shapes, None if dec_values is None else dec_values[lid],
+                                      merged, qkv, (self.reg_branches[lid], self.decoder[lid + 1] if lid < 5 else None,
+                                                    hs_all[lid], reg_all[lid]))
+                if tmp is None:
+                    chained, hs_all = False, None
+            else:
+                out = layer(out, bev_embed, query_pos, ref_xy, bev_shapes, None if dec_values is None else dec_values[lid], merged)
+            if tmp is None:
+                tmp = _mlp(self.ops, self.reg_branches[lid], out).view(1, -1, 10)
             if fused_refine is not None:
                 reference_points, ref_xy = fused_refine(tmp, reference_points)
             else:
@@ -1048,9 +1136,9 @@
                 classes.append(self.cls_branches[lvl](hs))
                 coords.append(crd)
             return bev_embed, torch.stack(classes), torch.stack(coords)
-        crd = torch.stack(regs)
+        crd = reg_all.view(6, 1, NUM_QUERY, 10) if hs_all is not None else torch.stack(regs)
         decode = getattr(self.ops, "decode_boxes", None) if fused_refine is not None else None
-        hs = torch.stack(inter).view(6, NUM_QUERY, EMBED)
+        hs = hs_all if hs_all is not None else torch.stack(inter).view(6, NUM_QUERY, EMBED)
         if decode is not None:
             crd = decode(crd, torch.stack([init_reference] + inter_refs[:-1]), PC_RANGE)
             return bev_embed, self._cls_batched(hs).view(6, 1, NUM_QUERY, -1), crd
@@ -1079,6 +1167,22 @@
 
     def _cls_batched(self, hs):
         key = tuple(p._version for p in self.cls_branches.parameters()) + (hs.dtype, hs.device)
+        b0 = self.cls_branches[0]
+        if hs.is_contiguous() and all(len(b) == 7 and (b[1].eps, b[4].eps) == (b0[1].eps, b0[4].eps) for b in self.cls_branches) \
+                and _chain_ok(self.ops, hs, [b[k] for b in self.cls_branches for k in (0, 3, 6)],
+                              [b[k] for b in self.cls_branches for k in (1, 4)]):
+            ckey = key + tuple(p.data_ptr() for p in self.cls_branches.parameters())
+            if getattr(self, "_cls_chain", None) is None or self._cls_chain[0] != ckey:
+                st = lambda k, attr: torch.stack([getattr(b[k], attr).detach() for b in self.cls_branches]).contiguous()
+                pk = lambda k: {"weight": self.ops.pack_chain_weight(st(k, "weight")), "packed": tuple(b0[k].weight.shape),
+                                "bias": st(k, "bias")}
+                self._cls_chain = (ckey, [
+                    dict(pk(0), norm=(st(1, "weight"), st(1, "bias"), b0[1].eps), relu=True),
+                    dict(pk(3), norm=(st(4, "weight"), st(4, "bias"), b0[4].eps), relu=True),
+                    dict(pk(6), store=True)])
+            got = _or_none(self.ops.row_chain, hs.view(-1, hs.shape[-1]), self._cls_chain[1], len(self.cls_branches))
+            if got is not None:
+                return got[0].view(len(self.cls_branches), hs.shape[1], -1)
         if getattr(self, "_cls_stack", None) is None or self._cls_stack[0] != key:
             st = lambda k, attr: torch.stack([getattr(b[k], attr).detach() for b in self.cls_branches]).to(hs.dtype)
             self._cls_stack = (key, [(st(k, "weight").transpose(1, 2).contiguous(), st(k, "bias").unsqueeze(1)) for k in (0, 3, 6)],
diff --git a/bevformer_tensorrt_amd/csrc/capi.hip b/bevformer_tensorrt_amd/csrc/capi.hip
--- a/bevformer_tensorrt_amd/csrc/capi.hip
+++ b/bevformer_tensorrt_amd/csrc/capi.hip
@@ -115,6 +115,7 @@
     {"bevops_gemm2_f16", (void *)&bevops_gemm2_f16},
     {"bevops_small_gemm_f16_dst", (void *)&bevops_small_gemm_f16_dst},
     {"bevops_small_gemm_f16", (void *)&bevops_small_gemm_f16},
+    {"bevops_row_chain_f16", (void *)&bevops_row_chain_f16},
     {"bevops_conv_tile_f16", (void *)&bevops_conv_tile_f16},
     {"bevops_conv3x3_c64_f16", (void *)&bevops_conv3x3_c64_f16},
     {"bevops_deconv4x4s2_packed_weight_size", (void *)&bevops_deconv4x4s2_packed_weight_size},
diff --git a/bevformer_tensorrt_amd/csrc/row_chain.hip b/bevformer_tensorrt_amd/csrc/row_chain.hip
--- /dev/null
+++ b/bevformer_tensorrt_amd/csrc/row_chain.hip
@@ -0,0 +1,356 @@
+#include "gemm_host.h"
+
+namespace bevops {
+namespace {
+
+typedef _Float16 f16x8_t __attribute__((ext_vector_type(8)));
+
+#ifndef RC_WAVES
+#define RC_WAVES 16
+#endif
+#ifndef RC_DEPTH
+#define RC_DEPTH 1
+#endif
+constexpr int kRcRows = 16, kRcWaves = RC_WAVES, kRcThreads = 64 * kRcWaves, kRcDepth = RC_DEPTH, kRcUnit = 8;
+constexpr int kRcLnLanes = kRcThreads / kRcRows;
+constexpr int kRcUnitK = kRcUnit * 32;
+constexpr int kRcMaxStages = 8, kRcMaxK = 768, kRcMaxN = 768, kRcPad = 8;
+constexpr int kRcXLoads = (kRcRows * kRcMaxK / 8 + kRcThreads - 1) / kRcThreads;
+constexpr int kRcParLoads = (kRcMaxN + kRcThreads - 1) / kRcThreads;
+constexpr int kRcMaxTiles = (kRcMaxN / 16 + kRcWaves - 1) / kRcWaves;
+constexpr size_t kRcMaxLds = 160 * 1024;
+
+struct RcStage {
+  const __half *w, *bias, *gamma, *beta, *res;
+  __half *out[2];
+  int pitch[2], c0[2], c1[2];
+  int K, N, act, norm, ndst, packed;
+  int in_off, in_stride, out_off, out_stride, res_off, res_stride, par_off;
+  unsigned res_bytes;
+  int res_pitch;
+  float eps;
+};
+
+struct RcArgs {
+  const __half *x;
+  unsigned x_bytes;
+  int x_pitch, M, tiles_m, nstages, ln_off, ln_stride, zero_bytes;
+  RcStage s[kRcMaxStages];
+};
+
+__device__ __forceinline__ void rc_emit(const RcStage &st, char *lds, long long grow, int row, bool m_ok, int n, f32x4 v) {
+  if (st.act) {
+#pragma unroll
+    for (int i = 0; i < 4; ++i) v[i] = fmaxf(v[i], 0.f);
+  }
+  const u32x2 q = {pack_h2(v[0], v[1]), pack_h2(v[2], v[3])};
+  if (st.out_off >= 0)
+    *reinterpret_cast<u32x2 *>(lds + st.out_off + ((size_t)row * st.out_stride + n) * 2) = q;
+  if (!m_ok) return;
+#pragma unroll
+  for (int d = 0; d < 2; ++d) {
+    if (d >= st.ndst || n < st.c0[d] || n >= st.c1[d]) continue;
+    __half *o = st.out[d] + grow * st.pitch[d] + (n - st.c0[d]);
+    if (n + 3 < st.c1[d] && (st.pitch[d] & 3) == 0) {
+      *reinterpret_cast<u32x2 *>(o) = q;
+    } else {
+#pragma unroll
+      for (int i = 0; i < 4; ++i)
+        if (n + i < st.c1[d]) o[i] = __ushort_as_half((unsigned short)((i & 1 ? q[i >> 1] >> 16 : q[i >> 1]) & 0xffffu));
+    }
+  }
+}
+
+__device__ __forceinline__ float rc_row_sum(float v) {
+#pragma unroll
+  for (int k = 1; k < kRcLnLanes; k <<= 1) v += __shfl_xor(v, k, kRcLnLanes);
+  return v;
+}
+
+__device__ __forceinline__ f32x4 rc_h4(u32x2 q) { return f32x4{h2f_lo(q[0]), h2f_hi(q[0]), h2f_lo(q[1]), h2f_hi(q[1])}; }
+
+__global__ __launch_bounds__(kRcThreads) void row_chain_f16_kernel(const RcArgs p) {
+  extern __shared__ __attribute__((aligned(16))) char lds[];
+  const int tid = threadIdx.x, lane = tid & 63, wave = tid >> 6;
+  const int g = (int)blockIdx.x / p.tiles_m, m0 = ((int)blockIdx.x % p.tiles_m) * kRcRows;
+  const long long grow0 = (long long)g * p.M + m0;
+  const int l15 = lane & 15, kofs = 8 * (lane >> 4);
+
+  {
+    const int K0 = p.s[0].K, per_row = K0 / 8;
+    const __amdgpu_buffer_rsrc_t rs_x = __builtin_amdgcn_make_buffer_rsrc(const_cast<__half *>(p.x), 0, p.x_bytes, 0x00020000);
+    u32x4 xr[kRcXLoads];
+#pragma unroll
+    for (int i = 0; i < kRcXLoads; ++i) {
+      const int id = tid + i * kRcThreads, r = id / per_row, c = (id % per_row) * 8;
+      const bool ok = r < kRcRows && m0 + r < p.M;
+      xr[i] = __builtin_amdgcn_raw_buffer_load_b128(rs_x, (int)(ok ? (unsigned)(((grow0 + r) * p.x_pitch + c) * 2) : kGemmOob), 0, 0);
+    }
+    unsigned short pr[kRcMaxStages][3][kRcParLoads];
+#pragma unroll
+    for (int s = 0; s < kRcMaxStages; ++s)
+#pragma unroll
+      for (int a = 0; a < 3; ++a) {
+        const __half *src = a == 0 ? p.s[s].bias : a == 1 ? p.s[s].gamma : p.s[s].beta;
+        const int n = s < p.nstages ? p.s[s].N : 0;
+        const __amdgpu_buffer_rsrc_t rs = __builtin_amdgcn_make_buffer_rsrc(
+            const_cast<__half *>(src), 0, src ? (unsigned)((g + 1) * n * 2) : 0u, 0x00020000);
+#pragma unroll
+        for (int i = 0; i < kRcParLoads; ++i) {
+          const int id = tid + i * kRcThreads;
+          pr[s][a][i] = __builtin_amdgcn_raw_buffer_load_b16(rs, (int)(id < n ? (unsigned)((g * n + id) * 2) : kGemmOob), 0, 0);
+        }
+      }
+    if (p.zero_bytes) {
+      for (int i = tid * 16; i < p.zero_bytes; i += kRcThreads * 16) *reinterpret_cast<uint4 *>(lds + i) = make_uint4(0u, 0u, 0u, 0u);
+      __syncthreads();
+    }
+#pragma unroll
+    for (int i = 0; i < kRcXLoads; ++i) {
+      const int id = tid + i * kRcThreads, r = id / per_row, c = (id % per_row) * 8;
+      if (r < kRcRows) *reinterpret_cast<u32x4 *>(lds + ((size_t)r * p.s[0].in_stride + c) * 2) = xr[i];
+    }
+#pragma unroll
+    for (int s = 0; s < kRcMaxStages; ++s)
+#pragma unroll
+      for (int a = 0; a < 3; ++a)
+#pragma unroll
+        for (int i = 0; i < kRcParLoads; ++i) {
+          const int id = tid + i * kRcThreads;
+          if (s < p.nstages && id < p.s[s].N)
+            *reinterpret_cast<unsigned short *>(lds + p.s[s].par_off + ((size_t)a * ((p.s[s].N + 3) & ~3) + id) * 2) = pr[s][a][i];
+        }
+  }
+
+  for (int s = 0; s < p.nstages; ++s) {
+    const RcStage &st = p.s[s];
+    const int K = st.K, N = st.N, N4 = (N + 3) & ~3, ksteps = K / 32;
+    const int chunks = (ksteps + kRcUnit - 1) / kRcUnit;
+    const int ntiles = (N + 15) / 16;
+    const int my_tiles = wave < ntiles ? (ntiles - wave + kRcWaves - 1) / kRcWaves : 0;
+    const int units = my_tiles * chunks;
+    const size_t w_elems = (size_t)(st.packed ? ntiles * 16 : N) * K;
+    const __half *wg = st.w + (size_t)g * w_elems;
+    const __amdgpu_buffer_rsrc_t rs_w = __builtin_amdgcn_make_buffer_rsrc(
+        const_cast<__half *>(wg), 0, (unsigned)(w_elems * 2), 0x00020000);
+    const __amdgpu_buffer_rsrc_t rs_r = __builtin_amdgcn_make_buffer_rsrc(
+        const_cast<__half *>(st.res), 0, st.res_bytes, 0x00020000);
+    const bool m_ok = m0 + l15 < p.M;
+    const char *in_rows = lds + st.in_off + ((size_t)l15 * st.in_stride + kofs) * 2;
+    const unsigned res_row = (unsigned)((grow0 + l15) * st.res_pitch * 2);
+    u32x2 res_t[kRcMaxTiles];
+#pragma unroll
+    for (int t = 0; t < kRcMaxTiles; ++t) {
+      const int n = (wave + kRcWaves * t) * 16 + 4 * (lane >> 4);
+      res_t[t] = __builtin_bit_cast(u32x2, __builtin_amdgcn_raw_buffer_load_b64(
+          rs_r, (int)(m_ok && n < N ? res_row + (unsigned)n * 2 : kGemmOob), 0, 0));
+    }
+    __builtin_amdgcn_sched_barrier(0);
+
+    auto load_unit = [&](u32x4(&f)[kRcUnit], int j, int c) {
+      const int tile = wave + kRcWaves * j, n = tile * 16 + l15;
+      const unsigned base = st.packed ? (unsigned)((((size_t)tile * ksteps + c * kRcUnit) * 64 + lane) * 16)
+                                      : (unsigned)(((size_t)n * K + c * kRcUnitK + kofs) * 2);
+      const unsigned step = st.packed ? 1024u : 64u;
+      const bool n_ok = st.packed ? tile < ntiles : n < N;
+#pragma unroll
+      for (int i = 0; i < kRcUnit; ++i) {
+        const bool ok = n_ok && c * kRcUnit + i < ksteps;
+        f[i] = __builtin_amdgcn_raw_buffer_load_b128(rs_w, (int)(ok ? base + i * step : kGemmOob), 0, 0);
+      }
+    };
+
+    u32x4 wf[kRcDepth][kRcUnit];
+    int pj = 0, pc = 0;
+#pragma unroll
+    for (int d = 0; d < kRcDepth; ++d) {
+      load_unit(wf[d], pj, pc);
+      if (++pc == chunks) { pc = 0; ++pj; }
+      __builtin_amdgcn_sched_barrier(0);
+    }
+    __syncthreads();
+    int cj = 0, cc = 0;
+    f32x4 acc = {0.f, 0.f, 0.f, 0.f};
+    for (int u0 = 0; u0 < units; u0 += kRcDepth) {
+#pragma unroll
+      for (int d = 0; d < kRcDepth; ++d) {
+        const int n = (wave + kRcWaves * cj) * 16 + 4 * (lane >> 4);
+        if (cc == 0) acc = f32x4{0.f, 0.f, 0.f, 0.f};
+#pragma unroll
+        for (int i = 0; i < kRcUnit; ++i) {
+          const u32x4 b = *reinterpret_cast<const u32x4 *>(in_rows + (size_t)(cc * kRcUnit + i) * 64);
+          acc = __builtin_amdgcn_mfma_f32_16x16x32_f16(__builtin_bit_cast(f16x8_t, wf[d][i]),
+                                                       __builtin_bit_cast(f16x8_t, b), acc, 0, 0, 0);
+        }
+        __builtin_amdgcn_sched_barrier(0);
+        load_unit(wf[d], pj, pc);
+        if (++pc == chunks) { pc = 0; ++pj; }
+        __builtin_amdgcn_sched_barrier(0);
+        if (cc == chunks - 1 && cj < my_tiles && n < N) {
+          f32x4 v = acc + rc_h4(*reinterpret_cast<const u32x2 *>(lds + st.par_off + (size_t)n * 2));
+          if (st.res_off >= 0)
+            v += rc_h4(*reinterpret_cast<const u32x2 *>(lds + st.res_off + ((size_t)l15 * st.res_stride + n) * 2));
+          else {
+            u32x2 rres = res_t[0];
+#pragma unroll
+            for (int t = 1; t < kRcMaxTiles; ++t) rres = cj == t ? res_t[t] : rres;
+            v += rc_h4(rres);
+          }
+          if (st.norm)
+            *reinterpret_cast<f32x4 *>(lds + p.ln_off + ((size_t)l15 * p.ln_stride + n) * 4) = v;
+          else
+            rc_emit(st, lds, grow0 + l15, l15, m_ok, n, v);
+        }
+        if (++cc == chunks) { cc = 0; ++cj; }
+      }
+    }
+
+    if (st.norm) {
+      __syncthreads();
+      const int row = tid / kRcLnLanes, j = tid % kRcLnLanes;
+      const float *srow = reinterpret_cast<const float *>(lds + p.ln_off) + (size_t)row * p.ln_stride;
+      const float inv_n = 1.f / (float)N;
+      float sum = 0.f;
+      for (int c = 4 * j; c < N; c += 4 * kRcLnLanes) {
+        const f32x4 v = *reinterpret_cast<const f32x4 *>(srow + c);
+#pragma unroll
+        for (int i = 0; i < 4; ++i)
+          if (c + i < N) sum += v[i];
+      }
+      const float mean = rc_row_sum(sum) * inv_n;
+      float sq = 0.f;
+      for (int c = 4 * j; c < N; c += 4 * kRcLnLanes) {
+        const f32x4 v = *reinterpret_cast<const f32x4 *>(srow + c);
+#pragma unroll
+        for (int i = 0; i < 4; ++i)
+          if (c + i < N) sq = fmaf(v[i] - mean, v[i] - mean, sq);
+      }
+      const float rstd = rsqrtf(rc_row_sum(sq) * inv_n + st.eps);
+      const char *gamma = lds + st.par_off + (size_t)N4 * 2, *beta = gamma + (size_t)N4 * 2;
+      for (int c = 4 * j; c < N; c += 4 * kRcLnLanes) {
+        const f32x4 v = *reinterpret_cast<const f32x4 *>(srow + c);
+        const f32x4 gg = rc_h4(*reinterpret_cast<const u32x2 *>(gamma + (size_t)c * 2));
+        const f32x4 bb = rc_h4(*reinterpret_cast<const u32x2 *>(beta + (size_t)c * 2));
+        f32x4 y = {0.f, 0.f, 0.f, 0.f};
+#pragma unroll
+        for (int i = 0; i < 4; ++i)
+          if (c + i < N) y[i] = fmaf((v[i] - mean) * rstd, gg[i], bb[i]);
+        rc_emit(st, lds, grow0 + row, row, m0 + row < p.M, c, y);
+      }
+    }
+  }
+}
+
+}
+}
+
+using namespace bevops;
+
+extern "C" int bevops_row_chain_f16(const void *x, long long x_pitch, const bevops_chain_stage *stages, int num_stages,
+                                    long long M, int groups, void *stream) {
+  if (!x || !stages || num_stages <= 0 || M < 0 || groups <= 0 || x_pitch <= 0) return BEVOPS_BAD_PARAM;
+  if (num_stages > kRcMaxStages) return BEVOPS_NOT_SUPPORTED;
+  RcArgs a{};
+  int src[kRcMaxStages];
+  bool read[kRcMaxStages + 1] = {};
+  for (int s = 0; s < num_stages; ++s) {
+    const bevops_chain_stage &e = stages[s];
+    if (!e.weight || e.K <= 0 || e.N <= 0 || e.input >= s || e.input < -1 || e.res_stage > s || e.res_stage < -1 ||
+        (e.res && e.res_stage >= 0) || (e.norm && (!e.gamma || !e.beta || !(e.eps >= 0.f))) || e.num_dst < 0 || e.num_dst > 2 ||
+        (e.act != 0 && e.act != 1))
+      return BEVOPS_BAD_PARAM;
+    if (e.K % 32 != 0 || e.K > kRcMaxK || e.N > kRcMaxN) return BEVOPS_NOT_SUPPORTED;
+    if (misaligned(e.weight, 15u) || (e.bias && misaligned(e.bias, 15u)) || (e.res && misaligned(e.res, 15u)) ||
+        (e.norm && (misaligned(e.gamma, 15u) || misaligned(e.beta, 15u))))
+      return BEVOPS_NOT_SUPPORTED;
+    src[s] = e.input < 0 ? s - 1 : e.input;
+    const int k_in = src[s] < 0 ? e.K : stages[src[s]].N;
+    if (k_in != e.K) return BEVOPS_BAD_PARAM;
+    read[src[s] + 1] = true;
+    if (e.res_stage >= 0) {
+      const int r = src[e.res_stage];
+      if ((r < 0 ? stages[0].K : stages[r].N) != e.N) return BEVOPS_BAD_PARAM;
+      read[r + 1] = true;
+    }
+    if (e.res) {
+      if (e.res_pitch < e.N || e.res_pitch > 0x7fffffffLL) return BEVOPS_BAD_PARAM;
+      if (e.N % 4 != 0 || e.res_pitch % 4 != 0 || gemm_over_limit((unsigned long long)M * groups, (int)e.res_pitch, 2))
+        return BEVOPS_NOT_SUPPORTED;
+    }
+    for (int d = 0; d < e.num_dst; ++d) {
+      const bevops_chain_dst &o = e.dst[d];
+      if (!o.out || o.col_begin < 0 || o.col_end > e.N || o.col_end <= o.col_begin || o.col_begin % 8 != 0 ||
+          o.pitch < o.col_end - o.col_begin || o.pitch > 0x7fffffffLL || (d == 1 && o.col_begin < e.dst[0].col_end))
+        return BEVOPS_BAD_PARAM;
+      if (misaligned(o.out, 15u)) return BEVOPS_NOT_SUPPORTED;
+    }
+  }
+  if (misaligned(x, 15u) || x_pitch % 8 != 0 || x_pitch < stages[0].K || x_pitch > 0x7fffffffLL ||
+      gemm_over_limit((unsigned long long)M * groups, (int)x_pitch, 2))
+    return BEVOPS_NOT_SUPPORTED;
+  const long long tiles_m = (M + kRcRows - 1) / kRcRows;
+  if (tiles_m * groups > 0x7fffffffLL || M * groups > 0x7fffffffLL) return BEVOPS_NOT_SUPPORTED;
+  size_t lds = 0;
+  int off[kRcMaxStages + 1], stride[kRcMaxStages + 1];
+  int ln_n = 0;
+  bool padded = false;
+  for (int s = -1; s < num_stages; ++s) {
+    const int width = s < 0 ? stages[0].K : stages[s].N;
+    off[s + 1] = -1;
+    stride[s + 1] = 0;
+    if (s >= 0 && stages[s].norm && width > ln_n) ln_n = width;
+    if (!read[s + 1] && s >= 0) continue;
+    const int wide = (width + kRcUnitK - 1) / kRcUnitK * kRcUnitK;
+    padded = padded || wide != width;
+    off[s + 1] = (int)lds;
+    stride[s + 1] = wide + kRcPad;
+    lds += (size_t)kRcRows * stride[s + 1] * 2;
+    if (lds > kRcMaxLds) return BEVOPS_NOT_SUPPORTED;
+  }
+  a.zero_bytes = padded ? (int)lds : 0;
+  a.ln_off = (int)lds;
+  a.ln_stride = (ln_n + 3) / 4 * 4 + 4;
+  if (ln_n) lds += (size_t)kRcRows * a.ln_stride * 4;
+  int par[kRcMaxStages];
+  for (int s = 0; s < num_stages; ++s) {
+    par[s] = (int)lds;
+    lds += (size_t)3 * ((stages[s].N + 3) / 4 * 4) * 2;
+    lds = (lds + 15) / 16 * 16;
+  }
+  if (lds > kRcMaxLds) return BEVOPS_NOT_SUPPORTED;
+  if (M == 0) return BEVOPS_SUCCESS;
+  a.x = static_cast<const __half *>(x);
+  a.x_pitch = (int)x_pitch;
+  a.x_bytes = (unsigned)((unsigned long long)M * groups * x_pitch * 2);
+  a.M = (int)M;
+  a.tiles_m = (int)tiles_m;
+  a.nstages = num_stages;
+  for (int s = 0; s < num_stages; ++s) {
+    const bevops_chain_stage &e = stages[s];
+    RcStage &t = a.s[s];
+    t.w = static_cast<const __half *>(e.weight);
+    t.bias = static_cast<const __half *>(e.bias);
+    t.gamma = e.norm ? static_cast<const __half *>(e.gamma) : nullptr;
+    t.beta = e.norm ? static_cast<const __half *>(e.beta) : nullptr;
+    t.res = static_cast<const __half *>(e.res);
+    t.res_pitch = e.res ? (int)e.res_pitch : 0;
+    t.res_bytes = e.res ? (unsigned)((unsigned long long)M * groups * e.res_pitch * 2) : 0u;
+    t.packed = e.packed ? 1 : 0;
+    t.K = e.K; t.N = e.N; t.act = e.act; t.norm = e.norm ? 1 : 0; t.ndst = e.num_dst; t.eps = e.eps;
+    for (int d = 0; d < e.num_dst; ++d) {
+      t.out[d] = static_cast<__half *>(e.dst[d].out);
+      t.pitch[d] = (int)e.dst[d].pitch; t.c0[d] = e.dst[d].col_begin; t.c1[d] = e.dst[d].col_end;
+    }
+    t.in_off = off[src[s] + 1];
+    t.in_stride = stride[src[s] + 1];
+    t.out_off = off[s + 1];
+    t.out_stride = stride[s + 1];
+    t.res_off = e.res_stage >= 0 ? off[src[e.res_stage] + 1] : -1;
+    t.res_stride = e.res_stage >= 0 ? stride[src[e.res_stage] + 1] : 0;
+    t.par_off = par[s];
+  }
+  if (!ensure_dynamic_lds<row_chain_f16_kernel>(lds)) return BEVOPS_FAILURE;
+  hipLaunchKernelGGL(row_chain_f16_kernel, dim3((unsigned)(tiles_m * groups)), dim3(kRcThreads), lds,
+                     static_cast<hipStream_t>(stream), a);
+  return launch_status();
+}
diff --git a/bevformer_tensorrt_amd/functions/__init__.py b/bevformer_tensorrt_amd/functions/__init__.py
--- a/bevformer_tensorrt_amd/functions/__init__.py
+++ b/bevformer_tensorrt_amd/functions/__init__.py
@@ -16,7 +16,7 @@
 from .spatial_cross_attention import (spatial_cross_attention_sample, spatial_cross_attention_projected,
                                       spatial_cross_attention_plan)
 from .linear import (linear_bias_act, layer_norm, quantize_rows, dequantize_rows, linear_int8, tsgemm, tsgemm_ln, tsgemm_grouped, tile_gemm, tile_gemm_dst, gemm2, small_gemm, small_gemm_dst,
-                     dense_auto, tsa_split, queue_mean2)
+                     dense_auto, tsa_split, queue_mean2, row_chain, pack_chain_weight)
 from .int8_chain import linear_int8_chain, linear_int8_ln, conv_int8_chain_nhwc, modulated_deformable_conv2d_int8_nhwc
 from .conv import conv_nhwc, conv3x3_nhwc, conv3x3_auto, conv3x3_c64, conv_int8_nhwc, stem_conv_pool
 from .image import (image_normalize_pad, padded_size, bevdet_test_augmentation, bevdet_post_transform, image_resize_plan,
@@ -71,7 +71,7 @@
     "BEVFORMER_IMAGE_PIPELINES", "scaled_size", "scale_lidar2img", "image_normalize_resize_pad",
     "DETECT2D_IMAGE_PIPELINES", "keep_ratio_size", "yolox_test_geometry", "centernet_test_geometry", "image_letterbox",
     "spatial_cross_attention_sample", "spatial_cross_attention_projected", "spatial_cross_attention_plan", "modulated_deformable_conv2d_nhwc", "bias_act_nhwc_", "linear_bias_act", "layer_norm", "rotate_hwc", "conv_offset_nhwc", "upsample_add_nhwc_", "feat_embed_nhwc",
-    "msda_pack_value", "multi_scale_deformable_attn_prepacked", "multi_scale_deformable_attn_local", "image_normalize_pad", "padded_size", "quantize_rows", "dequantize_rows", "linear_int8", "tsgemm", "tsgemm_ln", "tsgemm_grouped", "tile_gemm", "tile_gemm_dst", "gemm2", "small_gemm_dst", "small_gemm", "dense_auto", "tsa_split", "queue_mean2", "conv_nhwc", "conv3x3_nhwc", "conv3x3_auto", "conv3x3_c64", "conv_int8_nhwc", "bias_relu_maxpool_nhwc", "stem_conv_pool", "point_sampling", "self_attention_qkv", "refine_reference_points", "decode_boxes",
+    "msda_pack_value", "multi_scale_deformable_attn_prepacked", "multi_scale_deformable_attn_local", "image_normalize_pad", "padded_size", "quantize_rows", "dequantize_rows", "linear_int8", "tsgemm", "tsgemm_ln", "tsgemm_grouped", "tile_gemm", "tile_gemm_dst", "gemm2", "small_gemm_dst", "small_gemm", "row_chain", "pack_chain_weight", "dense_auto", "tsa_split", "queue_mean2", "conv_nhwc", "conv3x3_nhwc", "conv3x3_auto", "conv3x3_c64", "conv_int8_nhwc", "bias_relu_maxpool_nhwc", "stem_conv_pool", "point_sampling", "self_attention_qkv", "refine_reference_points", "decode_boxes",
     "linear_int8_chain", "linear_int8_ln", "conv_int8_chain_nhwc", "modulated_deformable_conv2d_int8_nhwc",
     "lss_depth_split", "upsample_bilinear_concat_nhwc", "lss_depth_split_q", "upsample_bilinear_nhwc_q",
     "conv_transpose2d_nhwc", "pack_deconv4x4s2", "deconv_packed_weight", "conv_transpose2d_q_nhwc", "quantize_deconv_weight",
diff --git a/bevformer_tensorrt_amd/functions/linear.py b/bevformer_tensorrt_amd/functions/linear.py
--- a/bevformer_tensorrt_amd/functions/linear.py
+++ b/bevformer_tensorrt_amd/functions/linear.py
@@ -243,6 +243,80 @@
     return tile_gemm_dst(x, weight, bias, widths, residuals, relu, outs, _entry="bevops_small_gemm_f16_dst")
 
 
+class _ChainDst(ctypes.Structure):
+    _fields_ = [("col_begin", ctypes.c_int), ("col_end", ctypes.c_int), ("out", ctypes.c_void_p), ("pitch", ctypes.c_longlong)]
+
+
+class _ChainStage(ctypes.Structure):
+    _fields_ = [("weight", ctypes.c_void_p), ("bias", ctypes.c_void_p), ("K", ctypes.c_int), ("N", ctypes.c_int),
+                ("input", ctypes.c_int), ("act", ctypes.c_int), ("packed", ctypes.c_int), ("res", ctypes.c_void_p), ("res_pitch", ctypes.c_longlong),
+                ("res_stage", ctypes.c_int), ("norm", ctypes.c_int), ("gamma", ctypes.c_void_p), ("beta", ctypes.c_void_p),
+                ("eps", ctypes.c_float), ("num_dst", ctypes.c_int), ("dst", _ChainDst * 2)]
+
+
+def pack_chain_weight(weight):
+    *lead, N, K = weight.shape
+    assert weight.dtype == torch.float16 and K % 32 == 0
+    T = (N + 15) // 16
+    w = torch.zeros(*lead, T * 16, K, dtype=weight.dtype, device=weight.device)
+    w[..., :N, :] = weight.detach()
+    w = w.view(*lead, T, 16, K // 32, 4, 8)
+    d = len(lead)
+    return w.permute(*range(d), d, d + 2, d + 3, d + 1, d + 4).reshape(*lead, T * 16 * K).contiguous()
+
+
+def row_chain(x, stages, groups=1):
+    assert x.is_cuda and x.dtype == torch.float16 and x.dim() == 2 and x.stride(1) == 1
+    rows = x.shape[0]
+    assert rows % groups == 0
+    M = rows // groups
+    tab = (_ChainStage * len(stages))()
+    outs, keep = [], []
+    for i, st in enumerate(stages):
+        w, b = st["weight"], st.get("bias")
+        assert w.dtype == torch.float16 and w.is_contiguous() and (b is None or (b.dtype == torch.float16 and b.is_contiguous()))
+        e = tab[i]
+        e.weight, e.bias = w.data_ptr(), _ptr(b)
+        e.N, e.K = st["packed"] if st.get("packed") else (w.shape[-2], w.shape[-1])
+        e.packed = int(bool(st.get("packed")))
+        if e.packed and w.numel() != groups * ((e.N + 15) // 16) * 16 * e.K:
+            raise ValueError("packed weight does not match (N, K)")
+        e.input, e.act = int(st.get("input", -1)), int(bool(st.get("relu", False)))
+        res = st.get("res")
+        e.res_stage = int(st.get("res_stage", -1))
+        if res is not None:
+            if res.dtype != torch.float16 or tuple(res.shape) != (rows, e.N) or res.stride(1) != 1:
+                raise ValueError("res must be fp16 [rows, N] with unit column stride")
+            e.res, e.res_pitch = res.data_ptr(), res.stride(0) if rows > 1 else e.N
+        norm = st.get("norm")
+        if norm is not None:
+            gamma, beta, eps = norm
+            assert gamma.dtype == torch.float16 and beta.dtype == torch.float16 and gamma.is_contiguous() and beta.is_contiguous()
+            e.norm, e.gamma, e.beta, e.eps = 1, gamma.data_ptr(), beta.data_ptr(), float(eps)
+            keep += [gamma, beta]
+        store = st.get("store", False)
+        if store is True:
+            store = torch.empty((rows, e.N), dtype=x.dtype, device=x.device)
+        if torch.is_tensor(store):
+            assert store.dtype == x.dtype and tuple(store.shape) == (rows, e.N) and (e.N == 1 or store.stride(1) == 1)
+            e.num_dst = 1
+            e.dst[0].col_begin, e.dst[0].col_end, e.dst[0].out = 0, e.N, store.data_ptr()
+            e.dst[0].pitch = store.stride(0) if rows > 1 else e.N
+            outs.append(store)
+        elif store:
+            col = 0
+            e.num_dst = len(store)
+            for d, n in enumerate(store):
+                o = torch.empty((rows, n), dtype=x.dtype, device=x.device)
+                e.dst[d].col_begin, e.dst[d].col_end, e.dst[d].out, e.dst[d].pitch = col, col + n, o.data_ptr(), n
+                col += n
+                outs.append(o)
+    if M:
+        _call("bevops_row_chain_f16", x.device, x.data_ptr(), x.stride(0) if rows > 1 else x.shape[1],
+              ctypes.addressof(tab), len(stages), M, int(groups))
+    return outs
+
+
 def tsgemm_weight_stationary(K):
     return _lib.load_library().bevops_tsgemm_tile_rows(int(K)) == 64
 
diff --git a/bevformer_tensorrt_amd/utils/lib.py b/bevformer_tensorrt_amd/utils/lib.py
--- a/bevformer_tensorrt_amd/utils/lib.py
+++ b/bevformer_tensorrt_amd/utils/lib.py
@@ -117,6 +117,7 @@
     "bevops_tile_gemm_f16_dst": (c_int, [c_void_p] * 4 + [c_int, ctypes.c_longlong, c_int, c_int, c_int, c_void_p]),
     "bevops_gemm2_f16": (c_int, [c_void_p] * 5 + [ctypes.c_longlong] + [c_int] * 8 + [c_void_p]),
     "bevops_small_gemm_f16_dst": (c_int, [c_void_p] * 4 + [c_int, ctypes.c_longlong, c_int, c_int, c_int, c_void_p]),
+    "bevops_row_chain_f16": (c_int, [c_void_p, ctypes.c_longlong, c_void_p, c_int, ctypes.c_longlong, c_int, c_void_p]),
     "bevops_conv_tile_f16": (c_int, [c_void_p] * 5 + [c_int] * 8 + [c_void_p]),
     "bevops_conv3x3_c64_f16": (c_int, [c_void_p] * 4 + [c_int] * 6 + [c_void_p]),
     "bevops_deconv4x4s2_packed_weight_size": (c_size_t, [c_int] * 3),
diff --git a/include/bevops.h b/include/bevops.h
--- a/include/bevops.h
+++ b/include/bevops.h
@@ -189,6 +189,26 @@
                              long long M, int N, int K, int relu, void *stream);
 int bevops_small_gemm_f16_dst(const void *x, const void *weight, const void *bias, const bevops_gemm_dst *dst, int num_dst,
                               long long M, int N, int K, int relu, void *stream);
+typedef struct bevops_chain_dst {
+  int col_begin, col_end;
+  void *out;
+  long long pitch;
+} bevops_chain_dst;
+typedef struct bevops_chain_stage {
+  const void *weight, *bias;
+  int K, N;
+  int input, act;
+  int packed;
+  const void *res;
+  long long res_pitch;
+  int res_stage, norm;
+  const void *gamma, *beta;
+  float eps;
+  int num_dst;
+  bevops_chain_dst dst[2];
+} bevops_chain_stage;
+int bevops_row_chain_f16(const void *x, long long x_pitch, const bevops_chain_stage *stages, int num_stages, long long M,
+                         int groups, void *stream);
 int bevops_conv_tile_f16(const void *x, const void *weight_taps, const void *bias, const void *residual,
                          void *out, int B, int H, int W, int Cin, int Cout, int ksize, int stride, int relu,
                          void *stream);
```

New measurement: 108.2, median of 6. 1.01x the previous value.
